# troyvvgroup/quemb

Hardware: AMD Instinct MI355X
Metric: fragment CCSD iters/sec (full BE sweep over synthetic n_occ=20 n_virt=200 fragments); corr-E error vs oracle in parity_max_abs_err_Eh / parity_n220_abs_err_Eh (higher is better)
Workload: dtype f64

## Files before the change

include/qemb_hip_ops.h:

```cpp
#ifndef QEMB_HIP_OPS_H
#define QEMB_HIP_OPS_H
#include "qemb_hip.h"
#ifdef __cplusplus
extern "C" {
#endif

#define QEMB_TIMER_LADDER 0
#define QEMB_TIMER_RINGS 1
#define QEMB_TIMER_ITER 2
#define QEMB_TIMER_AO2MO 3
#define QEMB_TIMER_SCF 4
#define QEMB_TIMER_GEMM_ANY 5
#define QEMB_TIMER_SCHMIDT 6
#define QEMB_TIMER_DF 7
int qemb_timer_begin(int slot);
int qemb_timer_end(int slot);
int qemb_timer_read(int slot, double* total_ms, int64_t* count);
int qemb_timer_reset(int slot);
int qemb_alloc_stats(long long* n_driver_allocs, long long* n_driver_frees, double* ms_in_driver_calls, double* gb_allocated, int reset);
int qemb_gemm_flop_count(double* flops, int reset);
int qemb_tape_cache_counters(int64_t* reused, int64_t* recorded, int reset);
int qemb_ctx_timer_read(int ctx, int slot, double* total_ms, int64_t* count, int reset);
int qemb_timer_live_events(int slot);


int qemb_op_gemm(int64_t M, int64_t N, int64_t K, double alpha, const double* A, int64_t lda, int a_kcontig,
                 int64_t strideA, const double* B, int64_t ldb, int b_kcontig, int64_t strideB, double beta,
                 double* C, int64_t ldc, int64_t strideC, int64_t batch);
int qemb_op_gemm_slab_rows(int64_t M, int64_t N, int64_t K, const double* A, int64_t lda, int64_t a_slab, int64_t a_slab_skip, const double* B, int64_t ldb,
                           int b_kcontig, double* C, int64_t ldc, int cfg);
int qemb_set_gemm_config(int cfg);
int qemb_mfma_f64_peak(int iters, int blocks_per_cu, double* tflops);
int qemb_set_gemm_splitk(int enabled);
int qemb_op_gemm_probe(int64_t M, int64_t N, int64_t K, const double* A, int64_t lda, int a_kcontig, const double* B, int64_t ldb, int b_kcontig,
                       double* C, int64_t ldc, int cfg, int ksplit, double* ms, double* clock_ghz, int64_t* workgroups);
int qemb_op_gemm_stamps(int64_t M, int64_t N, int64_t K, const double* A, int64_t lda, const double* B, int64_t ldb, double* C, int64_t ldc, int cfg,
                        int ksplit, double* out7);
int qemb_pair_gemm_choice(int64_t rows, int64_t cols, int* cfg, int* ksplit);
int qemb_ccsd_gemm_plans(int o, int v, int64_t* out);
int qemb_ccsd_ring_plan(int o, int v, int64_t* out);
int qemb_set_gemm_ksplit(int ksplit);
int qemb_gemm_tile_table(int index, int* id, int* rows, int* cols, int* bk, int* mode1, int* has_classic, int* ladder_twin);
int qemb_gemm_last_launch(int* cfg, int* vec2, int* mode, int* ksplit, int* sb_m, int* sb_n, int* wide_c);
int qemb_op_copy4(const int64_t dim[4], const double* in, const int64_t si[4], double* out,
                  const int64_t so[4], double alpha, double beta);
int qemb_op_outer4(const int64_t dim[4], const double* u, int64_t su0, int64_t su2, const double* v,
                   int64_t sv1, int64_t sv3, double* out, const int64_t so[4], double alpha, double beta);
int qemb_op_div_denom(double* x, int64_t d0, int64_t d1, int64_t d2, int64_t d3, const double* ea,
                      const double* eb, const double* ec, const double* ed);
int qemb_op_ladder_pack_vvvv(int64_t n, int64_t o, const double* M, double* Vp, int64_t ldp, double* Vm, int64_t ldm);
int qemb_op_ladder_pack_tau(int64_t o, int64_t v, const double* tau, double* Tp, int64_t ldp, double* Tm, int64_t ldm);
int qemb_op_ladder_scatter_pm(int64_t o, int64_t v, const double* Rp, int64_t ldp, const double* Rm, int64_t ldm, double* t2);
int qemb_op_dot(int64_t n, const double* x, const double* y, double* out_dev);
int qemb_op_absmax(int64_t n, const double* x, double* out_dev);
int qemb_op_gemv_rows(int64_t rows, int64_t cols, const double* T, int64_t ldt, const double* x, double* y,
                      double alpha, double beta);
int qemb_op_gemv_rows_batched(int64_t rows, int64_t cols, int64_t nbatch, const double* T, int64_t ldt, int64_t strideT,
                              const double* x, int64_t stridex, double* y, double alpha, double beta);
int qemb_op_contract_mid(int64_t outer, int64_t mid, int64_t inner, const double* T, const double* x,
                         double* Y, int64_t ldy, double alpha, double beta);
int qemb_op_unpack_s4(int64_t n, const double* s4, double* s1);
int qemb_op_pack_s4(int64_t n, const double* s1, double* s4);
int qemb_op_unpack_s8_to_s4(int64_t n, const double* s8, double* s4);
int qemb_op_mirror_lower(int64_t n, double* A, int64_t lda);
int qemb_op_k_from_pairs(int64_t n, const double* H, const double* D, double* K);
int qemb_op_jk_from_packed(int64_t n, const double* S4, const double* D, const double* Dp, double* Jp, double* K);
int qemb_op_pack_pm_cols(int64_t rows, int64_t v, const double* in, double* Op, int64_t ldp, double* Om, int64_t ldm);
int qemb_op_scatter_pm_rows(int64_t o, int64_t ncols, const double* Xp, const double* Xm, double* out);
int qemb_op_pack_w_pm(int64_t o, const double* W, double* Ap, int64_t lda_p, double* Am, int64_t lda_m);
int qemb_op_ladder_scatter_pm2(int64_t o, int64_t v, const double* Rp, int64_t ldp, const double* Rm, int64_t ldm, const double* Hp, const double* Hm,
                               int assign, double* t2);
int qemb_op_lincomb2(int64_t n, double a, const double* x, double b, const double* y, double beta, double* out);
int qemb_op_small_k_update(int64_t batch, int64_t M, int64_t N, int64_t K, double alpha, const double* A, int64_t sA, const double* B, int64_t sB, double* C, int64_t sC);
int qemb_op_ccsd_ph_layouts(int64_t o, int64_t v, const double* t2, const double* t1, double* T, double* Tp, double* S, double* Ut, double* Tpt, double* Th);
int qemb_op_ccsd_y_traces(int64_t o, int64_t v, const double* ZC, const double* ZB, double* Y);
int qemb_op_ccsd_ph_layouts_ring(int64_t o, int64_t v, const double* t2, const double* t1, double* Tp, double* S, double* Ut, double* Tpt);
int qemb_op_ccsd_ovvv_slabs(int64_t o, int64_t v);
int qemb_op_ccsd_ovvv_pass(int64_t o, int64_t v, const double* ovvv, const double* t1, const double* Thk, double* ZB, double* PA);
int qemb_op_ccsd_ring_prep(int64_t o, int64_t v, const double* t1, const double* P1, const double* W1base, const double* W2base, const double* ZB, const double* ZC,
                           const double* OB, const double* OC, double* R, double* W2);
int qemb_op_ccsd_ring_prep_rule(int64_t o, int64_t v, int replay);
int qemb_op_ccsd_u_update(int64_t o, int64_t v, const double* A, const double* t1, const double* Z, double* U);
int qemb_op_copy4_two(const int64_t dim[4], const double* in, const int64_t si[4], double* out, const int64_t so[4], double alpha, double beta, const double* base,
                      double* out2, const double* in2, double c2a, double c2b);
int qemb_op_scatter_pm_rows_add(int64_t o, int64_t ncols, const double* Xp, const double* Xm, double* out, const double* add);
int qemb_op_ccsd_y_traces_add(int64_t o, int64_t v, const double* ZC, const double* ZB, double* Y, const double* add);
int qemb_op_pack_w_pm_sum(int64_t o, const double* Wt, const double* X, const double* At, double* Ap, int64_t lda_p, double* Am, int64_t lda_m);
int qemb_op_ccsd_t1_assemble(int64_t o, int64_t v, const double* t1, const double* Lvv, const double* Loo, const double* Fov, const double* S, const double* Lph1,
                             const double* PA, int SA, int64_t strideA, const double* PB, int SB, int64_t strideB, double* t1n);
int qemb_op_gemv_rows_two(int64_t rows1, int64_t cols1, const double* T1, int64_t ld1, const double* x1, double* y1, double a1, double b1,
                          int64_t rows2, int64_t cols2, const double* T2, int64_t ld2, const double* x2, double* y2, double a2, double b2);
int qemb_op_ccsd_y_traces_slabs(int64_t o, int64_t v, const double* ZC, const double* ZB, double* Y, const double* add, int S, int64_t stride, double scale);
int qemb_op_ccsd_finish_t2_rings(int64_t o, int64_t v, double* t2n, const double* U, const double* OV, const double* RS, const double* M, const double* eo, const double* ev, double* t1n);
int qemb_op_diis_push(int64_t n, const double* trial, const double* prev, double* e, double* xcopy, int m, const double* const* ys, int self, double* row_dev, double* row_host);
int qemb_op_ccsd_extrapolate_energy(int64_t o, int64_t v, int nterms, const double* coef, const double* const* xs, double* amp, const double* L, double* tau, double* e_host);
int qemb_op_gather_rows(int64_t nrows, int64_t len, const int64_t* idx_dev, const double* src, int64_t ld, double* dst);
int qemb_op_scale_rows(int64_t nrows, int64_t len, double* x, const double* s);
int qemb_op_pack_pair_rows(int64_t n, int64_t ncols, const double* in, double* out);
int qemb_op_unpack_tril_pair_rows(int64_t nr, int64_t n, const double* in, double* full);
int qemb_op_extract_pf(int64_t n, const double* Mp, int64_t p0, int64_t q0, int64_t r0, int64_t s0, int64_t sp, int64_t sq,
                       int64_t sr, int64_t ss, double* out);
int qemb_op_extract_pf_t(int64_t n, const double* T, int64_t x0, int64_t r0, int64_t s0, int64_t c0, int64_t sx, int64_t sr,
                         int64_t ss, int64_t sc, double* out);
int qemb_op_ladder_pack_vvvv_pf(int64_t n, int64_t o, const double* Mp, double* Vp, int64_t ldp, double* Vm, int64_t ldm);
int qemb_op_extract_pf_t_compact(int64_t n, const double* T, int64_t x0, int64_t c0, int64_t sx, int64_t sr, int64_t ss, int64_t sc,
                                 double* out, int64_t slab);
int qemb_op_gather_pair_cols(int64_t rows, int64_t n, const double* in, int64_t r0, int64_t s0, int64_t sr, int64_t ss, double* out);
int qemb_op_extract_ps(int64_t n, const double* S, int64_t p0, int64_t q0, int64_t r0, int64_t s0, int64_t sp, int64_t sq,
                       int64_t sr, int64_t ss, double* out);
int qemb_op_extract_ps_packed(int64_t n, const double* S, int64_t p0, int64_t q0, int64_t r0, int64_t sp, int64_t sq, int64_t sr, double* out);
int qemb_op_unpack_pair_block(int64_t n, int64_t o, const double* S, double* Mv, int64_t ld);
int qemb_op_ladder_pack_vvvv_pf_ld(int64_t n, int64_t o, const double* Mp, int64_t ld, double* Vp, int64_t ldp, double* Vm, int64_t ldm);
int qemb_op_pack_pm_ovvv(int64_t o, int64_t v, const double* ovvv, double* Op, int64_t ldp, double* Om, int64_t ldm);
int qemb_op_df_pair_product(int64_t np, int64_t naux, const double* bb, double* out);
int qemb_op_unpack_tril_rows(int64_t rows, int64_t n, const double* packed, double* full);
int qemb_op_pack_tril_rows(int64_t rows, int64_t n, const double* full, double* packed);
int qemb_op_jacobi_eigh(int64_t n, double* A, double* w, double* V, int* sweeps);
int qemb_op_scf_fused_max(void);
int qemb_op_jacobi_eigh_in_basis(int64_t n, const double* F, const double* Cp, double* w, double* C_out, double* C2_out, int nocc, double* dm_out, double stop_below, int* sweeps);
int qemb_op_scf_fock_small(int64_t n, const double* h, const double* J, const double* K, const double* D, double* F, double* err, double* scal2);
int qemb_op_pack_density_sym(int64_t n, const double* D, double* Dp);
int qemb_op_jacobi_svd(int64_t m, int64_t n, double* G, double* s, double* U, double* V, int* sweeps);
int qemb_op_cholesky_lower(int64_t n, double* A);
int qemb_op_tri_inverse_lower(int64_t n, const double* L, double* Linv);


int qemb_op_mp2_amplitudes(int64_t o, int64_t v, const double* ovov, const double* eo, const double* ev, double* t2, double* G, double* e_host);

int qemb_op_rdm2_assemble(int kind, int64_t o, int64_t v, const double* t1, const double* t2, const double* dm1c, double* out);
int qemb_op_ccsd_t(int o, int v, const double* t1, const double* t2, const double* ovvv, const double* ovoo, const double* ovov, const double* eo, const double* ev, int tile, double* e_t);
int qemb_op_rdm2_add_nc(int64_t m, const double* g, double alpha, double* X);
int qemb_op_rdm2_symmetrize(int64_t m, const double* g, double* X);
int qemb_op_rdm2_eri_dot(int64_t m, int sym, const double* eri, const double* K, double* e_host);

int qemb_op_kdf_split(int64_t rows, int64_t nao, const double* z, double* planes);
int qemb_op_kdf_stack(int64_t nk, int64_t nao, int64_t n, const double* ta, double* Cs, double* Dk);
int qemb_op_kdf_pack(int64_t naux, int64_t n, const double* M, int paired, double w, double* F, int64_t ldf, double* out2_host);

int qemb_frag_prepare_ccsd(qemb_frag_t f, int nsocc, const double* h, const double* dm0, const qemb_solver_opts* opts);
int qemb_frag_ccsd_iterate(qemb_frag_t f, int niter, double* e_corr, double* normt);
int qemb_frag_ccsd_reset(qemb_frag_t f);
int qemb_frag_ccsd_export(qemb_frag_t f, const char* name, double* host, int64_t nelem);


int qemb_op_boys(int m_max, int64_t n, const double* x, double* out);
int qemb_op_int3c_class(int la, int lb, int lP, const void* bf_a, const void* bf_b, const void* bf_P, const double* c2s, double* out_host);
int qemb_op_int4c_class(int la, int lb, int lc, int ld, const void* bf_a, const void* bf_b, const void* bf_c, const void* bf_d, const double* c2s, double* out_host);
int qemb_op_int4c_tile(void* basis, const int32_t* pairs_r, int64_t n_r, const int32_t* pairs_s, int64_t n_s, double thresh, double* out_host);
int qemb_op_cd_panel_factor(int n, const double* A_host, double thr, double* T_host, int32_t* piv_host, int32_t* rank, int* in_lds);
int qemb_op_cd_diag_update(int64_t np, int r, const double* Lnew_host, const int32_t* pivrow_host, double* d_host, int64_t nsp, const int32_t* row0_host, const int32_t* cnt_host,
                           double* spmax_host, double* dmax_host);
int qemb_op_cd_permute(int64_t M, int64_t N, const double* L_host, const int32_t* pos_host, int full, double* out_host);
int qemb_op_df_get_ints(void* df, double* out_host, int* identity_metric);

int qemb_op_fci_sigma(int n, int nsocc, const double* h_host, const double* V_dev, const double* c_dev, double* sigma_dev);
int qemb_op_fci_rdm12(int n, int nsocc, const double* c_dev, int cumulant, double* dm1_host, double* dm2_dev);
int qemb_op_fci_sigma_timed(int n, int nsocc, const double* h_host, const double* V_dev, const double* c_dev, double* sigma_dev, double* ms3);
int qemb_op_fci_sigma_slab(int n, int nsocc, const double* h_host, const double* V_dev, const double* c_dev, double* sigma_dev, int64_t rows, double* ms3);
int qemb_op_fci_rdm12_slab(int n, int nsocc, const double* c_dev, int cumulant, int64_t rows, double* dm1_host, double* dm2_dev);
int qemb_op_fci_links(int n, int nsocc, int64_t* ns, int* nlink, int32_t* strings_host, int32_t* links_host);
int qemb_op_sci_screen(int n, int nsocc, const double* h_host, const double* V_dev, int64_t ndet, const uint64_t* alpha, const uint64_t* beta, const double* c, double eps,
                       int64_t slab, int64_t cap, int64_t max_out, int64_t* njoined, uint64_t* out_alpha, uint64_t* out_beta);
int qemb_op_sci_pt2(int n, int nsocc, const double* h_host, const double* V_dev, int64_t ndet, const uint64_t* alpha, const uint64_t* beta, const double* c, double e_var, double eps_pt,
                    int64_t max_ext, int64_t slab, int64_t cap, double* e_pt2, int64_t* n_ext, int* batches);
int qemb_op_sci_merge(int64_t ndet, const uint64_t* alpha, const uint64_t* beta, const double* c, int64_t njoined, const uint64_t* jalpha, const uint64_t* jbeta,
                      uint64_t* out_alpha, uint64_t* out_beta, double* out_c);
int qemb_op_sci_matrix(int n, const double* h_host, const double* V_dev, int64_t ndet, const uint64_t* alpha, const uint64_t* beta, int64_t max_nnz, int64_t* nnz,
                       int64_t* rowptr, int32_t* col, double* val);
int qemb_op_sci_spmv(int n, const double* h_host, const double* V_dev, int64_t ndet, const uint64_t* alpha, const uint64_t* beta, const double* x, double* y);
int qemb_op_sci_rdm12(int n, int nsocc, const double* h_host, const double* V_dev, int64_t ndet, const uint64_t* alpha, const uint64_t* beta, const double* c, int cumulant,
                      double* dm1, double* dm2);
int qemb_frag_sci_stage_ms(qemb_frag_t f, double* ms5);

int qemb_op_joint_diag(int64_t K, int64_t m, double* Q_dev, double* U_dev, double stop_angle, int max_sweeps, int* sweeps, double* f, int* converged);
int qemb_op_joint_diag_bytes(int64_t K, int64_t m, int64_t* bytes, int* in_lds);
int qemb_op_joint_diag_mem_limit(int64_t bytes);

#ifdef __cplusplus
}
#endif
#endif
```

quemb_amd/_lib.py:

```python

from __future__ import annotations

import ctypes as C
import os
from pathlib import Path

import numpy as np

_HERE = Path(__file__).resolve().parent
LIB_PATH = _HERE / "libqemb_hip.so"

c_dp = C.POINTER(C.c_double)
c_i64 = C.c_int64
c_vp = C.c_void_p


QEMB_ERR_ARG, QEMB_ERR_ALLOC, QEMB_ERR_DEVICE, QEMB_ERR_NOCONV, QEMB_ERR_NUMERIC, QEMB_ERR_UNSUPPORTED = -1, -2, -3, -4, -5, -6


class QembError(RuntimeError):

    def __init__(self, msg="", status=None):
        super().__init__(msg)
        self.status = status


class SolverOpts(C.Structure):
    _fields_ = [("struct_size", C.c_uint32), ("cc_conv_tol", C.c_double), ("cc_conv_tol_normt", C.c_double), ("cc_max_cycle", C.c_int),
                ("cc_diis_space", C.c_int), ("scf_conv_tol", C.c_double), ("scf_conv_tol_grad", C.c_double),
                ("scf_max_cycle", C.c_int), ("scf_diis_space", C.c_int), ("warm_start", C.c_int), ("verbose", C.c_int),
                ("relax_density", C.c_int), ("lambda_conv_tol", C.c_double), ("lambda_max_cycle", C.c_int),
                ("strict_convergence", C.c_int)]


class FciOpts(C.Structure):
    _fields_ = [("struct_size", C.c_uint32), ("conv_tol", C.c_double), ("max_cycle", C.c_int), ("max_space", C.c_int), ("lindep", C.c_double)]


class SciOpts(C.Structure):
    _fields_ = [("struct_size", C.c_uint32), ("eps_var", C.c_double), ("conv_tol", C.c_double), ("max_cycle", C.c_int), ("max_space", C.c_int),
                ("max_round", C.c_int), ("max_det", C.c_int64)]


_lib = None
_initialised_device = None


def _declare(lib):
    def f(name, restype, *argtypes):
        fn = getattr(lib, name)
        fn.restype = restype
        fn.argtypes = list(argtypes)

    I, D, P, V, L = C.c_int, C.c_double, c_vp, c_vp, c_i64
    f("qemb_init", I, I)
    f("qemb_last_error", C.c_char_p)
    f("qemb_backend", C.c_char_p)
    f("qemb_sync", I)
    f("qemb_device_sync", I)
    f("qemb_mem_info", I, C.POINTER(C.c_size_t), C.POINTER(C.c_size_t))
    f("qemb_malloc", I, C.POINTER(c_vp), C.c_size_t)
    f("qemb_free", I, V)
    f("qemb_trim", I)
    f("qemb_trim_all", I)
    f("qemb_h2d", I, V, V, C.c_size_t)
    f("qemb_d2h", I, V, V, C.c_size_t)
    f("qemb_h2d_async", I, V, V, C.c_size_t)
    f("qemb_d2d", I, V, V, C.c_size_t)
    f("qemb_timer_begin", I, I)
    f("qemb_timer_end", I, I)
    f("qemb_timer_read", I, I, C.POINTER(D), C.POINTER(L))
    f("qemb_timer_reset", I, I)
    f("qemb_timer_live_events", I, I)
    f("qemb_op_gemm", I, L, L, L, D, P, L, I, L, P, L, I, L, D, P, L, L, L)
    f("qemb_op_gemm_slab_rows", I, L, L, L, P, L, L, L, P, L, I, P, L, I)
    f("qemb_op_gemm_probe", I, L, L, L, P, L, I, P, L, I, P, L, I, I, C.POINTER(D), C.POINTER(D), C.POINTER(L))
    f("qemb_op_gemm_stamps", I, L, L, L, P, L, P, L, P, L, I, I, C.POINTER(D))
    f("qemb_set_gemm_config", I, I)
    f("qemb_set_gemm_splitk", I, I)
    f("qemb_set_gemm_ksplit", I, I)
    f("qemb_pair_gemm_choice", I, L, L, C.POINTER(I), C.POINTER(I))
    f("qemb_ccsd_gemm_plans", I, I, I, C.POINTER(L))
    f("qemb_ccsd_ring_plan", I, I, I, C.POINTER(L))
    f("qemb_gemm_tile_table", I, I, *([C.POINTER(I)] * 7))
    f("qemb_gemm_last_launch", I, *([C.POINTER(I)] * 7))
    f("qemb_op_ladder_pack_vvvv", I, L, L, P, P, L, P, L)
    f("qemb_op_ladder_pack_tau", I, L, L, P, P, L, P, L)
    f("qemb_op_ladder_scatter_pm", I, L, L, P, L, P, L, P)
    f("qemb_mfma_f64_peak", I, I, I, C.POINTER(D))
    f("qemb_op_copy4", I, C.POINTER(L), P, C.POINTER(L), P, C.POINTER(L), D, D)
    f("qemb_op_outer4", I, C.POINTER(L), P, L, L, P, L, L, P, C.POINTER(L), D, D)
    f("qemb_op_div_denom", I, P, L, L, L, L, P, P, P, P)
    f("qemb_op_dot", I, L, P, P, P)
    f("qemb_op_mp2_amplitudes", I, L, L, P, P, P, P, P, C.POINTER(D))
    f("qemb_op_rdm2_assemble", I, I, L, L, P, P, P, P)
    f("qemb_op_rdm2_add_nc", I, L, P, D, P)
    f("qemb_op_rdm2_symmetrize", I, L, P, P)
    f("qemb_op_rdm2_eri_dot", I, L, I, P, P, C.POINTER(D))
    f("qemb_op_absmax", I, L, P, P)
    f("qemb_op_gemv_rows", I, L, L, P, L, P, P, D, D)
    f("qemb_op_gemv_rows_batched", I, L, L, L, P, L, L, P, L, P, D, D)
    f("qemb_op_contract_mid", I, L, L, L, P, P, P, L, D, D)
    f("qemb_op_unpack_s4", I, L, P, P)
    f("qemb_op_pack_s4", I, L, P, P)
    f("qemb_op_unpack_s8_to_s4", I, L, P, P)
    f("qemb_op_unpack_tril_rows", I, L, L, P, P)
    f("qemb_op_pack_pair_rows", I, L, L, P, P)
    f("qemb_op_mirror_lower", I, L, P, L)
    f("qemb_op_k_from_pairs", I, L, P, P, P)
    f("qemb_op_jk_from_packed", I, L, P, P, P, P, P)
    f("qemb_op_pack_pm_cols", I, L, L, P, P, L, P, L)
    f("qemb_op_scatter_pm_rows", I, L, L, P, P, P)
    f("qemb_op_pack_w_pm", I, L, P, P, L, P, L)
    f("qemb_op_ladder_scatter_pm2", I, L, L, P, L, P, L, P, P, I, P)
    f("qemb_op_lincomb2", I, L, D, P, D, P, D, P)
    f("qemb_op_small_k_update", I, L, L, L, L, D, P, L, P, L, P, L)
    f("qemb_op_ccsd_ph_layouts", I, L, L, P, P, P, P, P, P, P, P)
    f("qemb_op_ccsd_ph_layouts_ring", I, L, L, P, P, P, P, P, P)
    f("qemb_op_ccsd_ring_prep", I, L, L, P, P, P, P, P, P, P, P, P, P)
    f("qemb_op_ccsd_ring_prep_rule", I, L, L, I)
    f("qemb_op_ccsd_u_update", I, L, L, P, P, P, P)
    f("qemb_op_ccsd_ovvv_slabs", I, L, L)
    f("qemb_op_ccsd_ovvv_pass", I, L, L, P, P, P, P, P)
    f("qemb_op_ccsd_y_traces", I, L, L, P, P, P)
    f("qemb_op_copy4_two", I, C.POINTER(L), P, C.POINTER(L), P, C.POINTER(L), D, D, P, P, P, D, D)
    f("qemb_op_scatter_pm_rows_add", I, L, L, P, P, P, P)
    f("qemb_op_ccsd_y_traces_add", I, L, L, P, P, P, P)
    f("qemb_op_pack_w_pm_sum", I, L, P, P, P, P, L, P, L)
    f("qemb_op_ccsd_t1_assemble", I, L, L, P, P, P, P, P, P, P, I, L, P, I, L, P)
    f("qemb_op_gemv_rows_two", I, L, L, P, L, P, P, D, D, L, L, P, L, P, P, D, D)
    f("qemb_op_ccsd_y_traces_slabs", I, L, L, P, P, P, P, I, L, D)
    f("qemb_op_ccsd_finish_t2_rings", I, L, L, P, P, P, P, P, P, P, P)
    f("qemb_op_diis_push", I, L, P, P, P, P, I, P, I, P, P)
    f("qemb_op_ccsd_extrapolate_energy", I, L, L, I, P, P, P, P, P, P)
    f("qemb_op_gather_rows", I, L, L, P, P, L, P)
    f("qemb_op_scale_rows", I, L, L, P, P)
    f("qemb_ctx_count", I, I)
    f("qemb_ctx_bind", I, I)
    f("qemb_ctx_partition", I, I)
    f("qemb_ctx_timer_read", I, I, I, C.POINTER(C.c_double), C.POINTER(c_i64), I)
    f("qemb_gemm_flop_count", I, C.POINTER(C.c_double), I)
    f("qemb_tape_cache_counters", I, C.POINTER(L), C.POINTER(L), I)
    f("qemb_alloc_stats", I, C.POINTER(C.c_longlong), C.POINTER(C.c_longlong), C.POINTER(C.c_double), C.POINTER(C.c_double), I)
    f("qemb_op_unpack_tril_pair_rows", I, L, L, P, P)
    f("qemb_op_extract_pf", I, L, P, L, L, L, L, L, L, L, L, P)
    f("qemb_op_extract_pf_t", I, L, P, L, L, L, L, L, L, L, L, P)
    f("qemb_op_ladder_pack_vvvv_pf", I, L, L, P, P, L, P, L)
    f("qemb_op_extract_pf_t_compact", I, L, P, L, L, L, L, L, L, P, L)
    f("qemb_op_gather_pair_cols", I, L, L, P, L, L, L, L, P)
    f("qemb_op_extract_ps", I, L, P, L, L, L, L, L, L, L, L, P)
    f("qemb_op_extract_ps_packed", I, L, P, L, L, L, L, L, L, P)
    f("qemb_op_unpack_pair_block", I, L, L, P, P, L)
    f("qemb_op_ladder_pack_vvvv_pf_ld", I, L, L, P, L, P, L, P, L)
    f("qemb_op_pack_pm_ovvv", I, L, L, P, P, L, P, L)
    f("qemb_op_df_pair_product", I, L, L, P, P)
    f("qemb_op_pack_tril_rows", I, L, L, P, P)
    f("qemb_op_jacobi_eigh", I, L, P, P, P, C.POINTER(I))
    f("qemb_op_scf_fused_max", I)
    f("qemb_op_jacobi_eigh_in_basis", I, L, P, P, P, P, P, I, P, D, C.POINTER(I))
    f("qemb_op_scf_fock_small", I, L, P, P, P, P, P, P, P)
    f("qemb_op_pack_density_sym", I, L, P, P)
    f("qemb_op_jacobi_svd", I, L, L, P, P, P, P, C.POINTER(I))
    f("qemb_op_cholesky_lower", I, L, P)
    f("qemb_op_joint_diag", I, L, L, P, P, D, I, C.POINTER(I), C.POINTER(D), C.POINTER(I))
    f("qemb_df_localize_er", I, V, P, I, D, I, P, C.POINTER(I), C.POINTER(D), C.POINTER(D), C.POINTER(I))
    f("qemb_op_joint_diag_bytes", I, L, L, C.POINTER(L), C.POINTER(I))
    f("qemb_op_joint_diag_mem_limit", I, L)
    f("qemb_op_tri_inverse_lower", I, L, P, P)
    f("qemb_comm_unique_id", I, P)
    f("qemb_comm_init", I, I, I, P)
    f("qemb_comm_info", I, C.POINTER(I), C.POINTER(I))
    f("qemb_comm_allreduce", I, P, L, I)
    f("qemb_comm_destroy", I)
    OP = C.POINTER(SolverOpts)
    IP = C.POINTER(I)
    DP = C.POINTER(D)
    f("qemb_default_opts", None, OP)
    f("qemb_frag_create", I, I, I, C.POINTER(c_vp))
    f("qemb_frag_free", I, V)
    f("qemb_frag_set_eri_s4", I, V, P)
    f("qemb_frag_set_eri_s4_dev", I, V, P)
    f("qemb_frag_set_df_factor", I, V, I, P)
    f("qemb_frag_set_df_factor_dev", I, V, I, P)
    f("qemb_frag_mo_route", I, V, I)
    f("qemb_frag_set_df_only", I, V, I, P)
    f("qemb_frag_set_df_only_dev", I, V, I, V)
    f("qemb_frag_resident_bytes", I, V, C.POINTER(L))
    f("qemb_frag_mo_route_used", I, V, IP, IP)
    f("qemb_frag_get_eri_s4", I, V, P)
    f("qemb_frag_set_energy_data", I, V, P, P, P, D, IP, I)
    f("qemb_frag_jk", I, V, P, P, P)
    f("qemb_frag_solve", I, V, I, P, P, OP, I, P, P, P, P, P, P, P, DP, DP, DP, IP, IP)
    f("qemb_frag_solve_mp2", I, V, I, P, P, OP, I, P, P, P, P, P, P, DP, DP, DP, IP)
    f("qemb_frag_solve_mp2_batch", I, I, P, IP, P, P, OP, I, P, P, P, P, P, P, P, P, P, IP)
    f("qemb_default_fci_opts", None, C.POINTER(FciOpts))
    f("qemb_frag_solve_fci", I, V, I, P, P, OP, C.POINTER(FciOpts), I, P, P, P, P, P, P, DP, DP, DP, IP, IP)
    f("qemb_frag_fci_bytes", I, I, I, I, C.POINTER(L))
    f("qemb_frag_fci_mem_limit", I, V, L)
    f("qemb_frag_fci_residual", I, V, DP)
    f("qemb_frag_fci_slab", I, V, L)
    f("qemb_frag_fci_bytes_slab", I, I, I, I, L, C.POINTER(L))
    f("qemb_frag_fci_slab_used", I, V, C.POINTER(L), C.POINTER(L))
    f("qemb_op_fci_sigma_slab", I, I, I, P, P, P, P, L, P)
    f("qemb_op_fci_rdm12_slab", I, I, I, P, I, L, P, P)
    f("qemb_op_fci_sigma", I, I, I, P, P, P, P)
    f("qemb_op_fci_rdm12", I, I, I, P, I, P, P)
    f("qemb_op_fci_sigma_timed", I, I, I, P, P, P, P, P)
    f("qemb_op_fci_links", I, I, I, C.POINTER(L), IP, P, P)
    f("qemb_default_sci_opts", None, C.POINTER(SciOpts))
    f("qemb_frag_solve_sci", I, V, I, P, P, OP, C.POINTER(SciOpts), I, P, P, P, P, P, DP, DP, DP, IP, IP)
    f("qemb_frag_sci_stats", I, V, C.POINTER(L), IP, C.POINTER(L), DP)
    f("qemb_frag_sci_stage_ms", I, V, P)
    f("qemb_frag_sci_dets", I, V, P, P, P)
    f("qemb_frag_sci_bytes", I, I, I, L, I, C.POINTER(L))
    f("qemb_frag_sci_mem_limit", I, V, L)
    f("qemb_frag_sci_pt2", I, V, D, L, DP, C.POINTER(L), IP, P)
    f("qemb_frag_sci_pt2_bytes", I, I, I, L, L, C.POINTER(L))
    f("qemb_op_sci_pt2", I, I, I, P, P, L, P, P, P, D, D, L, L, L, DP, C.POINTER(L), IP)
    f("qemb_op_sci_screen", I, I, I, P, P, L, P, P, P, D, L, L, L, C.POINTER(L), P, P)
    f("qemb_op_sci_merge", I, L, P, P, P, L, P, P, P, P, P)
    f("qemb_op_sci_matrix", I, I, P, P, L, P, P, L, C.POINTER(L), P, P, P)
    f("qemb_op_sci_spmv", I, I, P, P, L, P, P, P, P)
    f("qemb_op_sci_rdm12", I, I, I, P, P, L, P, P, P, I, P, P)
    f("qemb_frag_rdm2", I, V, I, I, P)
    f("qemb_frag_rdm2_mem_limit", I, V, L)
    f("qemb_frag_ccsd_t", I, V, DP, IP, C.POINTER(L), P)
    f("qemb_frag_ccsd_t_bytes", I, V, I, I, C.POINTER(L))
    f("qemb_frag_ccsd_t_mem_limit", I, V, L)
    f("qemb_frag_drop_amplitudes", I, V)
    f("qemb_op_ccsd_t", I, I, I, P, P, P, P, P, P, P, I, DP)
    f("qemb_frag_rdm2_dev", I, V, I, I, P)
    f("qemb_rdm2_full_guard", I, L, L, L)
    f("qemb_frag_lambda_iters", I, P, C.POINTER(C.c_int))
    f("qemb_frag_solve_batch", I, I, P, IP, P, P, OP, I, P, P, P, P, P, P, P, P, P, P, IP, IP, C.POINTER(L))
    f("qemb_frag_scf", I, V, I, P, P, OP, P, P, P, P, DP, IP, IP)
    f("qemb_frag_cphf", I, V, I, P, P, OP, P, I, P)
    f("qemb_ccsd_solve", I, I, I, I, P, P, P, OP, P, P, D, IP, I, P, P, P, P, P, P, DP, IP)
    f("qemb_frag_prepare_ccsd", I, V, I, P, P, OP)
    f("qemb_frag_ccsd_iterate", I, V, I, DP, DP)
    f("qemb_frag_ccsd_reset", I, V)
    f("qemb_frag_ccsd_export", I, V, C.c_char_p, P, L)
    LP = C.POINTER(L)
    f("qemb_aoeri_upload", I, I, P, I, C.POINTER(c_vp))
    f("qemb_aoeri_free", I, V)
    f("qemb_ao2mo_dense", I, V, P, I, P, V)
    f("qemb_df_create", I, I, P, C.POINTER(c_vp))
    f("qemb_lpq_upload", I, P, I, C.POINTER(c_vp))
    f("qemb_df_create_pbc", I, I, P, C.POINTER(c_vp), IP)
    f("qemb_df_alloc_ints", I, V, I)
    f("qemb_df_add_pw_block", I, V, I, P, P, P, P)
    f("qemb_df_add_rs_block", I, V, I, I, P)
    f("qemb_df_pw_imag_absmax", I, V, C.POINTER(C.c_double))
    f("qemb_df_pw_select", I, V, I)
    f("qemb_df_free", I, V)
    f("qemb_df_set_ints", I, V, I, P, I)
    f("qemb_df_set_ints_semisparse", I, V, I, L, P, P, P, P)
    f("qemb_df_transform", I, V, P, I, P, V)
    f("qemb_df_transform_screened", I, V, P, I, P, D, P, V)
    f("qemb_df_transform_factor", I, V, P, I, V)
    f("qemb_df_transform_screened_factor", I, V, P, I, P, D, V)
    f("qemb_kdf_create", I, I, I, I, IP, IP, C.POINTER(c_vp))
    f("qemb_kdf_set_pair", I, V, I, I, P)
    f("qemb_kdf_transform", I, V, P, I, P, V, I)
    f("qemb_kdf_free", I, V)
    f("qemb_kdf_guard", I, I, I, I, I, I, I, L)
    f("qemb_frag_get_df_factor", I, V, P)
    f("qemb_int_basis_create", I, I, P, C.c_size_t, P, C.POINTER(c_vp))
    f("qemb_int_basis_free", I, V)
    f("qemb_int3c2e", I, V, V, P, L, I, P, I)
    f("qemb_int2c2e", I, V, P, I)
    f("qemb_df_create_empty", I, C.POINTER(c_vp))
    f("qemb_df_set_ints_from_basis", I, V, V, V)
    f("qemb_df_set_ints_semisparse_from_basis", I, V, V, V, L, P, P, P, P)
    f("qemb_int4c2e", I, V, I, D, P, I)
    f("qemb_int4c_mem_limit", I, V, L)
    f("qemb_int4c_stats", I, V, C.POINTER(L), C.POINTER(L))
    f("qemb_aoeri_from_basis", I, V, D, C.POINTER(c_vp))
    f("qemb_int_jk_direct", I, V, P, D, P, P, I)
    f("qemb_int_jk_direct_bytes", I, V, C.POINTER(L))
    f("qemb_ao2mo_direct", I, V, I, P, P, P, P, L, D)
    f("qemb_ao2mo_direct_bytes", I, V, I, P, L, C.POINTER(L))
    f("qemb_int4c_tile_stats", I, V, C.POINTER(L), C.POINTER(L))
    f("qemb_op_int4c_tile", I, V, P, L, P, L, D, P)
    f("qemb_int_cholesky", I, V, D, D, L, L, P, C.POINTER(L))
    f("qemb_int_cholesky_bytes", I, V, L, L, C.POINTER(L))
    f("qemb_int_cholesky_stats", I, V, P)
    f("qemb_df_set_ints_from_cholesky", I, V, V, D, D, L, L)
# ... 112 lines not shown
```

quemb_amd/csrc/api.cpp:

```cpp
#include <cstring>
#include <cstdlib>
#include <vector>
#include <execinfo.h>
#include <signal.h>
#include <unistd.h>
#include "../../include/qemb_hip_ops.h"
#include "dev_ops.h"
#include "ccsd.h"
#include "fragment.h"
#include "ao2mo.h"
#include "kdf.h"
#include "int3c.h"
#include "int4c.h"
#include "cd_core.h"
#include "loc_core.h"
#include "sci_core.h"
#include <algorithm>
#include <cmath>
#include <mutex>
#include <set>

using namespace qemb;
namespace qemb {
int dev_mfma_f64_peak(int iters, int blocks_per_cu, double* tflops);
// ... 111 lines not shown
  if (ksplit) *ksplit = p.ks;
  return QEMB_OK;
}
int qemb_ccsd_gemm_plans(int o, int v, int64_t* out) {
  if (o < 1 || v < 0 || !out) { set_error("qemb_ccsd_gemm_plans: bad arguments"); return QEMB_ERR_ARG; }
  const CcsdGemmPlans p = ccsd_gemm_plans(o, v);
  for (const GemmPlan* g : {&p.fvv, &p.pa, &p.pb, &p.ladder_p, &p.ladder_m, &p.xw_p, &p.xw_m, &p.x_p, &p.x_m})
    for (const int64_t x : {g->M, g->N, g->K, (int64_t)g->cfg, (int64_t)g->ks, (int64_t)g->S}) *out++ = x;
  return QEMB_OK;
}
int qemb_ccsd_ring_plan(int o, int v, int64_t* out) {
  if (o < 1 || v < 0 || !out) { set_error("qemb_ccsd_ring_plan: bad arguments"); return QEMB_ERR_ARG; }
  const CcsdRingPlan r = ccsd_ring_plan(o, v);
  out[0] = ((int64_t)o * o * v * v <= (int64_t)1 << 22) ? 1 : 0; out[1] = r.cfg; out[2] = r.ks; out[3] = r.region_ws_bytes;
  return QEMB_OK;
}
int qemb_set_gemm_splitk(int enabled) { dev_gemm_set_auto_splitk(enabled); return QEMB_OK; }
int qemb_op_copy4(const int64_t dim[4], const double* in, const int64_t si[4], double* out, const int64_t so[4],
                  double alpha, double beta) {
  Copy4Desc c{};
  for (int k = 0; k < 4; ++k) { c.dim[k] = dim[k]; c.si[k] = si[k]; c.so[k] = so[k]; }
  c.in = in; c.out = out; c.alpha = alpha; c.beta = beta;
  return dev_copy4(c);
}
int qemb_op_outer4(const int64_t dim[4], const double* u, int64_t su0, int64_t su2, const double* v, int64_t sv1,
                   int64_t sv3, double* out, const int64_t so[4], double alpha, double beta) {
  Outer4Desc o{};
  for (int k = 0; k < 4; ++k) { o.dim[k] = dim[k]; o.so[k] = so[k]; }
  o.u = u; o.su0 = su0; o.su2 = su2; o.v = v; o.sv1 = sv1; o.sv3 = sv3; o.out = out; o.alpha = alpha; o.beta = beta;
  return dev_outer4(o);
}
int qemb_op_div_denom(double* x, int64_t d0, int64_t d1, int64_t d2, int64_t d3, const double* ea, const double* eb,
                      const double* ec, const double* ed) { return dev_div_denom(x, d0, d1, d2, d3, ea, eb, ec, ed); }
int qemb_op_ladder_pack_vvvv(int64_t n, int64_t o, const double* M, double* Vp, int64_t ldp, double* Vm, int64_t ldm) { return dev_ladder_pack_vvvv(n, o, M, Vp, ldp, Vm, ldm); }
int qemb_op_ladder_pack_tau(int64_t o, int64_t v, const double* tau, double* Tp, int64_t ldp, double* Tm, int64_t ldm) { return dev_ladder_pack_tau(o, v, tau, Tp, ldp, Tm, ldm); }
int qemb_op_ladder_scatter_pm(int64_t o, int64_t v, const double* Rp, int64_t ldp, const double* Rm, int64_t ldm, double* t2) { return dev_ladder_scatter_pm(o, v, Rp, ldp, Rm, ldm, t2); }
int qemb_op_dot(int64_t n, const double* x, const double* y, double* o) { return dev_dot(n, x, y, o); }
int qemb_op_absmax(int64_t n, const double* x, double* o) { return dev_absmax(n, x, o); }
int qemb_op_gemv_rows(int64_t rows, int64_t cols, const double* T, int64_t ldt, const double* x, double* y, double alpha,
                      double beta) { return dev_gemv_rows(rows, cols, T, ldt, x, y, alpha, beta); }
int qemb_op_gemv_rows_batched(int64_t rows, int64_t cols, int64_t nbatch, const double* T, int64_t ldt, int64_t strideT, const double* x,
                              int64_t stridex, double* y, double alpha, double beta) { return dev_gemv_rows_batched(rows, cols, nbatch, T, ldt, strideT, x, stridex, y, alpha, beta); }
int qemb_op_contract_mid(int64_t outer, int64_t mid, int64_t inner, const double* T, const double* x, double* Y,
                         int64_t ldy, double alpha, double beta) { return dev_contract_mid(outer, mid, inner, T, x, Y, ldy, alpha, beta); }
int qemb_op_unpack_s4(int64_t n, const double* s4, double* s1) { return dev_unpack_s4(n, s4, s1); }
int qemb_op_pack_s4(int64_t n, const double* s1, double* s4) { return dev_pack_s4(n, s1, s4); }
int qemb_op_unpack_s8_to_s4(int64_t n, const double* s8, double* s4) { return dev_unpack_s8_to_s4(n, s8, s4); }
int qemb_comm_unique_id(void* id) { return dev_comm_unique_id(id); }
int qemb_comm_init(int rank, int world, const void* id) { return dev_comm_init(rank, world, id); }
int qemb_comm_info(int* rank, int* world) { return dev_comm_info(rank, world); }
int qemb_comm_allreduce(double* buf, int64_t n, int op) { return dev_comm_allreduce(buf, n, op); }
int qemb_comm_destroy(void) { return dev_comm_destroy(); }
int qemb_ctx_count(int n) { return dev_ctx_count(n); }
int qemb_ctx_bind(int k) { return dev_ctx_bind(k); }
int qemb_ctx_partition(int parts) { return dev_ctx_partition(parts); }
int qemb_op_gemm_slab_rows(int64_t M, int64_t N, int64_t K, const double* A, int64_t lda, int64_t a_slab, int64_t a_slab_skip, const double* B, int64_t ldb,
                           int b_kcontig, double* C, int64_t ldc, int cfg) {
  GemmDesc g{};
  g.M = M; g.N = N; g.K = K; g.alpha = 1.0; g.beta = 0.0;
  g.A = A; g.lda = lda; g.a_kcontig = 0; g.strideA = 0; g.a_slab = a_slab; g.a_slab_skip = a_slab_skip;
  g.B = B; g.ldb = ldb; g.b_kcontig = b_kcontig; g.strideB = 0;
  g.C = C; g.ldc = ldc; g.strideC = 0; g.batch = 1; g.cfg = cfg; g.ksplit = 0;
  return dev_gemm(g);
}
int qemb_gemm_flop_count(double* flops, int reset) { return dev_gemm_flop_count(flops, reset); }
int qemb_tape_cache_counters(int64_t* reused, int64_t* recorded, int reset) {
  long long a = 0, b = 0;
  tape_cache_counters(&a, &b, reset);
  if (reused) *reused = a;
  if (recorded) *recorded = b;
  return QEMB_OK;
}
int qemb_alloc_stats(long long* n, long long* nfree, double* ms, double* gb, int reset) { return dev_alloc_stats(n, nfree, ms, gb, reset); }
int qemb_ctx_timer_read(int ctx, int slot, double* total_ms, int64_t* count, int reset) { return dev_ctx_timer_read(ctx, slot, total_ms, count, reset); }
int qemb_op_k_from_pairs(int64_t n, const double* H, const double* D, double* K) { return dev_k_from_pairs(n, H, D, K); }
int qemb_op_jk_from_packed(int64_t n, const double* S4, const double* D, const double* Dp, double* Jp, double* K) { return dev_jk_from_packed(n, S4, D, Dp, Jp, K); }
int qemb_op_pack_pm_cols(int64_t rows, int64_t v, const double* in, double* Op, int64_t ldp, double* Om, int64_t ldm) { return dev_pack_pm_cols(rows, v, in, Op, ldp, Om, ldm); }
int qemb_op_scatter_pm_rows(int64_t o, int64_t ncols, const double* Xp, const double* Xm, double* out) { return dev_scatter_pm_rows(o, ncols, Xp, Xm, out); }
int qemb_op_pack_w_pm(int64_t o, const double* W, double* Ap, int64_t lda_p, double* Am, int64_t lda_m) { return dev_pack_w_pm(o, W, Ap, lda_p, Am, lda_m); }
int qemb_op_ladder_scatter_pm2(int64_t o, int64_t v, const double* Rp, int64_t ldp, const double* Rm, int64_t ldm, const double* Hp, const double* Hm,
                               int assign, double* t2) { return dev_ladder_scatter_pm2(o, v, Rp, ldp, Rm, ldm, Hp, Hm, assign, t2); }
int qemb_op_lincomb2(int64_t n, double a, const double* x, double b, const double* y, double beta, double* out) {
  const double c[2] = {a, b};
  const double* xs[2] = {x, y};
  return dev_lincomb(n, 2, c, xs, beta, out);
}
int qemb_op_mirror_lower(int64_t n, double* A, int64_t lda) { return dev_mirror_lower(n, A, lda); }
int qemb_op_small_k_update(int64_t batch, int64_t M, int64_t N, int64_t K, double alpha, const double* A, int64_t sA, const double* B, int64_t sB, double* C, int64_t sC) {
  return dev_small_k_update(batch, M, N, K, alpha, A, sA, B, sB, C, sC);
}
int qemb_op_ccsd_ph_layouts(int64_t o, int64_t v, const double* t2, const double* t1, double* T, double* Tp, double* S, double* Ut, double* Tpt, double* Th) {
  return dev_ccsd_ph_layouts(o, v, t2, t1, T, Tp, S, Ut, Tpt, Th);
}
int qemb_op_ccsd_ph_layouts_ring(int64_t o, int64_t v, const double* t2, const double* t1, double* Tp, double* S, double* Ut, double* Tpt) {
  return dev_ccsd_ph_layouts_ring(o, v, t2, t1, Tp, S, Ut, Tpt);
}
int qemb_op_ccsd_ring_prep(int64_t o, int64_t v, const double* t1, const double* P1, const double* W1base, const double* W2base, const double* ZB, const double* ZC,
                           const double* OB, const double* OC, double* R, double* W2) {
  return dev_ccsd_ring_prep(o, v, t1, P1, W1base, W2base, ZB, ZC, OB, OC, R, W2);
}
int qemb_op_ccsd_u_update(int64_t o, int64_t v, const double* A, const double* t1, const double* Z, double* U) { return dev_ccsd_u_update(o, v, A, t1, Z, U); }
int qemb_op_ccsd_ring_prep_rule(int64_t o, int64_t v, int replay) { return ccsd_use_ring_prep(o, v, replay != 0) ? 1 : 0; }
int qemb_op_ccsd_ovvv_slabs(int64_t o, int64_t v) { return dev_ccsd_ovvv_slabs(o, v); }
int qemb_op_ccsd_ovvv_pass(int64_t o, int64_t v, const double* ovvv, const double* t1, const double* Thk, double* ZB, double* PA) {
  return dev_ccsd_ovvv_pass(o, v, ovvv, t1, Thk, ZB, PA);
}
int qemb_op_copy4_two(const int64_t dim[4], const double* in, const int64_t si[4], double* out, const int64_t so[4], double alpha, double beta, const double* base,
                      double* out2, const double* in2, double c2a, double c2b) {
  Copy4Desc c{};
  for (int k = 0; k < 4; ++k) { c.dim[k] = dim[k]; c.si[k] = si[k]; c.so[k] = so[k]; }
  c.in = in; c.out = out; c.alpha = alpha; c.beta = beta; c.base = base;
  c.out2 = out2; c.in2 = in2; c.c2a = c2a; c.c2b = c2b;
  return dev_copy4(c);
}
int qemb_op_scatter_pm_rows_add(int64_t o, int64_t ncols, const double* Xp, const double* Xm, double* out, const double* add) { return dev_scatter_pm_rows(o, ncols, Xp, Xm, out, add); }
int qemb_op_ccsd_y_traces_add(int64_t o, int64_t v, const double* ZC, const double* ZB, double* Y, const double* add) { return dev_ccsd_y_traces(o, v, ZC, ZB, Y, add); }
int qemb_op_pack_w_pm_sum(int64_t o, const double* Wt, const double* X, const double* At, double* Ap, int64_t lda_p, double* Am, int64_t lda_m) {
  return dev_pack_w_pm_sum(o, Wt, X, At, Ap, lda_p, Am, lda_m);
}
int qemb_op_ccsd_t1_assemble(int64_t o, int64_t v, const double* t1, const double* Lvv, const double* Loo, const double* Fov, const double* S, const double* Lph1,
                             const double* PA, int SA, int64_t strideA, const double* PB, int SB, int64_t strideB, double* t1n) {
  return dev_ccsd_t1_assemble(o, v, t1, Lvv, Loo, Fov, S, Lph1, PA, SA, strideA, PB, SB, strideB, t1n);
}
int qemb_op_gemv_rows_two(int64_t rows1, int64_t cols1, const double* T1, int64_t ld1, const double* x1, double* y1, double a1, double b1,
                          int64_t rows2, int64_t cols2, const double* T2, int64_t ld2, const double* x2, double* y2, double a2, double b2) {
  return dev_gemv_rows_two(rows1, cols1, T1, ld1, x1, y1, a1, b1, rows2, cols2, T2, ld2, x2, y2, a2, b2);
}
int qemb_op_ccsd_y_traces_slabs(int64_t o, int64_t v, const double* ZC, const double* ZB, double* Y, const double* add, int S, int64_t stride, double scale) {
  return dev_ccsd_y_traces(o, v, ZC, ZB, Y, add, S, stride, scale);
}
int qemb_op_ccsd_finish_t2_rings(int64_t o, int64_t v, double* t2n, const double* U, const double* OV, const double* RS, const double* M, const double* eo, const double* ev, double* t1n) {
  return dev_ccsd_finish_t2_rings(o, v, t2n, U, OV, RS, M, eo, ev, t1n);
}
int qemb_op_diis_push(int64_t n, const double* trial, const double* prev, double* e, double* xcopy, int m, const double* const* ys, int self, double* row_dev, double* row_host) {
  void* pin = nullptr;
  QTRY(dev_pinned_alloc(&pin, sizeof(double) * 8));
  int rc = dev_diis_push(n, trial, prev, e, xcopy, m, ys, self, row_dev, (double*)pin);
  if (!rc) rc = dev_sync();
  if (!rc) for (int j = 0; j < m; ++j) row_host[j] = ((double*)pin)[j];
  dev_pinned_free(pin);
  return rc;
}
int qemb_op_ccsd_extrapolate_energy(int64_t o, int64_t v, int nterms, const double* coef, const double* const* xs, double* amp, const double* L, double* tau, double* e_host) {
  void* pin = nullptr;
  DBuf e_dev;
  QTRY(e_dev.alloc(1));
  QTRY(dev_pinned_alloc(&pin, sizeof(double) * 8));
  int rc = dev_ccsd_extrapolate_energy(o, v, nterms, coef, xs, amp, L, tau, e_dev, (double*)pin);
  if (!rc) rc = dev_sync();
  if (!rc) *e_host = *(double*)pin;
  dev_pinned_free(pin);
  return rc;
}
int qemb_op_ccsd_y_traces(int64_t o, int64_t v, const double* ZC, const double* ZB, double* Y) { return dev_ccsd_y_traces(o, v, ZC, ZB, Y); }
int qemb_op_gather_rows(int64_t nrows, int64_t len, const int64_t* idx_dev, const double* src, int64_t ld, double* dst) { return dev_gather_rows(nrows, len, idx_dev, src, ld, dst); }
int qemb_op_scale_rows(int64_t nrows, int64_t len, double* x, const double* s) { return dev_scale_rows(nrows, len, x, s); }
int qemb_op_pack_pair_rows(int64_t n, int64_t ncols, const double* in, double* out) { return dev_pack_pair_rows(n, ncols, in, out); }
int qemb_op_extract_pf(int64_t n, const double* Mp, int64_t p0, int64_t q0, int64_t r0, int64_t s0, int64_t sp, int64_t sq, int64_t sr, int64_t ss, double* out) {
  return dev_extract_pf(n, Mp, p0, q0, r0, s0, sp, sq, sr, ss, out);
}
int qemb_op_extract_pf_t(int64_t n, const double* T, int64_t x0, int64_t r0, int64_t s0, int64_t c0, int64_t sx, int64_t sr, int64_t ss, int64_t sc, double* out) {
  return dev_extract_pf_t(n, T, x0, r0, s0, c0, sx, sr, ss, sc, out);
}
int qemb_op_ladder_pack_vvvv_pf(int64_t n, int64_t o, const double* Mp, double* Vp, int64_t ldp, double* Vm, int64_t ldm) { return dev_ladder_pack_vvvv_pf(n, o, Mp, Vp, ldp, Vm, ldm); }
int qemb_op_extract_pf_t_compact(int64_t n, const double* T, int64_t x0, int64_t c0, int64_t sx, int64_t sr, int64_t ss, int64_t sc, double* out, int64_t slab) {
  return dev_extract_pf_t_compact(n, T, x0, c0, sx, sr, ss, sc, out, slab);
}
int qemb_op_gather_pair_cols(int64_t rows, int64_t n, const double* in, int64_t r0, int64_t s0, int64_t sr, int64_t ss, double* out) {
  return dev_gather_pair_cols(rows, n, in, r0, s0, sr, ss, out);
}
int qemb_op_extract_ps(int64_t n, const double* S, int64_t p0, int64_t q0, int64_t r0, int64_t s0, int64_t sp, int64_t sq, int64_t sr, int64_t ss, double* out) {
  return dev_extract_ps(n, S, p0, q0, r0, s0, sp, sq, sr, ss, out);
}
int qemb_op_extract_ps_packed(int64_t n, const double* S, int64_t p0, int64_t q0, int64_t r0, int64_t sp, int64_t sq, int64_t sr, double* out) {
  return dev_extract_ps_packed(n, S, p0, q0, r0, sp, sq, sr, out);
}
int qemb_op_unpack_pair_block(int64_t n, int64_t o, const double* S, double* Mv, int64_t ld) { return dev_unpack_pair_block(n, o, S, Mv, ld); }
int qemb_op_ladder_pack_vvvv_pf_ld(int64_t n, int64_t o, const double* Mp, int64_t ld, double* Vp, int64_t ldp, double* Vm, int64_t ldm) {
  return dev_ladder_pack_vvvv_pf_ld(n, o, Mp, ld, Vp, ldp, Vm, ldm);
}
int qemb_op_pack_pm_ovvv(int64_t o, int64_t v, const double* ovvv, double* Op, int64_t ldp, double* Om, int64_t ldm) { return dev_pack_pm_ovvv(o, v, ovvv, Op, ldp, Om, ldm); }
int qemb_op_df_pair_product(int64_t np, int64_t naux, const double* bb, double* out) { return df_pair_product(np, naux, bb, out); }
int qemb_op_unpack_tril_pair_rows(int64_t nr, int64_t n, const double* in, double* full) { return dev_unpack_tril_pair_rows(nr, n, in, full); }
int qemb_op_unpack_tril_rows(int64_t rows, int64_t n, const double* p, double* f) { return dev_unpack_tril_rows(rows, n, p, f); }
int qemb_op_pack_tril_rows(int64_t rows, int64_t n, const double* f, double* p) { return dev_pack_tril_rows(rows, n, f, p); }
int qemb_op_jacobi_eigh(int64_t n, double* A, double* w, double* V, int* sweeps) { return dev_jacobi_eigh(n, A, w, V, sweeps); }
int qemb_op_scf_fused_max(void) { return dev_scf_fused_max(); }
int qemb_op_jacobi_eigh_in_basis(int64_t n, const double* F, const double* Cp, double* w, double* C_out, double* C2_out, int nocc, double* dm_out, double stop_below, int* sweeps) {
  DBuf st;
  QTRY(st.alloc(1));
  QTRY(dev_jacobi_eigh_in_basis(n, F, Cp, w, C_out, C2_out, nocc, dm_out, stop_below, reinterpret_cast<int*>(st.p)));
  double word = 0.0;
  QTRY(dev_d2h(&word, st.p, sizeof(double)));
  int sw; std::memcpy(&sw, &word, sizeof(int));
  if (sweeps) *sweeps = sw;
  return jacobi_status_code(sw, "dev_jacobi_eigh_in_basis");
}
int qemb_op_scf_fock_small(int64_t n, const double* h, const double* J, const double* K, const double* D, double* F, double* err, double* scal2) { return dev_scf_fock_small(n, h, J, K, D, F, err, scal2); }
int qemb_op_pack_density_sym(int64_t n, const double* D, double* Dp) { return dev_pack_density_sym(n, D, Dp); }
int qemb_op_jacobi_svd(int64_t m, int64_t n, double* G, double* s, double* U, double* V, int* sweeps) { return dev_jacobi_svd(m, n, G, s, U, V, sweeps); }
int qemb_op_cholesky_lower(int64_t n, double* A) { return dev_cholesky_lower(n, A); }
static thread_local int64_t g_joint_diag_limit = -1;
int qemb_op_joint_diag_mem_limit(int64_t bytes) { g_joint_diag_limit = bytes; return QEMB_OK; }
int qemb_op_joint_diag_bytes(int64_t K, int64_t m, int64_t* bytes, int* in_lds) {
  if (K < 0 || m < 0 || !bytes) { set_error("qemb_op_joint_diag_bytes: bad arguments"); return QEMB_ERR_ARG; }
  *bytes = (int64_t)loc::footprint_bytes(K, m);
  if (in_lds) *in_lds = loc::in_lds(K, m) ? 1 : 0;
  return QEMB_OK;
}
static int joint_diag_guard(const char* who, int64_t K, int64_t m, double extra_bytes, double to_allocate) {
  size_t free_b = 0, total_b = 0;
  QTRY(dev_mem_info(&free_b, &total_b));
  const double need = loc::footprint_bytes(K, m) + extra_bytes;
  if ((g_joint_diag_limit >= 0 && need > (double)g_joint_diag_limit) || to_allocate > (double)free_b) {
    set_error(std::string(who) + ": with K = " + std::to_string(K) + " and m = " + std::to_string(m) + " the stack, U and the workspace take " + std::to_string(need * 1e-9) +
              " GB (" + std::to_string(to_allocate * 1e-9) + " GB still to allocate), more than the " +
              std::to_string((g_joint_diag_limit >= 0 && (double)g_joint_diag_limit < (double)free_b ? (double)g_joint_diag_limit : (double)free_b) * 1e-9) + " GB they may take");
    return QEMB_ERR_ALLOC;
  }
  return QEMB_OK;
}
int qemb_op_joint_diag(int64_t K, int64_t m, double* Q_dev, double* U_dev, double stop_angle, int max_sweeps, int* sweeps, double* f, int* converged) {
  QTRY(loc::check_joint_diag("qemb_op_joint_diag", K, m, Q_dev != nullptr, U_dev != nullptr, stop_angle, max_sweeps));
  QTRY(joint_diag_guard("qemb_op_joint_diag", K, m, 0.0, 8.0 * (double)loc::work_doubles(K, m)));
  return dev_joint_diag(K, m, Q_dev, U_dev, stop_angle, max_sweeps, sweeps, f, converged);
}
int qemb_df_localize_er(qemb_df_t df, const double* C_host, int m, double stop_angle, int max_sweeps, double* U_host, int* sweeps, double* f_before, double* f_after, int* converged) {
  if (!df || !C_host || !U_host) { set_error("qemb_df_localize_er: null argument"); return QEMB_ERR_ARG; }
  const DfContext* d = reinterpret_cast<const DfContext*>(df);
  if (d->Usp.p || d->Lpq_im.p) { set_error("qemb_df_localize_er: a semi-sparse or periodic context holds no dense real 3-index tensor"); return QEMB_ERR_UNSUPPORTED; }
  if ((!d->Linv.p && !d->identity_metric) || !d->Lpq.p || d->N <= 0 || d->naux <= 0) { set_error("qemb_df_localize_er: metric and 3-index integrals must be set"); return QEMB_ERR_ARG; }
  if (m <= 0 || m > d->N) { set_error("qemb_df_localize_er: need 0 < m <= N"); return QEMB_ERR_ARG; }
  const int64_t K = d->naux, N = d->N, np = (int64_t)m * (m + 1) / 2;
  QTRY(loc::check_joint_diag("qemb_df_localize_er", K, m, true, true, stop_angle, max_sweeps));
  const double transform_b = 8.0 * ((double)K * m * N + (double)K * m * m + (d->identity_metric ? 1.0 : 2.0) * (double)K * np + (double)N * m);
  QTRY(joint_diag_guard("qemb_df_localize_er", K, m, transform_b, transform_b + loc::footprint_bytes(K, m)));
  DBuf dC, bb, Q, U;
  QTRY(dC.alloc(N * m));
  QTRY(dev_h2d(dC, C_host, sizeof(double) * N * m));
  QTRY(d->transform(dC, m, nullptr, nullptr, 0.0, &bb));
  QTRY(Q.alloc(K * m * m));
  QTRY(dev_unpack_tril_rows(K, m, bb, Q));
  bb.release();
  QTRY(U.alloc((int64_t)m * m));
  int cv0 = 0;
  QTRY(dev_joint_diag(K, m, Q, U, stop_angle, 0, nullptr, f_before, &cv0));
  QTRY(dev_joint_diag(K, m, Q, U, stop_angle, max_sweeps, sweeps, f_after, converged));
  return dev_d2h(U_host, U, sizeof(double) * m * m);
}

int qemb_op_tri_inverse_lower(int64_t n, const double* L, double* Linv) { return dev_tri_inverse_lower(n, L, Linv); }
int qemb_op_boys(int m_max, int64_t n, const double* x, double* out) { QTRY(dev_boys(m_max, n, x, out)); return dev_sync(); }
int qemb_op_int4c_class(int la, int lb, int lc, int ld, const void* bf_a, const void* bf_b, const void* bf_c, const void* bf_d, const double* c2s, double* out_host) {
  const int l[4] = {la, lb, lc, ld};
  const BfRecord* const rec[4] = {reinterpret_cast<const BfRecord*>(bf_a), reinterpret_cast<const BfRecord*>(bf_b), reinterpret_cast<const BfRecord*>(bf_c), reinterpret_cast<const BfRecord*>(bf_d)};
  return int4c_block(l, rec, c2s, out_host);
}
int qemb_op_int3c_class(int la, int lb, int lP, const void* bf_a, const void* bf_b, const void* bf_P, const double* c2s, double* out_host) {
  return int3c_block(la, lb, lP, reinterpret_cast<const BfRecord*>(bf_a), reinterpret_cast<const BfRecord*>(bf_b), reinterpret_cast<const BfRecord*>(bf_P), c2s, out_host);
}
int qemb_op_mp2_amplitudes(int64_t o, int64_t v, const double* ovov, const double* eo, const double* ev, double* t2, double* G, double* e_host) {
  DBuf part, e;
  QTRY(part.alloc(dev_mp2_partial_count(o, v))); QTRY(e.alloc(1));
  QTRY(dev_mp2_amplitudes(o, v, ovov, eo, ev, t2, G, part, e));
  return e_host ? dev_d2h(e_host, e, sizeof(double)) : dev_sync();
}

int qemb_op_rdm2_assemble(int kind, int64_t o, int64_t v, const double* t1, const double* t2, const double* dm1c, double* out) {
  QTRY(dev_rdm2_assemble(kind, o, v, t1, t2, dm1c, out));
  return dev_sync();
}

int qemb_op_ccsd_t(int o, int v, const double* t1, const double* t2, const double* ovvv, const double* ovoo, const double* ovov, const double* eo, const double* ev, int tile, double* e_t) {
  if (!e_t) { set_error("qemb_op_ccsd_t: e_t is NULL"); return QEMB_ERR_ARG; }
  return ccsd_t_energy(o, v, t1, t2, ovvv, ovoo, ovov, eo, ev, tile, e_t, nullptr);
}

int qemb_op_rdm2_add_nc(int64_t m, const double* g, double alpha, double* X) { return dev_rdm2_add_nc(m, g, alpha, X); }
int qemb_op_rdm2_symmetrize(int64_t m, const double* g, double* X) { return dev_rdm2_symmetrize(m, g, X); }
int qemb_op_rdm2_eri_dot(int64_t m, int sym, const double* eri, const double* K, double* e_host) {
  if (!e_host) { set_error("qemb_op_rdm2_eri_dot: e_host is NULL"); return QEMB_ERR_ARG; }
  DBuf w;
  QTRY(w.alloc(rdm2_full_grid(m > 0 ? m : 1) + 1));
  QTRY(dev_rdm2_eri_dot(m, sym, eri, K, w.p + 1, w.p));
  return dev_d2h(e_host, w.p, sizeof(double));
}

int qemb_op_kdf_split(int64_t rows, int64_t nao, const double* z, double* planes) { QTRY(dev_kdf_split(rows, nao, z, planes)); return dev_sync(); }
int qemb_op_kdf_stack(int64_t nk, int64_t nao, int64_t n, const double* ta, double* Cs, double* Dk) { QTRY(dev_kdf_stack(nk, nao, n, ta, Cs, Dk)); return dev_sync(); }
int qemb_op_kdf_pack(int64_t naux, int64_t n, const double* M, int paired, double w, double* F, int64_t ldf, double* out2_host) {
  if (!out2_host) { set_error("qemb_op_kdf_pack: out2_host is NULL"); return QEMB_ERR_ARG; }
  DBuf wk;
  QTRY(wk.alloc(dev_kdf_partial_count(naux > 0 ? naux : 1, n > 0 ? n : 1) + 2));
  QTRY(dev_kdf_pack(naux, n, M, paired, w, F, ldf, wk.p + 2, wk.p));
  return dev_d2h(out2_host, wk.p, 2 * sizeof(double));
}

void qemb_default_opts(qemb_solver_opts* o) {
  CcsdOptions c; ScfOptions s;
  memset(o, 0, sizeof *o);
  o->struct_size = (uint32_t)sizeof(qemb_solver_opts);
  o->cc_conv_tol = c.conv_tol; o->cc_conv_tol_normt = c.conv_tol_normt; o->cc_max_cycle = c.max_cycle; o->cc_diis_space = c.diis_space;
  o->scf_conv_tol = s.conv_tol; o->scf_conv_tol_grad = s.conv_tol_grad; o->scf_max_cycle = s.max_cycle; o->scf_diis_space = s.diis_space;
  o->warm_start = 0; o->verbose = 0;
  LambdaOptions l;
  o->relax_density = 0; o->lambda_conv_tol = l.conv_tol; o->lambda_max_cycle = l.max_cycle;
// ... 933 lines not shown
```

quemb_amd/csrc/ccsd.cpp:

```cpp
#include "ccsd.h"
#include "ao2mo.h"
#include <algorithm>
#include <chrono>
#include <cmath>
#include <cstdio>
#include <cstdlib>
#include <cstring>
#include <string>

namespace qemb {

int mo_slab_ld(int n) { return (n >= 64 && n <= 1024) ? (n + 15) / 16 * 16 : n; }
int64_t mo_transform_work(int n) { return (int64_t)n * mo_slab_ld(n) * ((int64_t)n * (n + 1) / 2); }

static int mo_three_quarter_blocks(int n, int o, int nf, const double* T, int64_t slab, MoIntegrals& out, bool build_T34) {
  const int v = n - o;
  if (nf > 0 && build_T34) {
    QTRY(out.T34.alloc((int64_t)n * n * n * nf));
    QTRY(dev_extract_pf_t(n, T, 0, 0, 0, 0, n, n, n, nf, out.T34, slab));
  } else if (nf > 0) {
    QTRY(out.A1.alloc((int64_t)v * o * v * nf));
    QTRY(out.A2.alloc((int64_t)o * o * v * nf));
    QTRY(dev_extract_pf_t(n, T, o, 0, o, 0, v, o, v, nf, out.A1, slab));
    QTRY(dev_extract_pf_t(n, T, 0, 0, o, 0, o, o, v, nf, out.A2, slab));
// ... 175 lines not shown
  QTRY(axpby(N2, 2.0, W1base_, -1.0, Lph1_));
  {
    QTRY(OVp_.alloc(nov * I_.ldp)); QTRY(OVm_.alloc(nov * I_.ldm));
    if (v >= 32) QTRY(dev_pack_pm_ovvv(o, v, I_.ovvv, OVp_, I_.ldp, OVm_, I_.ldm));
    else {
      DBuf OVl;
      QTRY(OVl.alloc(o * v * vv));
      QTRY(perm4(OVl, I_.ovvv, o, v, v, v, 0, 2, 3, 1));
      QTRY(dev_pack_pm_cols(nov, v, OVl, OVp_, I_.ldp, OVm_, I_.ldm));
    }
  }
  {
    const int64_t npv = v * (v + 1) / 2;
    QTRY(ZCp_.alloc(oo * npv));
    if (I_.ovvv_pk.p) ovvv_pk_ = std::move(I_.ovvv_pk);
    else { QTRY(ovvv_pk_.alloc(o * v * npv)); QTRY(dev_pack_tril_rows(o * v, v, I_.ovvv, ovvv_pk_)); }
  }
  QTRY(Gp_.alloc(oo * I_.ldp)); QTRY(Gm_.alloc(oo * I_.ldm));
  QTRY(dev_pack_pm_cols(oo, v, OVoovv_, Gp_, I_.ldp, Gm_, I_.ldm));
  QTRY(perm4(oooo_p_, I_.oooo, o, o, o, o, 1, 3, 0, 2));
  QTRY(ovoo_cikl_.alloc(v * oo * o));
  QTRY(perm4(ovoo_cikl_, I_.ovoo, o, v, o, o, 1, 3, 2, 0));
  const int64_t na = nov + N2;
  QTRY(amp_.alloc(na)); QTRY(ampn_.alloc(na)); QTRY(diff_.alloc(na));
  for (DBuf* b : {&tau_, &T_, &Tp_, &S_, &W1_, &W2_, &W12_, &W12b_, &R_, &U_}) QTRY(b->alloc(N2));
  const int64_t NG = std::max<int64_t>(N2, oo * o * v);
  QTRY(G2_.alloc(NG));
  plans_ = ccsd_gemm_plans(o, v);
  if (replay_regime()) QTRY(dev_region_workspace_reserve((size_t)ccsd_ring_plan(o, v).region_ws_bytes));
  QTRY(Fvv_.alloc(plans_.fvv.elems()));
  ovvv_pass_ = use_ovvv_pass(o, v, replay_regime());
  ovvv_G_ = ovvv_pass_ ? dev_ccsd_ovvv_slabs(o, v) : 0;
  if (ovvv_pass_ && ovvv_G_ <= 0) ovvv_pass_ = false;
  if (ovvv_pass_) {
    QTRY(LovooK_.alloc(o * v * oo));
    QTRY(perm4(LovooK_, Lovoo_, o, v, o, o, 0, 2, 1, 3));
  }
  ring_prep_ = ccsd_use_ring_prep(o, v, replay_regime());
  if (ring_prep_) {
    QTRY(ovoo_kicl_.alloc(o * v * oo));
    QTRY(perm4(ovoo_kicl_, I_.ovoo, o, v, o, o, 0, 3, 2, 1));
  }
  QTRY(T1P_.alloc((ovvv_pass_ ? (int64_t)ovvv_G_ * nov : plans_.pa.elems()) + plans_.pb.elems()));
  QTRY(Foo_.alloc(oo)); QTRY(Fov_.alloc(nov)); QTRY(Z_.alloc(oo)); QTRY(Y_.alloc(vv));
  QTRY(Ytmp_.alloc(vv)); QTRY(Loo_.alloc(oo)); QTRY(Lvv_.alloc(vv)); QTRY(Q_.alloc(oo)); QTRY(Wo_.alloc(oo * oo));
  QTRY(O1_.alloc(oo * oo)); QTRY(X_.alloc(oo * nov)); QTRY(scal_.alloc(8));
  {
    const int64_t npo = o * (o + 1) / 2, nmo = std::max<int64_t>(o * (o - 1) / 2, 1);
    QTRY(LTp_.alloc(npo * I_.ldp)); QTRY(LRp_.alloc(std::max(npo * I_.ldp, plans_.ladder_p.elems())));
    QTRY(LTm_.alloc(nmo * I_.ldm)); QTRY(LRm_.alloc(std::max(nmo * I_.ldm, plans_.ladder_m.elems())));
    QTRY(Xp_.alloc(plans_.x_p.elems())); QTRY(Xm_.alloc(plans_.x_m.elems()));
    QTRY(Xwp_.alloc(plans_.xw_p.elems())); QTRY(Xwm_.alloc(plans_.xw_m.elems())); QTRY(Xw_.alloc(oo * oo));
    lwp_ = npo + (npo & 1); lwm_ = std::max<int64_t>(2, nmo + (nmo & 1));
    QTRY(WAp_.alloc(npo * lwp_)); QTRY(WAm_.alloc(nmo * lwm_)); QTRY(HRp_.alloc(npo * I_.ldp)); QTRY(HRm_.alloc(nmo * I_.ldm));
    QTRY(ZB_.alloc(N2)); QTRY(ZC_.alloc(N2));
  }
  first_ = true;
  return 0;
}

int CcsdSolver::make_tau(const double* t1, const double* t2, double* tau) {
  const int64_t o = o_, v = v_;
  Outer4Desc d{};
  d.dim[0] = o; d.dim[1] = o; d.dim[2] = v; d.dim[3] = v;
  d.u = t1; d.su0 = v; d.su2 = 1; d.v = t1; d.sv1 = v; d.sv3 = 1;
  d.out = tau; d.so[0] = o * v * v; d.so[1] = v * v; d.so[2] = v; d.so[3] = 1;
  d.alpha = 1.0; d.beta = 1.0; d.base = t2;
  return dev_outer4(d);
}

int CcsdSolver::energy(const double* t1, const double* t2, double* e) {
  QTRY(make_tau(t1, t2, tau_));
  QTRY(dev_dot((int64_t)o_ * o_ * v_ * v_, Loovv_, tau_, scal_));
  return dev_d2h(e, scal_, sizeof(double));
}

int CcsdSolver::init_amps() {
  const int64_t o = o_, v = v_;
  QTRY(dev_fill(t1(), o * v, 0.0));
  QTRY(dcopy(o * o * v * v, OVoovv_, t2()));
  QTRY(dev_div_denom(t2(), o, o, v, v, eo_, eo_, ev_, ev_));
  first_ = true;
  diis_.clear();
  return energy(t1(), t2(), &ecc_);
}

int CcsdSolver::set_amps(const double* t1d, const double* t2d) {
  QTRY(dev_d2d(t1(), t1d, sizeof(double) * o_ * v_));
  QTRY(dev_d2d(t2(), t2d, sizeof(double) * (int64_t)o_ * o_ * v_ * v_));
  first_ = true;
  diis_.clear();
  return energy(t1(), t2(), &ecc_);
}

GemmPlan pick_pair_gemm(int64_t rows, int64_t cols, int64_t K, bool k_aware) {
  int cfg = -1, ks = 0;
  if (cols < 1024) return GemmPlan(rows, cols, K, cfg, ks);
  static const struct { int cfg; double cost; } cand[] = {{GEMM_224x128, 1.0}, {GEMM_192x128, 1.0}, {GEMM_160x128, 1.03}, {GEMM_128x256, 1.0},
                                                          {GEMM_112x128_COL, 1.25}, {GEMM_80x128, 1.08}, {GEMM_64x128_COL, 1.6}, {GEMM_48x128, 1.12}};
  double best_cost = -1.0;
  int64_t tiles = 0;
  for (const auto& c : cand) {
    const int64_t tile_rows = gemm_tile_rows(c.cfg), mt = (rows + tile_rows - 1) / tile_rows;
    if (c.cfg == GEMM_48x128 && mt > 1) continue;
    const double cost = (double)(mt * tile_rows) * c.cost;
    if (best_cost < 0 || cost < best_cost - 1e-9) { best_cost = cost; cfg = c.cfg; tiles = gemm_tile_count(c.cfg, rows, cols); }
  }
  double best = 0.0;
  for (int c = 1; c <= 8; ++c) {
    const int64_t units = tiles * c, rounds = (units + 255) / 256;
    const double eff = (double)units / (double)(rounds * 256) - (c == 1 ? 0.0 : 0.002 * c);
    if (units >= 512 && eff > best + 1e-9) { best = eff; ks = c; }
  }
  if (ks == 0) ks = (int)std::max<int64_t>(1, std::min<int64_t>(8, (1024 + tiles - 1) / tiles));
  if (k_aware && K > 0 && tiles * ks < 256) ks = (int)std::max<int64_t>(ks, std::min<int64_t>(std::min<int64_t>(32, K / 256), (512 + tiles - 1) / tiles));
  return GemmPlan(rows, cols, K, cfg, ks);
}

struct SlabGemm { int S = 1; int64_t stride = 0, ld = 0; };
static int gemm_slabs(const GemmPlan& p, const double* A, int64_t lda, const double* B, int64_t ldb, double* C, int64_t ldc, SlabGemm& out, bool a_kc = true, bool b_kc = true) {
  GemmDesc g{};
  g.M = p.M; g.N = p.N; g.K = p.K; g.alpha = 1.0; g.beta = 0.0;
  g.A = A; g.lda = lda; g.a_kcontig = a_kc ? 1 : 0; g.B = B; g.ldb = ldb; g.b_kcontig = b_kc ? 1 : 0;
  g.C = C; g.ldc = ldc; g.batch = 1; g.cfg = p.cfg; g.ksplit = p.ks;
  out.S = p.S;
  if (out.S > 1) { g.keep_slabs = 1; out.stride = p.M * p.N; out.ld = p.N; }
  else { out.stride = 0; out.ld = ldc; }
  return dev_gemm(g);
}
static GemmPlan pick_xw_split(int64_t rows, int64_t oo, int64_t K) {
  if (K < 2048) return GemmPlan(rows, oo, K, -1, 0);
  const int cfg = GEMM_64x64;
  const int64_t tiles = gemm_tile_count(cfg, rows, oo);
  return GemmPlan(rows, oo, K, cfg, (int)std::max<int64_t>(1, std::min<int64_t>(std::min<int64_t>(64, K / 256), (512 + tiles - 1) / tiles)));
}
static GemmPlan pick_long_k(int64_t M, int64_t N, int64_t K, int cfg, bool many_slices = false) {
  if (cfg < 0) return GemmPlan(M, N, K, cfg, 0);
  int ks = gemm_auto_ksplit(gemm_tile_count(cfg, M, N), K);
  if (many_slices && ks > 1 && M <= 32 && N <= 32) ks = (int)std::min<int64_t>(512, K / 64);
  return GemmPlan(M, N, K, cfg, ks);
}
static int tile_tall(int64_t o) { return (o <= 32) ? GEMM_128x32 : -1; }
static int tile_wide(int64_t o) { return (o <= 32) ? GEMM_32x128 : -1; }
static bool use_ovvv_pass(int64_t o, int64_t v, bool replay) {
  const long long sw = env_int("QEMB_OVVV_PASS", -1);
  if (sw == 0 || !ccsd_ovvv_shape_ok(o, v)) return false;
  return sw > 0 || !replay;
}
bool ccsd_use_ring_prep(int64_t o, int64_t v, bool replay) {
  const long long sw = env_int("QEMB_RING_PREP", -1);
  if (sw == 0 || !ccsd_ring_prep_shape_ok(o, v)) return false;
  return sw > 0 || !replay;
}

CcsdGemmPlans ccsd_gemm_plans(int64_t o, int64_t v) {
  int64_t ldp, ldm;
  packed_pair_lds(v, ldp, ldm);
  const int64_t oo = o * o, vv = v * v, nov = o * v;
  const int64_t npo = o * (o + 1) / 2, nmo = std::max<int64_t>(o * (o - 1) / 2, 1), npv = v * (v + 1) / 2, nmv = std::max<int64_t>(v * (v - 1) / 2, 1);
  CcsdGemmPlans p;
  p.fvv = pick_long_k(v, v, oo * v, (v <= 256) ? GEMM_64x64 : -1);
  p.pa = pick_long_k(o, v, o * vv, tile_wide(o), true);
  p.pb = pick_long_k(o, v, o * v * o, tile_wide(o), true);
  p.ladder_p = pick_pair_gemm(npo, npv, ldp);
  p.ladder_m = pick_pair_gemm(nmo, nmv, ldm);
  p.xw_p = pick_xw_split(npo, oo, ldp);
  p.xw_m = pick_xw_split(nmo, oo, ldm);
  p.x_p = pick_pair_gemm(npo, nov, ldp, true);
  p.x_m = pick_pair_gemm(nmo, nov, ldm, true);
  return p;
}
CcsdRingPlan ccsd_ring_plan(int64_t o, int64_t v) {
  const int64_t nov = o * v;
  CcsdRingPlan r;
  const bool mid_ring = nov >= 1024 && nov < 2048;
  r.cfg = (nov >= 2048) ? GEMM_128x256 : mid_ring ? GEMM_96x96 : (nov >= 256 && gemm_tile_count(GEMM_64x64, nov, nov) >= 200) ? GEMM_64x64 : -1;
  r.ks = mid_ring ? 2 : 0;
  const int S = gemm_slab_count(nov, r.ks > 1 ? r.ks : r.cfg >= 0 ? gemm_auto_ksplit(gemm_tile_count(r.cfg, nov, nov), nov) : 0);
  if (S > 1) r.region_ws_bytes = 2 * (((int64_t)sizeof(double) * S * nov * nov + 255) / 256 * 256);
  return r;
}
int CcsdSolver::apply_ladder(const double* x, double* out, bool rows_packed, bool hh) {
  const int64_t o = o_, v = v_;
  {
    const int64_t npo = o * (o + 1) / 2, nmo = o * (o - 1) / 2, npv = v * (v + 1) / 2, nmv = v * (v - 1) / 2;
    const int64_t ldp = I_.ldp, ldm = I_.ldm;
    if (!rows_packed) QTRY(dev_ladder_pack_tau(o, v, x, LTp_, ldp, LTm_, ldm));
    TimerScope lap_LADDER(TIMER_LADDER);
    SlabGemm sp, sm;
    GemmPlan lp = plans_.ladder_p, lm = plans_.ladder_m;
    lp.cfg = gemm_tile_ladder_symbol(lp.cfg); lm.cfg = gemm_tile_ladder_symbol(lm.cfg);
    QTRY(dev_region_begin());
    QTRY(gemm_slabs(lp, LTp_, ldp, I_.Vp, ldp, LRp_, ldp, sp));
    QTRY(dev_region_chain());
    if (nmo > 0 && nmv > 0) QTRY(gemm_slabs(lm, LTm_, ldm, I_.Vm, ldm, LRm_, ldm, sm));
    QTRY(dev_region_end());
    QTRY(lap_LADDER.close());
    if (hh) {
      static const int cand[] = {GEMM_224x128, GEMM_192x128, GEMM_160x128, GEMM_128x128, GEMM_64x64};
      auto tile_for = [&](int64_t rows) { int best = -1; int64_t pad = -1; for (const int c : cand) { const int64_t r = gemm_tile_rows(c), q = (rows + r - 1) / r * r; if (pad < 0 || q < pad) { pad = q; best = c; } } return best; };
      QTRY(dev_region_begin());
      QTRY(gemm(npo, npv, npo, 1.0, WAp_, lwp_, true, LTp_, ldp, false, 0.0, HRp_, ldp, 1, 0, 0, 0, npv >= 2048 ? tile_for(npo) : -1));
      QTRY(dev_region_chain());
      if (nmo > 0 && nmv > 0) QTRY(gemm(nmo, nmv, nmo, 1.0, WAm_, lwm_, true, LTm_, ldm, false, 0.0, HRm_, ldm, 1, 0, 0, 0, nmv >= 2048 ? tile_for(nmo) : -1));
      QTRY(dev_region_end());
      QTRY(dev_ladder_scatter_pm2(o, v, LRp_, sp.ld, LRm_, sm.ld, HRp_, (nmo > 0 && nmv > 0) ? HRm_.p : nullptr, 1, out, sp.S, sp.stride, sm.S, sm.stride, ldp, ldm));
    } else {
      QTRY(dev_ladder_scatter_pm2(o, v, LRp_, sp.ld, LRm_, sm.ld, nullptr, nullptr, 0, out, sp.S, sp.stride, sm.S, sm.stride));
    }
  }
  return 0;
}

int CcsdSolver::update_amps(double* t1n, double* t2n) {
  const int64_t o = o_, v = v_, nov = o * v, oo = o * o, vv = v * v;
  const double* t1 = this->t1();
  const double* t2 = this->t2();
  QTRY(dev_region_begin());
  if (ovvv_pass_) QTRY(dev_ccsd_ph_layouts_ring(o, v, t2, t1, Tp_, S_, W12_, W12b_));
  else QTRY(dev_ccsd_ph_layouts(o, v, t2, t1, T_, Tp_, S_, W12_, W12b_, R_));
  QTRY(dev_region_chain());
  QTRY(dev_ladder_pack_tau(o, v, tau_, LTp_, I_.ldp, LTm_, I_.ldm));
  QTRY(dev_region_end());

  {
    const int64_t nmo = o * (o - 1) / 2, nmv = v * (v - 1) / 2;
    SlabGemm sp, sm;
    QTRY(dev_region_begin());
    QTRY(gemm_slabs(plans_.xw_p, LTp_, I_.ldp, Gp_, I_.ldp, Xwp_, oo, sp));
    QTRY(dev_region_chain());
    if (nmo > 0) {
      if (nmv > 0) QTRY(gemm_slabs(plans_.xw_m, LTm_, I_.ldm, Gm_, I_.ldm, Xwm_, oo, sm));
      else QTRY(dev_fill(Xwm_, nmo * oo, 0.0));
    }
    QTRY(dev_region_end());
    QTRY(dev_scatter_pm_rows(o, oo, Xwp_, Xwm_, Xw_, nullptr, sp.S, sp.stride, sm.S, sm.stride));
  }
  QTRY(dev_foo_from_x(o, Xw_, Loo_));
  SlabGemm sfvv;
  double fvv_scale = -1.0;
  if (plans_.fvv.ks > 1) QTRY(gemm_slabs(plans_.fvv, tau_, v, Loovv_, v, Fvv_, v, sfvv, false, false));
  else { QTRY(gemm(v, v, oo * v, -1.0, tau_, v, false, Loovv_, v, false, 0.0, Fvv_, v, 1, 0, 0, 0, plans_.fvv.cfg)); fvv_scale = 1.0; }
  QTRY(dev_gemv_rows_two(nov, nov, Lovov_, nov, t1, Fov_, 1.0, 0.0, oo, nov, LovooT_, nov, t1, Loo_, 1.0, 1.0));
  const int cfg_tall = tile_tall(o), cfg_wide = tile_wide(o);
  double* PA = T1P_.p;
  QTRY(dev_region_begin());
  if (ovvv_pass_) QTRY(dev_ccsd_ovvv_pass(o, v, I_.ovvv, t1, S_, ZB_, PA));
  else QTRY(gemm(o * vv, o, v, 1.0, I_.ovvv, v, true, t1, v, true, 0.0, ZB_, o, 1, 0, 0, 0, cfg_tall));
  QTRY(dev_region_chain());
  {
    const int64_t npv = v * (v + 1) / 2;
    const bool vec_ok = (npv % 2) == 0;
    QTRY(gemm(o, npv, v, 1.0, t1, v, true, ovvv_pk_, npv, false, 0.0, ZCp_, npv, o, 0, v * npv, o * npv, vec_ok ? cfg_wide : -1));
    QTRY(dev_unpack_tril_rows(oo, v, ZCp_, ZC_));
  }
  QTRY(dev_region_end());
  QTRY(dev_ccsd_y_traces(o, v, ZC_, ZB_, Lvv_, Fvv_, sfvv.S, sfvv.stride, fvv_scale));

  SlabGemm spa, spb;
  double* PB = nullptr;
  if (ovvv_pass_) {
    spa.S = ovvv_G_; spa.stride = nov; spa.ld = v;
    PB = PA + (int64_t)spa.S * nov;
    QTRY(gemm_slabs(plans_.pb, LovooK_, o, t2, v, PB, v, spb, false, false));
  } else {
    QTRY(dev_region_begin());
    QTRY(gemm_slabs(plans_.pa, R_, o * vv, I_.ovvv, v, PA, v, spa, true, false));
    PB = PA + (int64_t)spa.S * nov;
    QTRY(dev_region_chain());
    QTRY(gemm_slabs(plans_.pb, Lovoo_, o, T_, v, PB, v, spb, false, false));
    QTRY(dev_region_end());
  }
  QTRY(dev_ccsd_t1_assemble(o, v, t1, Lvv_, Loo_, Fov_, S_, Lph1_, PA, spa.S, nov, PB, spb.S, nov, t1n));

  QTRY(gemm(o, oo * o, v, 1.0, t1, v, true, ovoo_cikl_, oo * o, false, 0.0, O1_, oo * o));
  QTRY(dev_pack_w_pm_sum(o, oooo_p_, Xw_, O1_, WAp_, lwp_, WAm_, lwm_));
  QTRY(apply_ladder(tau_, t2n, true, true));

  QTRY(gemm(oo * v, v, v, 1.0, t2, v, true, Lvv_, v, true, 0.0, U_, v));
  QTRY(gemm(o, o * vv, o, -1.0, Loo_, o, false, t2, o * vv, false, 1.0, U_, o * vv, 1, 0, 0, 0, cfg_wide));
  {
    const int64_t nmo = o * (o - 1) / 2;
    SlabGemm sp, sm;
    QTRY(dev_region_begin());
    QTRY(gemm_slabs(plans_.x_p, LTp_, I_.ldp, OVp_, I_.ldp, Xp_, nov, sp));
    QTRY(dev_region_chain());
    if (nmo > 0) QTRY(gemm_slabs(plans_.x_m, LTm_, I_.ldm, OVm_, I_.ldm, Xm_, nov, sm));
    QTRY(dev_region_end());
    QTRY(dev_scatter_pm_rows(o, nov, Xp_, Xm_, X_, ovoo_ijka_, sp.S, sp.stride, sm.S, sm.stride));
  }
  if (!ring_prep_) {
    QTRY(dev_region_begin());
    QTRY(perm4(U_, ZB_, o, v, v, o, 0, 3, 1, 2, 1.0, 1.0));
    QTRY(dev_region_chain());
  }
  QTRY(gemm(oo * v, o, v, 1.0, I_.oovv, v, true, t1, v, true, 0.0, G2_, o, 1, 0, 0, 0, cfg_tall));
  QTRY(gemm(o, v * o, v, 1.0, t1, v, true, I_.ovvo, v * o, false, 1.0, G2_, v * o, o, 0, v * v * o, o * v * o, cfg_wide));
  if (!ring_prep_) QTRY(dev_region_end());
  QTRY(perm4(X_, G2_, o, o, v, o, 3, 1, 0, 2, 1.0, 1.0));
  if (ring_prep_) QTRY(dev_ccsd_u_update(o, v, X_, t1, ZB_, U_));
  else QTRY(dev_small_k_update(oo, v, v, o, -1.0, X_, nov, t1, 0, U_, vv));
  TimerScope lap_RINGS(TIMER_RINGS);
  if (!ring_prep_) {
    QTRY(dev_small_k_update(nov, v, o, o, -1.0, t1, 0, I_.ovoo, oo, ZB_, v * o));
    QTRY(perm4(W1_, ZB_, o, v, v, o, 3, 2, 0, 1, 1.0, 1.0, W1base_));
  }
  const CcsdRingPlan rp = ccsd_ring_plan(o, v);
  auto ring = [&](double al, const double* A, const double* Bsym, double be, double* C) {
    return gemm(nov, nov, nov, al, A, nov, true, Bsym, nov, true, be, C, nov, 1, 0, 0, 0, rp.cfg, rp.ks);
  };
  if (ring_prep_) {
    QTRY(ring(0.25, W12_, Lovov_, 0.0, W1_));
    QTRY(dev_ccsd_ring_prep(o, v, t1, W1_, W1base_, W2base_, ZB_, ZC_, ovoo_kicl_, ovoo_kilc_, R_, W2_));
  } else {
    QTRY(ring(0.25, W12_, Lovov_, 1.0, W1_));
    QTRY(dev_small_k_update(oo, v, v, o, -1.0, t1, 0, ovoo_kilc_, nov, ZC_, vv));
    {
      Copy4Desc c{};
      const int64_t d[4] = {o, o, v, v};
      const int perm[4] = {1, 2, 0, 3};
      int64_t od[4], ostr[4];
      for (int k = 0; k < 4; ++k) od[k] = d[perm[k]];
      ostr[3] = 1; ostr[2] = od[3]; ostr[1] = od[3] * od[2]; ostr[0] = od[3] * od[2] * od[1];
      c.in = ZC_; c.out = W2_; c.alpha = 1.0; c.beta = 1.0; c.base = W2base_;
      c.si[3] = 1; c.si[2] = d[3]; c.si[1] = d[3] * d[2]; c.si[0] = d[3] * d[2] * d[1];
      for (int k = 0; k < 4; ++k) { c.dim[k] = d[k]; c.so[perm[k]] = ostr[k]; }
      c.out2 = R_; c.in2 = W1_; c.c2a = 1.0; c.c2b = -0.5;
      QTRY(dev_copy4(c));
    }
  }
  QTRY(ring(-0.5, W12b_, ovov_t_, 1.0, W2_));
  QTRY(dev_region_begin());
  QTRY(ring(1.0, W2_, Tp_, 0.0, W1_));
  QTRY(dev_region_chain());
  QTRY(ring(1.0, R_, S_, 0.0, W12_));
  QTRY(dev_region_end());
  QTRY(lap_RINGS.close());

  QTRY(dev_ccsd_finish_t2_rings(o, v, t2n, U_, OVoovv_, W12_, W1_, eo_, ev_, t1n));
  return 0;
}

int CcsdSolver::iterate(double* e_corr, double* normt) {
  TimerScope lap_ITER(TIMER_ITER);
  QTRY(iterate_update(false, false, nullptr));
  QTRY(iterate_post(e_corr, normt));
  QTRY(lap_ITER.close());
  return 0;
}

static bool graphs_allowed() {
  static const bool on = env_flag("QEMB_GRAPH", !profiled_run());
  return on;
}
bool CcsdSolver::replay_regime() const { return (int64_t)o_ * o_ * v_ * v_ <= (int64_t)1 << 22 && graph_ok_; }

int CcsdSolver::record_update(bool as_tape, bool* began, bool regions) {
  *began = false;
  const int rc = dev_graph_begin(as_tape ? (regions ? 1 : 2) : 0);
  if (rc != 0) return rc;
  *began = true;
  const int rc2 = update_amps(ampn_.p, ampn_.p + (int64_t)o_ * v_);
  dev_tape_t t = nullptr;
  dev_graph_t g = nullptr;
  const int rc3 = as_tape ? dev_tape_end(&t) : dev_graph_end(&g);
  if (!rc2 && !rc3) { if (as_tape) tape_ = t; else graph_ = g; return 0; }
  if (t) dev_tape_destroy(t);
  if (g) dev_graph_destroy(g);
  return rc2 ? rc2 : rc3;
}

int CcsdSolver::iterate_update(bool prefer_tape, bool defer_tape, bool* deferred) {
  if (deferred) *deferred = false;
  const bool use_diis = !first_ && !diis_.empty();
  const bool replayable = graphs_allowed() && replay_regime();
  double* out = (use_diis && !replayable) ? diis_[0].next_x() : ampn_.p;
  last_out_ = out; last_use_diis_ = use_diis; last_replayable_ = replayable;
  if (replayable && tape_) {
    if (defer_tape && deferred) { *deferred = true; return 0; }
    QTRY(dev_tape_run(&tape_, 1));
  } else if (replayable && graph_) {
    QTRY(dev_graph_launch(graph_));
  } else if (replayable && eager_iters_ >= 1) {
    bool began = false;
    const int rc = record_update(prefer_tape, &began);
    if (rc == 0) QTRY(prefer_tape ? dev_tape_run(&tape_, 1) : dev_graph_launch(graph_));
    else {
      graph_ok_ = false;
      if (prefer_tape && began && rc < 0) return rc;
      QTRY(update_amps(ampn_.p, ampn_.p + (int64_t)o_ * v_));
    }
  } else {
    QTRY(update_amps(out, out + (int64_t)o_ * v_));
    ++eager_iters_;
  }
  return 0;
}

int CcsdSolver::prepare_tape() {
  if (tape_ || !(graphs_allowed() && replay_regime())) return 0;
  for (int attempt = 0; attempt < 2; ++attempt) {
    if (attempt == 1) { QTRY(update_amps(ampn_.p, ampn_.p + (int64_t)o_ * v_)); ++eager_iters_; }
    bool began = false;
    const int rc = record_update(true, &began);
    if (rc == 0) return 0;
    if (!began || attempt == 1) {
      if (began && rc == QEMB_ERR_ALLOC && record_update(true, &began, false) == 0) return 0;
      graph_ok_ = false; return rc < 0 ? rc : 0;
    }
  }
  return 0;
}

int CcsdSolver::iterate_post(double* e_corr, double* normt) {
  QTRY(post_issue());
  QTRY(post_wait(1));
  QTRY(post_extrapolate(normt));
  QTRY(post_wait(2));
  return post_energy(e_corr);
}
int CcsdSolver::post_wait(int step) {
  if (!fused_post()) return dev_sync();
  if (step == 1 && last_use_diis_) return diis_[0].wait_row();
  QTRY(dev_wait_flag(step == 1 ? host_scal_ + 3 : host_scal_ + 2, step == 1 ? seq_push_ : seq_energy_));
  post_pending_ = false;
  return 0;
}
bool CcsdSolver::fused_post() const {
  return !(last_use_diis_ && diis_[0].space() > 8) && (int64_t)o_ * o_ <= 16384 && v_ <= 4096;
}
int CcsdSolver::post_issue() {
  const int64_t na = n_amp();
  double* out = last_out_;
  if (!host_scal_) { void* q = nullptr; QTRY(dev_pinned_alloc(&q, 4 * sizeof(double))); host_scal_ = (double*)q; for (int k = 0; k < 4; ++k) host_scal_[k] = 0.0; seq_push_ = seq_energy_ = 0; }
  if (!fused_post()) {
    double* err = last_use_diis_ ? diis_[0].next_e() : diff_.p;
    QTRY(lincomb2(na, 1.0, out, -1.0, amp_, err));
    if (last_use_diis_) {
      if (out != diis_[0].next_x()) QTRY(dcopy(na, out, diis_[0].next_x()));
      return diis_[0].gram_issue();
    }
    QTRY(dev_dot(na, err, err, scal_.p + 1));
    QTRY(dcopy(na, out, amp_));
    return dev_d2h_async(host_scal_ + 1, scal_.p + 1, sizeof(double));
  }
  if (last_use_diis_) return diis_[0].push_diff_issue(out, amp_);
  const double* self[1] = {diff_.p};
  post_pending_ = true;
  return dev_diis_push(na, out, amp_, diff_, amp_, 1, self, 0, scal_.p + 1, host_scal_ + 1, host_scal_ + 3, ++seq_push_);
}
int CcsdSolver::post_extrapolate(double* normt) {
  double nn = 0.0;
  first_ = false;
  if (!fused_post()) {
    if (last_use_diis_) QTRY(diis_[0].gram_finish(amp_, false, &nn));
    else nn = host_scal_[1];
    *normt = std::sqrt(nn);
    QTRY(make_tau(t1(), t2(), tau_));
    QTRY(dev_dot((int64_t)o_ * o_ * v_ * v_, Loovv_, tau_, scal_));
    return dev_d2h_async(host_scal_, scal_, sizeof(double));
  }
  double c[8] = {1.0};
  const double* xs[8] = {amp_.p};
  int m = 1;
  if (last_use_diis_) QTRY(diis_[0].coefficients(&m, c, xs, &nn));
  else nn = host_scal_[1];
  *normt = std::sqrt(nn);
  post_pending_ = true;
  return dev_ccsd_extrapolate_energy(o_, v_, m, c, xs, amp_, Loovv_, tau_, scal_, host_scal_, host_scal_ + 2, ++seq_energy_);
}
int CcsdSolver::post_energy(double* e_corr) {
  ecc_ = host_scal_[0];
  *e_corr = ecc_;
  return 0;
}

struct CcsdSolver::Convergence {
  CcsdSolver* s; CcsdOptions opt; int frag;
  double eold = 0.0, e = 0.0, normt = 0.0;
  int n_iter = 0;
  bool converged = false, active = true;
  int begin() {
    s->diis_.clear();
    if (opt.diis_space > 1) { s->diis_.emplace_back(opt.diis_space, s->n_amp()); QTRY(s->diis_[0].init()); }
    eold = e = s->ecc_;
    return 0;
  }
  int verdict(int it) {
    n_iter = it;
    if (opt.verbose > 0) {
      if (frag < 0) std::fprintf(stderr, "[qemb ccsd] cycle %3d  E(corr) = %.12f  dE = %.3e  |dt| = %.3e\n", it, e, e - eold, normt);
      else std::fprintf(stderr, "[qemb ccsd lockstep] frag %d cycle %3d  E(corr) = %.12f  dE = %.3e  |dt| = %.3e\n", frag, it, e, e - eold, normt);
    }
    if (!std::isfinite(e)) { set_error("CCSD diverged (non-finite energy)"); return QEMB_ERR_NUMERIC; }
    if (std::fabs(e - eold) < opt.conv_tol && normt < opt.conv_tol_normt) { converged = true; active = false; }
    else if (it >= opt.max_cycle) active = false;
    eold = e;
    return 0;
  }
  double end() { s->diis_.clear(); return e; }
};

int ccsd_kernel_lockstep(const std::vector<CcsdSolver*>& s, const std::vector<CcsdOptions>& opt, const std::vector<int>& ctx, int home_ctx,
                         std::vector<double>& e_corr, std::vector<int>& n_iter, std::vector<char>& converged, LockstepStats* stats) {
  const int F = (int)s.size();
  e_corr.assign(F, 0.0); n_iter.assign(F, 0); converged.assign(F, 0);
  std::vector<CcsdSolver::Convergence> c;
  struct Rebind { int home; ~Rebind() { (void)dev_ctx_bind(home); } } rebind{home_ctx};
  int max_cycle = 0;
  for (int f = 0; f < F; ++f) {
    QTRY(dev_ctx_bind(ctx[f]));
    c.push_back({s[f], opt[f], f});
    QTRY(c[f].begin());
    max_cycle = std::max(max_cycle, opt[f].max_cycle);
  }
  for (int it = 1; it <= max_cycle; ++it) {
    std::vector<dev_tape_t> tapes;
    int nactive = 0;
    for (int f = 0; f < F; ++f) {
      if (!c[f].active) continue;
      ++nactive;
      QTRY(dev_ctx_bind(ctx[f]));
      bool deferred = false;
      QTRY(s[f]->iterate_update(true, true, &deferred));
      if (deferred) tapes.push_back(s[f]->tape());
    }
    if (nactive == 0) break;
    auto now = [] { return std::chrono::duration<double, std::milli>(std::chrono::steady_clock::now().time_since_epoch()).count(); };
    const double t0 = now();
    bool batched_post = false;
    if (!tapes.empty()) {
      const int nt = (int)tapes.size();
      QTRY(dev_ctx_bind(home_ctx));
      QTRY(dev_tape_run(tapes.data(), nt));
      if (stats) {
        long long l = 0, g = 0, ops = 0;
        (void)dev_tape_last_stats(&l, &g, &ops);
        stats->launches += l; stats->grouped += g; stats->operations += ops;
        stats->max_group = std::max<long long>(stats->max_group, (long long)nt);
        stats->merged_runs += 1;
      }
      batched_post = (nt == nactive);
      for (int f = 0; f < F && batched_post; ++f) if (c[f].active && !s[f]->fused_post()) batched_post = false;
      if (!batched_post) QTRY(dev_sync());
    }
    const double t1 = now();
    if (stats) stats->ms_tapes += t1 - t0;
    static const bool trace_iters = env_int("QEMB_BATCH_TRACE", 0) >= 2;
    struct IterTrace { bool on; int it; double t0, t1; double (*now)(); ~IterTrace() { const double t = now(); if (on && t - t0 > 5.0) std::fprintf(stderr, "[qemb lockstep] iteration %d took %.2f ms: tape issue %.2f, post steps %.2f\n", it, t - t0, t1 - t0, t - t1); } } iter_trace{trace_iters, it, t0, t1, +now};
    struct PostTime { LockstepStats* st; double t1; double (*now)(); ~PostTime() { if (st) st->ms_post += now() - t1; } } post_time{stats, t1, +now};
    if (batched_post) {
      struct Flush { bool open = false; ~Flush() { if (open) (void)dev_batch_flush(); } } guard;
      QTRY(dev_ctx_bind(home_ctx));
      QTRY(dev_batch_begin()); guard.open = true;
      for (int f = 0; f < F; ++f) if (c[f].active) QTRY(s[f]->post_issue());
      guard.open = false; QTRY(dev_batch_flush());
      QTRY(dev_batch_begin()); guard.open = true;
      for (int f = 0; f < F; ++f) if (c[f].active) { QTRY(s[f]->post_wait(1)); QTRY(s[f]->post_extrapolate(&c[f].normt)); }
      guard.open = false; QTRY(dev_batch_flush());
    } else {
      for (int f = 0; f < F; ++f) if (c[f].active) { QTRY(dev_ctx_bind(ctx[f])); QTRY(s[f]->post_issue()); }
      for (int f = 0; f < F; ++f) if (c[f].active) { QTRY(dev_ctx_bind(ctx[f])); QTRY(s[f]->post_wait(1)); QTRY(s[f]->post_extrapolate(&c[f].normt)); }
    }
    for (int f = 0; f < F; ++f) {
      if (!c[f].active) continue;
      if (!batched_post) QTRY(dev_ctx_bind(ctx[f]));
      QTRY(s[f]->post_wait(2));
      QTRY(s[f]->post_energy(&c[f].e));
      QTRY(c[f].verdict(it));
    }
  }
  for (int f = 0; f < F; ++f) { e_corr[f] = c[f].end(); n_iter[f] = c[f].n_iter; converged[f] = c[f].converged ? 1 : 0; }
  return 0;
}

int CcsdSolver::kernel(const CcsdOptions& opt, double* e_corr, int* n_iter, bool* converged) {
  Convergence c{this, opt, -1};
  *converged = false;
  QTRY(c.begin());
  for (int it = 1; c.active && it <= opt.max_cycle; ++it) {
    QTRY(iterate(&c.e, &c.normt));
    QTRY(c.verdict(it));
  }
  *e_corr = c.end();
  *n_iter = c.n_iter;
  *converged = c.converged;
  return 0;
}

int CcsdSolver::export_block(const char* name, double* host, int64_t nelem) {
  const std::string nm(name ? name : "");
  const DBuf* b = nullptr;
  if (nm == "oooo") b = &I_.oooo; else if (nm == "ovoo") b = &I_.ovoo; else if (nm == "ovov") b = &I_.ovov;
  else if (nm == "ovvv") b = &I_.ovvv; else if (nm == "Vl") b = &I_.Vl; else if (nm == "Vp") b = &I_.Vp; else if (nm == "Vm") b = &I_.Vm; else if (nm == "W1base") b = &W1base_;
  else if (nm == "W2base") b = &W2base_; else if (nm == "eo") b = &eo_; else if (nm == "ev") b = &ev_;
  if (!b || !b->p) { set_error("export_block: unknown block name"); return QEMB_ERR_ARG; }
  if (nelem != b->n) { set_error("export_block: element count mismatch"); return QEMB_ERR_ARG; }
  return dev_d2h(host, b->p, sizeof(double) * nelem);
}

int CcsdSolver::energy_intermediates(std::vector<double>& Z1, std::vector<double>& Z2) {
  const int64_t o = o_, v = v_, nf = nf_, N2 = o * o * v * v;
  Z1.assign((size_t)(o * nf), 0.0); Z2.assign((size_t)(v * nf), 0.0);
  if (nf <= 0) return 0;
  QTRY(make_tau(t1(), t2(), tau_));
  QTRY(perm4(S_, tau_, o, o, v, v, 0, 2, 1, 3, 2.0, 0.0));
  QTRY(perm4(S_, tau_, o, o, v, v, 1, 2, 0, 3, -1.0, 1.0));
  DBuf z1, z2, a2p;
  QTRY(z1.alloc(o * nf)); QTRY(z2.alloc(v * nf)); QTRY(a2p.alloc(o * o * v * nf));
  QTRY(gemm_nn(o, nf, v * o * v, 1.0, S_, I_.A1, 0.0, z1));
  QTRY(perm4(a2p, I_.A2, o, o, v, nf, 1, 2, 0, 3));
  QTRY(gemm_tn(v, nf, o * v * o, 1.0, S_, a2p, 0.0, z2));
  QTRY(dev_d2h(Z1.data(), z1, sizeof(double) * o * nf));
  QTRY(dev_d2h(Z2.data(), z2, sizeof(double) * v * nf));
  (void)N2;
  return 0;
}

}
```

quemb_amd/csrc/ccsd.h:

```cpp
#pragma once
#include <cstdint>
#include <vector>
#include "dev_ops.h"
#include "tensor_utils.h"

namespace qemb {

struct CcsdOptions {
  double conv_tol = 1e-10;
  double conv_tol_normt = 1e-8;
  int max_cycle = 100;
  int diis_space = 6;
  int verbose = 0;
};

struct MoIntegrals {
  int n = 0, o = 0, v = 0, nf = 0;
  DBuf oooo, ovoo, ovov, oovv, ovvo, ovvv;
  DBuf ovvv_pk;
  DBuf Vl;
  DBuf Vp, Vm;
  int64_t ldp = 0, ldm = 0;
  DBuf A1, A2;
  DBuf T34;
};

int mo_slab_ld(int n);
int64_t mo_transform_work(int n);
int mo_transform(int n, int o, int nf, const double* eri_s4, double* X0, double* X1, const double* C, MoIntegrals& out,
                 bool build_Vl = false, bool build_T34 = false, bool x1_is_unpacked = false);
int mo_transform_factor(int n, int o, int nf, int naux, const double* B_packed, double* X0, double* X1, const double* C, MoIntegrals& out,
                        bool build_Vl = false, bool build_T34 = false);
inline bool mo_factor_route_pays(int n, int naux) { return naux > 0 && (int64_t)naux <= 8 * (int64_t)n; }

struct CcsdGemmPlans { GemmPlan fvv, pa, pb, ladder_p, ladder_m, xw_p, xw_m, x_p, x_m; };
CcsdGemmPlans ccsd_gemm_plans(int64_t o, int64_t v);
bool ccsd_use_ring_prep(int64_t o, int64_t v, bool replay);
struct CcsdRingPlan { int cfg = -1, ks = 0; int64_t region_ws_bytes = 0; };
CcsdRingPlan ccsd_ring_plan(int64_t o, int64_t v);

class CcLambda;

struct LockstepStats { long long merged_runs = 0, launches = 0, grouped = 0, operations = 0, max_group = 0; double ms_tapes = 0.0, ms_post = 0.0; };
class CcsdSolver;
int ccsd_kernel_lockstep(const std::vector<CcsdSolver*>& s, const std::vector<CcsdOptions>& opt, const std::vector<int>& ctx, int home_ctx,
                         std::vector<double>& e_corr, std::vector<int>& n_iter, std::vector<char>& converged, LockstepStats* stats);

class CcsdSolver {
  friend class CcLambda;
 public:
  int setup(MoIntegrals&& ints, const double* mo_energy_dev);
  int init_amps();
  int set_amps(const double* t1_dev, const double* t2_dev);
  int iterate(double* e_corr, double* normt);
  int iterate_update(bool prefer_tape, bool defer_tape, bool* deferred);
  int iterate_post(double* e_corr, double* normt);
  bool fused_post() const;
  int post_wait(int step);
  int post_issue();
  int post_extrapolate(double* normt);
  int post_energy(double* e_corr);
  int prepare_tape();
  struct Convergence;
  int kernel(const CcsdOptions& opt, double* e_corr, int* n_iter, bool* converged);
  int energy_intermediates(std::vector<double>& Z1, std::vector<double>& Z2);
  int export_block(const char* name, double* host, int64_t nelem);
  int apply_ladder(const double* x, double* out, bool rows_packed = false, bool hh = false);
  const MoIntegrals& integrals() const { return I_; }
  double* t1() { return amp_.p; }
  double* t2() { return amp_.p + (int64_t)o_ * v_; }
  int o() const { return o_; }
  int v() const { return v_; }
  int64_t n_amp() const { return (int64_t)o_ * v_ + (int64_t)o_ * o_ * v_ * v_; }

 private:
  int update_amps(double* t1n, double* t2n);
  bool replay_regime() const;
  int record_update(bool as_tape, bool* began, bool regions = true);
  int energy(const double* t1, const double* t2, double* e);
  int make_tau(const double* t1, const double* t2, double* tau);

  int o_ = 0, v_ = 0, nf_ = 0;
  MoIntegrals I_;
  DBuf eo_, ev_;
  DBuf ovov_t_, Lovov_, Loovv_, OVoovv_, Lovoo_, ovoo_ijka_, ovoo_kilc_, W1base_, W2base_, Lph1_, OVp_, OVm_, oooo_p_, ovoo_cikl_;
  DBuf amp_, ampn_, diff_;
  DBuf tau_, T_, Tp_, S_, W1_, W2_, W12_, W12b_, R_, U_, G2_, T1P_;
  bool ovvv_pass_ = false;
  int ovvv_G_ = 0;
  DBuf LovooK_;
  bool ring_prep_ = false;
  DBuf ovoo_kicl_;
  DBuf LTp_, LTm_, LRp_, LRm_;
  DBuf Xp_, Xm_;
  DBuf ovvv_pk_, ZCp_;
  DBuf Gp_, Gm_;
  DBuf Xwp_, Xwm_, Xw_;
  DBuf WAp_, WAm_, HRp_, HRm_;
  int64_t lwp_ = 0, lwm_ = 0;
  DBuf ZB_, ZC_;
  CcsdGemmPlans plans_;
  DBuf Foo_, Fvv_, Fov_, Z_, Y_, Ytmp_, Loo_, Lvv_, Q_, Wo_, O1_, X_, scal_, LovooT_;
  std::vector<DeviceDIIS> diis_;
  bool first_ = true;
  dev_graph_t graph_ = nullptr;
  dev_tape_t tape_ = nullptr;
  int eager_iters_ = 0;
  bool graph_ok_ = true;
  double* last_out_ = nullptr;
  double* host_scal_ = nullptr;
  unsigned long long seq_push_ = 0, seq_energy_ = 0;
  bool post_pending_ = false;
  bool last_use_diis_ = false, last_replayable_ = false;
 public:
  ~CcsdSolver() {
    if (graph_) dev_graph_destroy(graph_);
    if (tape_) dev_tape_destroy(tape_);
    if (host_scal_) { if (post_pending_) (void)dev_sync_device(); dev_pinned_free(host_scal_); }
  }
  CcsdSolver() = default;
  dev_tape_t release_tape() { dev_tape_t t = tape_; tape_ = nullptr; return t; }
  void adopt_tape(dev_tape_t t) { if (tape_) dev_tape_destroy(tape_); tape_ = t; }
  dev_tape_t tape() const { return tape_; }
  CcsdSolver(const CcsdSolver&) = delete;
  CcsdSolver& operator=(const CcsdSolver&) = delete;
 private:
  double ecc_ = 0.0;
};

GemmPlan pick_pair_gemm(int64_t rows, int64_t cols, int64_t K = 0, bool k_aware = false);
}
```

quemb_amd/csrc/dev_ops.h:

```cpp
#pragma once
#include <cstddef>
#include <cstdint>
#include <string>
#include "../../include/qemb_hip_ops.h"
#include "gemm_tiles.h"
#include "env.h"

namespace qemb {

void set_error(const std::string& msg);
const char* last_error();

#define QTRY(expr)              \
  do {                          \
    int _rc = (expr);           \
    if (_rc != 0) return _rc;   \
  } while (0)


int dev_init(int device);
int dev_sync();
int dev_sync_device();
int dev_ctx_count(int n);
int dev_ctx_bind(int k);
// ... 161 lines not shown
int dev_ladder_scatter_pm(int64_t o, int64_t v, const double* Rp, int64_t ldp, const double* Rm, int64_t ldm, double* t2);
int dev_ladder_scatter_pm2(int64_t o, int64_t v, const double* Rp, int64_t ldp, const double* Rm, int64_t ldm, const double* Hp, const double* Hm,
                           int assign, double* t2, int Sp = 1, int64_t strideP = 0, int Sm = 1, int64_t strideM = 0, int64_t ldhp = 0, int64_t ldhm = 0);
int dev_pack_w_pm(int64_t o, const double* W, double* Ap, int64_t lda_p, double* Am, int64_t lda_m);
int dev_pack_w_pm_sum(int64_t o, const double* Wt, const double* X, const double* At, double* Ap, int64_t lda_p, double* Am, int64_t lda_m);
int dev_ccsd_t1_assemble(int64_t o, int64_t v, const double* t1, const double* Lvv, const double* Loo, const double* Fov, const double* S, const double* Lph1,
                         const double* PA, int SA, int64_t strideA, const double* PB, int SB, int64_t strideB, double* t1n);
int dev_gemv_rows_two(int64_t rows1, int64_t cols1, const double* T1, int64_t ld1, const double* x1, double* y1, double a1, double b1,
                      int64_t rows2, int64_t cols2, const double* T2, int64_t ld2, const double* x2, double* y2, double a2, double b2);
int dev_foo_from_x(int64_t o, const double* X, double* F);
int dev_ccsd_ph_layouts(int64_t o, int64_t v, const double* t2, const double* t1, double* T, double* Tp, double* S, double* Ut, double* Tpt, double* Th);
int dev_ccsd_ph_layouts_ring(int64_t o, int64_t v, const double* t2, const double* t1, double* Tp, double* S, double* Ut, double* Tpt);
constexpr int CCSD_OVVV_MAX_TILES = 48;
constexpr int CCSD_OVVV_MAX_ROWT = 18;
inline bool ccsd_ovvv_shape_ok(int64_t o, int64_t v) {
  if (o < 1 || v < 1 || o > 32) return false;
  const int64_t rt = (v + 15) / 16, nt = (2 * o + 15) / 16;
  return rt * nt <= CCSD_OVVV_MAX_TILES && rt + nt <= CCSD_OVVV_MAX_ROWT;
}
int dev_ccsd_ovvv_slabs(int64_t o, int64_t v);
int dev_ccsd_ovvv_pass(int64_t o, int64_t v, const double* ovvv, const double* t1, const double* Thk, double* ZB, double* PA);
constexpr int CCSD_RING_PREP_MAX_O = 32;
inline bool ccsd_ring_prep_shape_ok(int64_t o, int64_t v) { return o >= 1 && o <= CCSD_RING_PREP_MAX_O && v >= 1 && v <= 4096; }
int dev_ccsd_ring_prep(int64_t o, int64_t v, const double* t1, const double* P1, const double* W1base, const double* W2base, const double* ZB, const double* ZC,
                       const double* OB, const double* OC, double* R, double* W2);
int dev_ccsd_u_update(int64_t o, int64_t v, const double* A, const double* t1, const double* Z, double* U);
int dev_small_k_update(int64_t batch, int64_t M, int64_t N, int64_t K, double alpha, const double* A, int64_t sA, const double* B, int64_t sB,
                       double* C, int64_t sC);
int dev_ccsd_y_traces(int64_t o, int64_t v, const double* ZC, const double* ZB, double* Y, const double* add = nullptr, int S = 1, int64_t stride = 0, double scale = 1.0);

inline int64_t dev_mp2_partial_count(int64_t o, int64_t v) {
  const int64_t nt = (v + 31) / 32, oo = o * o;
  return nt * (nt + 1) / 2 * (oo < 4096 ? oo : 4096);
}
int dev_mp2_amplitudes(int64_t o, int64_t v, const double* ovov, const double* eo, const double* ev, double* t2, double* G, double* partials, double* e_dev);

inline int rdm2_check_args(int kind, int64_t o, int64_t v, const double* t1, const double* t2, const double* out) {
  if (kind != QEMB_RDM2_CCSD && kind != QEMB_RDM2_MP2) { set_error("dev_rdm2_assemble: kind must be QEMB_RDM2_CCSD or QEMB_RDM2_MP2"); return QEMB_ERR_ARG; }
  if (o <= 0 || v < 0 || !out || (v > 0 && (!t2 || (kind == QEMB_RDM2_CCSD && !t1)))) { set_error("dev_rdm2_assemble: bad arguments"); return QEMB_ERR_ARG; }
  if (o + v > 32767) { set_error("dev_rdm2_assemble: n = " + std::to_string(o + v) + " is beyond any n^4 tensor"); return QEMB_ERR_ARG; }
  return 0;
}
int dev_rdm2_assemble(int kind, int64_t o, int64_t v, const double* t1, const double* t2, const double* dm1c, double* out);
inline int64_t rdm2_full_grid(int64_t m) { return m * m < 4096 ? m * m : 4096; }
inline int rdm2_check_full(int64_t m, const void* a, const void* b) {
  if (m <= 0 || m > 32767 || !a || !b) { set_error("rdm2 full-basis pass: bad arguments (N = " + std::to_string(m) + ")"); return QEMB_ERR_ARG; }
  return 0;
}
int dev_rdm2_add_nc(int64_t m, const double* g, double alpha, double* X);
int dev_rdm2_symmetrize(int64_t m, const double* g, double* X);
int dev_rdm2_eri_dot(int64_t m, int sym, const double* eri, const double* K, double* partials, double* out_dev);

constexpr int kFciMaxOrb = 16;
constexpr int64_t kFciMaxDet = (int64_t)12870 * 12870;
inline int fci_check_args(const char* who, int n, int64_t ns, int nlink, const void* a, const void* b, const void* c) {
  if (n <= 0 || n > kFciMaxOrb || ns <= 0 || ns > 12870 || nlink <= 0 || nlink > kFciMaxOrb * kFciMaxOrb || !a || !b || !c) {
    set_error(std::string(who) + ": bad arguments (n = " + std::to_string(n) + ", strings = " + std::to_string(ns) + ")");
    return QEMB_ERR_ARG;
  }
  return 0;
}
inline int fci_check_slab(const char* who, int64_t ns, int64_t a0, int64_t a1) {
  if (a0 < 0 || a1 <= a0 || a1 > ns) { set_error(std::string(who) + ": bad slab [" + std::to_string(a0) + ", " + std::to_string(a1) + ") of " + std::to_string(ns) + " alpha rows"); return QEMB_ERR_ARG; }
  return 0;
}
int dev_fci_gather_slab(int n, int64_t ns, int nlink, const int32_t* links, const double* c, int64_t a0, int64_t a1, double* Ds);
int dev_fci_sigma_slab(int n, int64_t ns, int nlink, const int32_t* links, const double* k, int64_t a0, int64_t a1, const double* Ds, const double* Gs, double* sigma);
int dev_fci_diag(int n, int64_t ns, const int32_t* strings, const double* h, const double* V, double* hdiag);
int dev_fci_precond(int64_t N, const double* r, const double* hdiag, double theta, double* out);
int dev_fci_dm2(int n, int o_cum, const double* A, const double* dm1, double* out);

constexpr int kSciMaxOrb = 64;
constexpr int kSciScreenLanes = 256;
int dev_sci_screen_count(int n, const double* h, const double* V, int64_t nd, const uint64_t* keys, const double* c, double eps, double dbl_bound, int32_t* counts);
int dev_sci_screen_emit(int n, const double* h, const double* V, int64_t nd, const uint64_t* keys, const double* c, double eps, double dbl_bound, const int64_t* offsets, uint64_t* out,
                        uint64_t alpha_lo = 0, uint64_t alpha_hi = ~(uint64_t)0);
int dev_sci_pt2_rows(int n, const double* h, const double* V, int64_t N, const uint64_t* keys, const double* c, int64_t nseg, const int64_t* seg, int64_t K, const uint64_t* ext,
                     double e_var, double eps, double dbl_bound, double* contrib);
int dev_sci_sum(int64_t m, const double* in, double* out);
int dev_sci_scan(int64_t m, const int32_t* in, int64_t* out);
int dev_sci_sort(int64_t m, int64_t mpad, uint64_t* keys);
int dev_sci_flag_new(int64_t m, const uint64_t* cand, int64_t nA, const uint64_t* A, int64_t nB, const uint64_t* B, int32_t* flags);
int dev_sci_compact(int64_t m, const uint64_t* cand, const int32_t* flags, const int64_t* offsets, uint64_t* out);
int dev_sci_merge(int64_t nA, const uint64_t* A, const double* cA, int64_t nB, const uint64_t* B, uint64_t* out, double* cout);
int dev_sci_csr_count(int64_t N, const uint64_t* keys, int64_t nseg, const int64_t* seg, int32_t* counts);
int dev_sci_csr_fill(int n, const double* h, const double* V, int64_t N, const uint64_t* keys, int64_t nseg, const int64_t* seg, const int64_t* rowptr, int32_t* col, double* val, double* hdiag);
int dev_sci_spmv(int64_t N, const int64_t* rowptr, const int32_t* col, const double* val, const double* x, double* y);
int dev_sci_rdm(int n, int64_t N, const uint64_t* keys, const int64_t* rowptr, const int32_t* col, const double* c, double* dm1, double* dm2);
int dev_sci_dm2_finish(int n, int o_cum, const double* dm1, double* dm2);

struct CcsdTArgs;
int dev_ccsd_t_assemble(const CcsdTArgs& A);
int dev_ccsd_t_sum(int64_t m, const double* in, double* out, int64_t slot);
int dev_ccsd_t_total(int64_t m, const double* in, double* out);

inline int64_t kdf_ld(int64_t nao) { return (nao + 15) / 16 * 16; }
int dev_kdf_split(int64_t rows, int64_t nao, const double* z, double* planes);
int dev_kdf_stack(int64_t nk, int64_t nao, int64_t n, const double* ta, double* Cs, double* Dk);
inline int64_t dev_kdf_partial_count(int64_t naux, int64_t n) {
  const int64_t nt = (n + 31) / 32;
  return 2 * (nt * (nt + 1) / 2) * (naux < 1024 ? naux : 1024);
}
inline int kdf_check_pack(int64_t naux, int64_t n, const void* M, const void* F, int64_t ldf, const void* partials, const void* out2) {
  if (naux <= 0 || n <= 0 || n > 32767 || !M || !F || !partials || !out2 || ldf < n * (n + 1) / 2) { set_error("dev_kdf_pack: bad arguments"); return QEMB_ERR_ARG; }
  return 0;
}
int dev_kdf_pack(int64_t naux, int64_t n, const double* M, int paired, double w, double* F, int64_t ldf, double* partials, double* out2_dev);

int dev_boys(int m_max, int64_t n, const double* x, double* out);
namespace int3c { struct ClassArgs; }
int dev_int3c_class(int la, int lb, int lp, const int3c::ClassArgs& args);

namespace int1e { struct Args; }
int dev_int1e_class(int la, int lb, const int1e::Args& args);

namespace int4c { struct PairArgs; struct ClassArgs; }
int dev_int4c_pairs(int la, int lb, const int4c::PairArgs& args);
int dev_int4c_class(int la, int lb, int lc, int ld, const int4c::ClassArgs& args);
namespace int4c { struct JkArgs; }
namespace int3c { struct Shell; }
int dev_int4c_jk_class(int la, int lb, int lc, int ld, const int4c::JkArgs& args);
int dev_int4c_dmax(const int3c::Shell* sh, int nshell, int64_t N, const double* dm, double* out);
namespace int4c { struct PairProdArgs; }
int dev_int4c_pairprod(const int4c::PairProdArgs& args);
int dev_int4c_add_transpose(int64_t m, double* A);

int dev_cd_gather_cols(int64_t rows, int64_t ncols, const double* in, int64_t ldi, const int32_t* idx, double* out, int64_t ldo);
int dev_joint_diag(int64_t K, int64_t m, double* Q, double* U, double stop_angle, int max_sweeps, int* sweeps, double* f, int* converged);
int dev_cd_panel_factor(const double* E, int64_t ld, const int32_t* srow, int n, double thr, const double* d, double* T, int32_t* piv, int32_t* rank, double* work);
int dev_cd_new_rows(int64_t np, int n, int r, const double* E, int64_t ld, const double* T, const int32_t* piv, double* Lnew, int64_t ldl);
int dev_cd_diag_update(int64_t np, int r, const double* Lnew, int64_t ldl, const int32_t* piv, const int32_t* srow, double* d, int64_t nsp, const int32_t* row0, const int32_t* cnt,
                       double* spmax, double* partials, double* dmax);
int dev_cd_unpack(int64_t M, int64_t N, const double* L, int64_t ld, const int32_t* pos, double* out);

int dev_threshold_mask(int64_t n, const double* x, double eps, double* out);
int dev_mul_bcast_rows(int64_t rows, int64_t cols, double* x, const double* m);

int dev_abs_overlap_prim(int nsh, const int* l, const double* ex, const double* xyz, const int64_t* cart0, int64_t ncart, int nroots,
                         const double* roots, const double* weights, double* out);

int dev_gather_rows(int64_t nrows, int64_t len, const int64_t* idx_dev, const double* src, int64_t ld, double* dst);
int dev_scale_rows(int64_t nrows, int64_t len, double* x, const double* s);

int dev_dot(int64_t n, const double* x, const double* y, double* out_dev);
int dev_absmax(int64_t n, const double* x, double* out_dev);
int dev_dot_many(int64_t n, const double* x, int m, const double* const* ys, double* out_dev);
int dev_diis_push(int64_t n, const double* trial, const double* prev, double* e, double* xcopy, int m, const double* const* ys, int self,
                  double* row_dev, double* row_host, void* flag_host = nullptr, unsigned long long seq = 0);
int dev_batch_begin();
int dev_batch_flush();
int dev_wait_flag(const void* flag_host, unsigned long long seq);
int dev_ccsd_extrapolate_energy(int64_t o, int64_t v, int nterms, const double* coef, const double* const* xs, double* amp, const double* L,
                                double* tau, double* e_dev, double* e_host, void* flag_host = nullptr, unsigned long long seq = 0);

int dev_gemv_rows(int64_t rows, int64_t cols, const double* T, int64_t ldt, const double* x,
                  double* y, double alpha, double beta);
int dev_gemv_rows_batched(int64_t rows, int64_t cols, int64_t nbatch, const double* T, int64_t ldt, int64_t strideT,
                          const double* x, int64_t stridex, double* y, double alpha, double beta);
int dev_contract_mid(int64_t outer, int64_t mid, int64_t inner, const double* T, const double* x,
                     double* Y, int64_t ldy, double alpha, double beta);

int dev_unpack_s4(int64_t n, const double* s4, double* s1);
int dev_pack_s4(int64_t n, const double* s1, double* s4);
int dev_unpack_s8_to_s4(int64_t n, const double* s8, double* s4);
int dev_unpack_tril_rows(int64_t rows, int64_t n, const double* packed, double* full);
int dev_unpack_tril_rows_ld(int64_t rows, int64_t n, int64_t ld, const double* packed, double* full);
int dev_pack_tril_rows(int64_t rows, int64_t n, const double* full, double* packed);
int dev_unpack_tril_pair_rows(int64_t nr, int64_t n, const double* in, double* full);
int dev_unpack_tril_pair_rows_ld(int64_t nr, int64_t n, int64_t ld, const double* in, double* full);

int dev_jacobi_eigh(int64_t n, double* A, double* w, double* V, int* sweeps_out);
int dev_jacobi_eigh_until(int64_t n, double* A, double* w, double* V, int* sweeps_out, double stop_below);
enum { JACOBI_STATUS_NOCONV = -1, JACOBI_STATUS_NONFINITE = -2 };
inline int jacobi_status_code(int st, const char* who) {
  if (st == JACOBI_STATUS_NONFINITE) { set_error(std::string(who) + ": the matrix holds a NaN or an infinity"); return QEMB_ERR_NUMERIC; }
  if (st < 0) { set_error(std::string(who) + ": Jacobi sweeps did not converge in 40 sweeps"); return QEMB_ERR_NOCONV; }
  return QEMB_OK;
}
int dev_scf_fused_max();
int dev_jacobi_eigh_in_basis(int64_t n, const double* F, const double* Cp, double* w, double* C_out, double* C2_out, int nocc, double* dm_out, double stop_below,
                             int* status_dev);
int dev_scf_fock_small(int64_t n, const double* h, const double* J, const double* K, const double* D, double* F, double* err, double* scal2);
int dev_pack_density_sym(int64_t n, const double* D, double* Dp);
int dev_jacobi_svd(int64_t m, int64_t n, double* G, double* s, double* U, double* V, int* sweeps_out);

enum { COMM_ID_BYTES = 128, COMM_SUM = 0, COMM_MAX = 1 };
int dev_comm_unique_id(void* id128);
int dev_comm_init(int rank, int world, const void* id128);
int dev_comm_info(int* rank, int* world);
int dev_comm_allreduce(double* host_buf, int64_t n, int op);
int dev_comm_destroy();

int dev_cholesky_lower(int64_t n, double* A);
int dev_tri_inverse_lower(int64_t n, const double* L, double* Linv);

}
```

quemb_amd/csrc/tensor_utils.h:

```cpp
#pragma once
#include <algorithm>
#include <cmath>
#include <cstdint>
#include <cstring>
#include <string>
#include <vector>
#include "dev_ops.h"

namespace qemb {

struct DBuf {
  double* p = nullptr;
  int64_t n = 0;
  DBuf() = default;
  DBuf(const DBuf&) = delete;
  DBuf& operator=(const DBuf&) = delete;
  DBuf(DBuf&& o) noexcept : p(o.p), n(o.n) { o.p = nullptr; o.n = 0; }
  DBuf& operator=(DBuf&& o) noexcept { if (this != &o) { release(); p = o.p; n = o.n; o.p = nullptr; o.n = 0; } return *this; }
  ~DBuf() { release(); }
  int alloc(int64_t nelem) {
    release();
    void* q = nullptr;
    int rc = dev_alloc(&q, (size_t)(nelem > 0 ? nelem : 1) * sizeof(double));
    if (rc) return rc;
    p = (double*)q; n = nelem;
    return 0;
  }
  void release() { if (p) { dev_free(p); p = nullptr; n = 0; } }
  operator double*() const { return p; }
};

inline int axpby(int64_t n, double alpha, const double* x, double beta, double* y) {
  const int64_t C = 1 << 20;
  int64_t done = 0;
  while (done < n) {
    const int64_t left = n - done;
    Copy4Desc c{};
    if (left >= C) {
      int64_t rows = left / C;
      if (rows > (1 << 10)) rows = 1 << 10;
      c.dim[0] = 1; c.dim[1] = 1; c.dim[2] = rows; c.dim[3] = C;
    } else {
      c.dim[0] = 1; c.dim[1] = 1; c.dim[2] = 1; c.dim[3] = left;
    }
    c.in = x + done; c.out = y + done;
    c.si[0] = c.si[1] = 0; c.si[2] = c.dim[3]; c.si[3] = 1;
    c.so[0] = c.so[1] = 0; c.so[2] = c.dim[3]; c.so[3] = 1;
    c.alpha = alpha; c.beta = beta;
    QTRY(dev_copy4(c));
    done += c.dim[2] * c.dim[3];
  }
  return 0;
}
inline int dcopy(int64_t n, const double* x, double* y) { return axpby(n, 1.0, x, 0.0, y); }
inline int lincomb2(int64_t n, double a, const double* x, double b, const double* y, double* out) {
  const double c[2] = {a, b};
  const double* xs[2] = {x, y};
  return dev_lincomb(n, 2, c, xs, 0.0, out);
}

inline int perm4(double* dst, const double* src, int64_t d0, int64_t d1, int64_t d2, int64_t d3, int p0, int p1, int p2,
                 int p3, double alpha = 1.0, double beta = 0.0, const double* base = nullptr) {
  const int64_t d[4] = {d0, d1, d2, d3};
  const int perm[4] = {p0, p1, p2, p3};
  int64_t od[4], ostr[4];
  for (int k = 0; k < 4; ++k) od[k] = d[perm[k]];
  ostr[3] = 1; ostr[2] = od[3]; ostr[1] = od[3] * od[2]; ostr[0] = od[3] * od[2] * od[1];
  Copy4Desc c{};
  c.in = src; c.out = dst; c.alpha = alpha; c.beta = beta;
  c.si[3] = 1; c.si[2] = d[3]; c.si[1] = d[3] * d[2]; c.si[0] = d[3] * d[2] * d[1];
  for (int k = 0; k < 4; ++k) { c.dim[k] = d[k]; }
  for (int k = 0; k < 4; ++k) c.so[perm[k]] = ostr[k];
  c.base = base;
  return dev_copy4(c);
}

inline int extract4(double* dst, const double* src, int64_t n1, int64_t n2, int64_t n3, int64_t o0, int64_t o1, int64_t o2,
                    int64_t o3, int64_t s0, int64_t s1, int64_t s2, int64_t s3) {
  Copy4Desc c{};
  c.dim[0] = s0; c.dim[1] = s1; c.dim[2] = s2; c.dim[3] = s3;
  c.si[3] = 1; c.si[2] = n3; c.si[1] = n3 * n2; c.si[0] = n3 * n2 * n1;
  c.in = src + o0 * c.si[0] + o1 * c.si[1] + o2 * c.si[2] + o3;
  c.so[3] = 1; c.so[2] = s3; c.so[1] = s3 * s2; c.so[0] = s3 * s2 * s1;
  c.out = dst; c.alpha = 1.0; c.beta = 0.0;
  return dev_copy4(c);
}

inline int gemm(int64_t M, int64_t N, int64_t K, double alpha, const double* A, int64_t lda, bool a_kc, const double* B,
                int64_t ldb, bool b_kc, double beta, double* C, int64_t ldc, int64_t batch = 1, int64_t sA = 0,
                int64_t sB = 0, int64_t sC = 0, int cfg = -1, int ksplit = 0) {
  GemmDesc g{};
  g.M = M; g.N = N; g.K = K; g.alpha = alpha; g.beta = beta;
  g.A = A; g.lda = lda; g.a_kcontig = a_kc ? 1 : 0; g.strideA = sA;
  g.B = B; g.ldb = ldb; g.b_kcontig = b_kc ? 1 : 0; g.strideB = sB;
  g.C = C; g.ldc = ldc; g.strideC = sC; g.batch = batch; g.cfg = cfg; g.ksplit = ksplit;
  return dev_gemm(g);
}
inline int gemm_nn(int64_t M, int64_t N, int64_t K, double al, const double* A, const double* B, double be, double* C) {
  return gemm(M, N, K, al, A, K, true, B, N, false, be, C, N);
}
inline int gemm_nt(int64_t M, int64_t N, int64_t K, double al, const double* A, const double* B, double be, double* C) {
  return gemm(M, N, K, al, A, K, true, B, K, true, be, C, N);
}
inline int gemm_tn(int64_t M, int64_t N, int64_t K, double al, const double* A, const double* B, double be, double* C) {
  return gemm(M, N, K, al, A, M, false, B, N, false, be, C, N);
}

inline int gemm_quarter_lower_rows(int n, int64_t inner, int64_t K, const double* C, const double* In, double* Out) {
  const int64_t ncol = (int64_t)n * inner;
  if (!fits_one_224_tile(n)) return gemm(n, ncol, K, 1.0, C, n, false, In, K, true, 0.0, Out, ncol);
  static const int tiles[] = {GEMM_224x128, GEMM_192x128, GEMM_128x256, GEMM_112x128, GEMM_64x128_COL};
  int s0 = 0;
  for (int t = 0; t < 5 && s0 < n; ++t) {
    const int s1 = (t + 1 < 5) ? std::min(n, std::max(s0, n - gemm_tile_rows(tiles[t + 1]))) : n;
    if (s1 > s0) {
      const int rc = gemm(n - s0, (int64_t)(s1 - s0) * inner, K, 1.0, C + s0, n, false, In + (int64_t)s0 * inner * K, K, true, 0.0,
                          Out + (int64_t)s0 * ncol + (int64_t)s0 * inner, ncol, 1, 0, 0, 0, tiles[t]);
      if (rc) return rc;
    }
    s0 = s1;
  }
  return 0;
}

inline bool solve_dense(int n, std::vector<double>& A, std::vector<double>& b) {
  for (int k = 0; k < n; ++k) {
    int piv = k; double best = std::fabs(A[k * n + k]);
    for (int i = k + 1; i < n; ++i) if (std::fabs(A[i * n + k]) > best) { best = std::fabs(A[i * n + k]); piv = i; }
    if (best < 1e-300) return false;
    if (piv != k) { for (int j = 0; j < n; ++j) std::swap(A[k * n + j], A[piv * n + j]); std::swap(b[k], b[piv]); }
    for (int i = k + 1; i < n; ++i) {
      const double f = A[i * n + k] / A[k * n + k];
      if (f == 0.0) continue;
      for (int j = k; j < n; ++j) A[i * n + j] -= f * A[k * n + j];
      b[i] -= f * b[k];
    }
  }
  for (int k = n - 1; k >= 0; --k) {
    double s = b[k];
    for (int j = k + 1; j < n; ++j) s -= A[k * n + j] * b[j];
    b[k] = s / A[k * n + k];
  }
  return true;
}

class DeviceDIIS {
 public:
  DeviceDIIS(int space, int64_t n) : space_(space), n_(n) {}
  int init() {
    xs_.resize(space_); es_.resize(space_);
    for (int i = 0; i < space_; ++i) { QTRY(xs_[i].alloc(n_)); QTRY(es_[i].alloc(n_)); }
    QTRY(scal_.alloc(space_ + 1));
    B_.assign((size_t)space_ * space_, 0.0);
    return 0;
  }
  int size() const { return count_ < space_ ? count_ : space_; }
  int extrapolate(double* x, const double* e) {
    QTRY(dcopy(n_, x, next_x()));
    QTRY(dcopy(n_, e, next_e()));
    return extrapolate_pushed(x, true);
  }
  double* next_x() { return xs_[count_ % space_]; }
  double* next_e() { return es_[count_ % space_]; }
  int extrapolate_pushed(double* x, bool x_holds_trial = false, double* err_dot = nullptr) {
    QTRY(gram_issue());
    QTRY(dev_sync());
    return gram_finish(x, x_holds_trial, err_dot);
  }
  int gram_issue() {
    const int slot = count_ % space_;
    ++count_;
    const int m = size();
    QTRY(ensure_row_host());
    flagged_ = false;
    for (int j0 = 0; j0 < m; j0 += 8) {
      const int cnt = std::min(8, m - j0);
      const double* ps[8];
      for (int q = 0; q < cnt; ++q) ps[q] = es_[j0 + q].p;
      QTRY(dev_dot_many(n_, es_[slot], cnt, ps, scal_.p + j0));
    }
    QTRY(dev_d2h_async(row_host_, scal_.p, sizeof(double) * m));
    pending_slot_ = slot;
    return 0;
  }
  int push_diff_issue(const double* trial, const double* prev) {
    const int slot = count_ % space_;
    if (space_ > 8) {
      QTRY(lincomb2(n_, 1.0, trial, -1.0, prev, es_[slot]));
      if (trial != xs_[slot].p) QTRY(dcopy(n_, trial, xs_[slot]));
      return gram_issue();
    }
    ++count_;
    const int m = size();
    QTRY(ensure_row_host());
    const double* ps[8];
    for (int q = 0; q < m; ++q) ps[q] = es_[q].p;
    QTRY(dev_diis_push(n_, trial, prev, es_[slot], trial == xs_[slot].p ? nullptr : xs_[slot].p, m, ps, slot, scal_.p, row_host_, row_host_ + space_ + 1, ++seq_));
    pending_slot_ = slot; flagged_ = true;
    return 0;
  }
  int wait_row() {
    if (flagged_) { flagged_ = false; return dev_wait_flag(row_host_ + space_ + 1, seq_); }
    return dev_sync();
  }
  int coefficients(int* nterms, double* c, const double** xs, double* err_dot = nullptr) {
    const int slot = pending_slot_;
    *nterms = 1; c[0] = 1.0; xs[0] = xs_[slot].p;
    const int m = size();
    const double* row = row_host_;
    for (int j = 0; j < m; ++j) { B_[(size_t)slot * space_ + j] = row[j]; B_[(size_t)j * space_ + slot] = row[j]; }
    if (err_dot) *err_dot = row[slot];
    if (m < 2) return 0;
    std::vector<double> A((size_t)(m + 1) * (m + 1), 0.0), rhs(m + 1, 0.0);
    double scale = 0.0;
    for (int i = 0; i < m; ++i) scale = std::fmax(scale, B_[(size_t)i * space_ + i]);
    if (scale <= 0.0) return 0;
    for (int i = 0; i < m; ++i) {
      for (int j = 0; j < m; ++j) A[(size_t)(i + 1) * (m + 1) + (j + 1)] = B_[(size_t)i * space_ + j] / scale;
      A[i + 1] = 1.0; A[(size_t)(i + 1) * (m + 1)] = 1.0;
    }
    rhs[0] = 1.0;
    if (!solve_dense(m + 1, A, rhs)) return 0;
    for (int i = 0; i < m; ++i) if (!std::isfinite(rhs[i + 1])) return 0;
    *nterms = m;
    for (int i = 0; i < m; ++i) { c[i] = rhs[i + 1]; xs[i] = xs_[i].p; }
    return 0;
  }
  int gram_finish(double* x, bool x_holds_trial = false, double* err_dot = nullptr) {
    std::vector<double> c((size_t)space_);
    std::vector<const double*> ps((size_t)space_);
    int m = 0;
    QTRY(coefficients(&m, c.data(), ps.data(), err_dot));
    if (m == 1) return x_holds_trial ? 0 : dcopy(n_, ps[0], x);
    for (int i0 = 0; i0 < m; i0 += 8)
      QTRY(dev_lincomb(n_, std::min(8, m - i0), c.data() + i0, ps.data() + i0, i0 == 0 ? 0.0 : 1.0, x));
    return 0;
  }
  int space() const { return space_; }
  void reset() { count_ = 0; }

 private:
  int space_; int64_t n_; int count_ = 0;
  std::vector<DBuf> xs_, es_;
  DBuf scal_;
  std::vector<double> B_;
  double* row_host_ = nullptr;
  unsigned long long seq_ = 0;
  bool flagged_ = false;
  int pending_slot_ = 0;
  int ensure_row_host() {
    if (row_host_) return 0;
    void* q = nullptr;
    QTRY(dev_pinned_alloc(&q, sizeof(double) * (space_ + 2)));
    row_host_ = (double*)q;
    for (int i = 0; i < space_ + 2; ++i) row_host_[i] = 0.0;
    seq_ = 0;
    return 0;
  }
 public:
  ~DeviceDIIS() { if (row_host_) { if (flagged_) (void)dev_sync_device(); dev_pinned_free(row_host_); } }
  DeviceDIIS(DeviceDIIS&& o) noexcept : space_(o.space_), n_(o.n_), count_(o.count_), xs_(std::move(o.xs_)), es_(std::move(o.es_)), scal_(std::move(o.scal_)),
                                        B_(std::move(o.B_)), row_host_(o.row_host_), seq_(o.seq_), flagged_(o.flagged_), pending_slot_(o.pending_slot_) { o.row_host_ = nullptr; }
  DeviceDIIS(const DeviceDIIS&) = delete;
  DeviceDIIS& operator=(const DeviceDIIS&) = delete;
  DeviceDIIS& operator=(DeviceDIIS&&) = delete;
};

}
```

Baseline: 59.43.

## Store DIIS t2 amplitudes in packed i>=j pair layout to halve DIIS traffic

Adds a pair-packed layout for the DIIS history of t2 amplitudes. Only i>=j occupied pairs are kept, and off-diagonal pairs get weight two in the error dot products. The ladder scatter and the ring/denominator finish write straight into this packed layout. A new extrapolation kernel rebuilds the full t2 and tau while it computes the energy. The aim is to cut the memory footprint and bandwidth of the DIIS push, Gram and extrapolation steps, at the cost of new kernels, index unpairing math, and disabling graph replay when the path is on.

```diff
diff --git a/include/qemb_hip_ops.h b/include/qemb_hip_ops.h
--- a/include/qemb_hip_ops.h
+++ b/include/qemb_hip_ops.h
@@ -94,6 +94,12 @@
 int qemb_op_ccsd_finish_t2_rings(int64_t o, int64_t v, double* t2n, const double* U, const double* OV, const double* RS, const double* M, const double* eo, const double* ev, double* t1n);
 int qemb_op_diis_push(int64_t n, const double* trial, const double* prev, double* e, double* xcopy, int m, const double* const* ys, int self, double* row_dev, double* row_host);
 int qemb_op_ccsd_extrapolate_energy(int64_t o, int64_t v, int nterms, const double* coef, const double* const* xs, double* amp, const double* L, double* tau, double* e_host);
+int qemb_op_ccsd_pair_diis_rule(int64_t o, int64_t v, int replay);
+int qemb_op_ladder_scatter_pm_pairs(int64_t o, int64_t v, const double* Rp, int64_t ldp, const double* Rm, int64_t ldm, const double* Hp, const double* Hm,
+                                    int assign, double* t2p);
+int qemb_op_ccsd_finish_t2_rings_pairs(int64_t o, int64_t v, double* t2p, const double* U, const double* OV, const double* RS, const double* M, const double* eo, const double* ev, double* t1n);
+int qemb_op_diis_push_pairs(int64_t o, int64_t v, const double* trial, const double* prev, double* e, int m, const double* const* ys, int self, double* row_dev, double* row_host);
+int qemb_op_ccsd_extrapolate_energy_pairs(int64_t o, int64_t v, int nterms, const double* coef, const double* const* xs, double* amp, const double* L, double* tau, double* e_host);
 int qemb_op_gather_rows(int64_t nrows, int64_t len, const int64_t* idx_dev, const double* src, int64_t ld, double* dst);
 int qemb_op_scale_rows(int64_t nrows, int64_t len, double* x, const double* s);
 int qemb_op_pack_pair_rows(int64_t n, int64_t ncols, const double* in, double* out);
diff --git a/quemb_amd/_lib.py b/quemb_amd/_lib.py
--- a/quemb_amd/_lib.py
+++ b/quemb_amd/_lib.py
@@ -133,6 +133,11 @@
     f("qemb_op_ccsd_finish_t2_rings", I, L, L, P, P, P, P, P, P, P, P)
     f("qemb_op_diis_push", I, L, P, P, P, P, I, P, I, P, P)
     f("qemb_op_ccsd_extrapolate_energy", I, L, L, I, P, P, P, P, P, P)
+    f("qemb_op_ccsd_pair_diis_rule", I, L, L, I)
+    f("qemb_op_ladder_scatter_pm_pairs", I, L, L, P, L, P, L, P, P, I, P)
+    f("qemb_op_ccsd_finish_t2_rings_pairs", I, L, L, P, P, P, P, P, P, P, P)
+    f("qemb_op_diis_push_pairs", I, L, L, P, P, P, I, P, I, P, P)
+    f("qemb_op_ccsd_extrapolate_energy_pairs", I, L, L, I, P, P, P, P, P, P)
     f("qemb_op_gather_rows", I, L, L, P, P, L, P)
     f("qemb_op_scale_rows", I, L, L, P, P)
     f("qemb_ctx_count", I, I)
diff --git a/quemb_amd/csrc/api.cpp b/quemb_amd/csrc/api.cpp
--- a/quemb_amd/csrc/api.cpp
+++ b/quemb_amd/csrc/api.cpp
@@ -287,6 +287,32 @@
   dev_pinned_free(pin);
   return rc;
 }
+int qemb_op_ccsd_pair_diis_rule(int64_t o, int64_t v, int replay) { return ccsd_use_pair_diis(o, v, CcsdOptions().diis_space, replay != 0) ? 1 : 0; }
+int qemb_op_ladder_scatter_pm_pairs(int64_t o, int64_t v, const double* Rp, int64_t ldp, const double* Rm, int64_t ldm, const double* Hp, const double* Hm,
+                                    int assign, double* t2p) { return dev_ladder_scatter_pm_pairs(o, v, Rp, ldp, Rm, ldm, Hp, Hm, assign, t2p); }
+int qemb_op_ccsd_finish_t2_rings_pairs(int64_t o, int64_t v, double* t2p, const double* U, const double* OV, const double* RS, const double* M, const double* eo, const double* ev, double* t1n) {
+  return dev_ccsd_finish_t2_rings_pairs(o, v, t2p, U, OV, RS, M, eo, ev, t1n);
+}
+int qemb_op_diis_push_pairs(int64_t o, int64_t v, const double* trial, const double* prev, double* e, int m, const double* const* ys, int self, double* row_dev, double* row_host) {
+  void* pin = nullptr;
+  QTRY(dev_pinned_alloc(&pin, sizeof(double) * 8));
+  int rc = dev_diis_push_pairs(o, v, trial, prev, e, m, ys, self, row_dev, (double*)pin);
+  if (!rc) rc = dev_sync();
+  if (!rc) for (int j = 0; j < m; ++j) row_host[j] = ((double*)pin)[j];
+  dev_pinned_free(pin);
+  return rc;
+}
+int qemb_op_ccsd_extrapolate_energy_pairs(int64_t o, int64_t v, int nterms, const double* coef, const double* const* xs, double* amp, const double* L, double* tau, double* e_host) {
+  void* pin = nullptr;
+  DBuf e_dev;
+  QTRY(e_dev.alloc(1));
+  QTRY(dev_pinned_alloc(&pin, sizeof(double) * 8));
+  int rc = dev_ccsd_extrapolate_energy_pairs(o, v, nterms, coef, xs, amp, L, tau, e_dev, (double*)pin);
+  if (!rc) rc = dev_sync();
+  if (!rc) *e_host = *(double*)pin;
+  dev_pinned_free(pin);
+  return rc;
+}
 int qemb_op_ccsd_y_traces(int64_t o, int64_t v, const double* ZC, const double* ZB, double* Y) { return dev_ccsd_y_traces(o, v, ZC, ZB, Y); }
 int qemb_op_gather_rows(int64_t nrows, int64_t len, const int64_t* idx_dev, const double* src, int64_t ld, double* dst) { return dev_gather_rows(nrows, len, idx_dev, src, ld, dst); }
 int qemb_op_scale_rows(int64_t nrows, int64_t len, double* x, const double* s) { return dev_scale_rows(nrows, len, x, s); }
diff --git a/quemb_amd/csrc/ccsd.cpp b/quemb_amd/csrc/ccsd.cpp
--- a/quemb_amd/csrc/ccsd.cpp
+++ b/quemb_amd/csrc/ccsd.cpp
@@ -351,6 +351,11 @@
   if (sw == 0 || !ccsd_ring_prep_shape_ok(o, v)) return false;
   return sw > 0 || !replay;
 }
+bool ccsd_use_pair_diis(int64_t o, int64_t v, int diis_space, bool replay) {
+  const long long sw = env_int("QEMB_PAIR_DIIS", -1);
+  if (sw == 0 || diis_space < 2 || diis_space > 8 || !ccsd_pair_diis_shape_ok(o, v)) return false;
+  return sw > 0 || !replay;
+}
 
 CcsdGemmPlans ccsd_gemm_plans(int64_t o, int64_t v) {
   int64_t ldp, ldm;
@@ -379,7 +384,7 @@
   if (S > 1) r.region_ws_bytes = 2 * (((int64_t)sizeof(double) * S * nov * nov + 255) / 256 * 256);
   return r;
 }
-int CcsdSolver::apply_ladder(const double* x, double* out, bool rows_packed, bool hh) {
+int CcsdSolver::apply_ladder(const double* x, double* out, bool rows_packed, bool hh, bool pairs) {
   const int64_t o = o_, v = v_;
   {
     const int64_t npo = o * (o + 1) / 2, nmo = o * (o - 1) / 2, npv = v * (v + 1) / 2, nmv = v * (v - 1) / 2;
@@ -403,15 +408,18 @@
       QTRY(dev_region_chain());
       if (nmo > 0 && nmv > 0) QTRY(gemm(nmo, nmv, nmo, 1.0, WAm_, lwm_, true, LTm_, ldm, false, 0.0, HRm_, ldm, 1, 0, 0, 0, nmv >= 2048 ? tile_for(nmo) : -1));
       QTRY(dev_region_end());
-      QTRY(dev_ladder_scatter_pm2(o, v, LRp_, sp.ld, LRm_, sm.ld, HRp_, (nmo > 0 && nmv > 0) ? HRm_.p : nullptr, 1, out, sp.S, sp.stride, sm.S, sm.stride, ldp, ldm));
+      const double* hrm = (nmo > 0 && nmv > 0) ? HRm_.p : nullptr;
+      if (pairs) QTRY(dev_ladder_scatter_pm_pairs(o, v, LRp_, sp.ld, LRm_, sm.ld, HRp_, hrm, 1, out, sp.S, sp.stride, sm.S, sm.stride, ldp, ldm));
+      else QTRY(dev_ladder_scatter_pm2(o, v, LRp_, sp.ld, LRm_, sm.ld, HRp_, hrm, 1, out, sp.S, sp.stride, sm.S, sm.stride, ldp, ldm));
     } else {
-      QTRY(dev_ladder_scatter_pm2(o, v, LRp_, sp.ld, LRm_, sm.ld, nullptr, nullptr, 0, out, sp.S, sp.stride, sm.S, sm.stride));
-    }
-  }
-  return 0;
-}
-
-int CcsdSolver::update_amps(double* t1n, double* t2n) {
+      if (pairs) QTRY(dev_ladder_scatter_pm_pairs(o, v, LRp_, sp.ld, LRm_, sm.ld, nullptr, nullptr, 0, out, sp.S, sp.stride, sm.S, sm.stride));
+      else QTRY(dev_ladder_scatter_pm2(o, v, LRp_, sp.ld, LRm_, sm.ld, nullptr, nullptr, 0, out, sp.S, sp.stride, sm.S, sm.stride));
+    }
+  }
+  return 0;
+}
+
+int CcsdSolver::update_amps(double* t1n, double* t2n, bool pairs) {
   const int64_t o = o_, v = v_, nov = o * v, oo = o * o, vv = v * v;
   const double* t1 = this->t1();
   const double* t2 = this->t2();
@@ -474,7 +482,7 @@
 
   QTRY(gemm(o, oo * o, v, 1.0, t1, v, true, ovoo_cikl_, oo * o, false, 0.0, O1_, oo * o));
   QTRY(dev_pack_w_pm_sum(o, oooo_p_, Xw_, O1_, WAp_, lwp_, WAm_, lwm_));
-  QTRY(apply_ladder(tau_, t2n, true, true));
+  QTRY(apply_ladder(tau_, t2n, true, true, pairs));
 
   QTRY(gemm(oo * v, v, v, 1.0, t2, v, true, Lvv_, v, true, 0.0, U_, v));
   QTRY(gemm(o, o * vv, o, -1.0, Loo_, o, false, t2, o * vv, false, 1.0, U_, o * vv, 1, 0, 0, 0, cfg_wide));
@@ -536,7 +544,8 @@
   QTRY(dev_region_end());
   QTRY(lap_RINGS.close());
 
-  QTRY(dev_ccsd_finish_t2_rings(o, v, t2n, U_, OVoovv_, W12_, W1_, eo_, ev_, t1n));
+  if (pairs) QTRY(dev_ccsd_finish_t2_rings_pairs(o, v, t2n, U_, OVoovv_, W12_, W1_, eo_, ev_, t1n));
+  else QTRY(dev_ccsd_finish_t2_rings(o, v, t2n, U_, OVoovv_, W12_, W1_, eo_, ev_, t1n));
   return 0;
 }
 
@@ -552,7 +561,8 @@
   static const bool on = env_flag("QEMB_GRAPH", !profiled_run());
   return on;
 }
-bool CcsdSolver::replay_regime() const { return (int64_t)o_ * o_ * v_ * v_ <= (int64_t)1 << 22 && graph_ok_; }
+static bool replay_size(int64_t o, int64_t v) { return o * o * v * v <= (int64_t)1 << 22; }
+bool CcsdSolver::replay_regime() const { return replay_size(o_, v_) && graph_ok_; }
 
 int CcsdSolver::record_update(bool as_tape, bool* began, bool regions) {
   *began = false;
@@ -572,7 +582,7 @@
 int CcsdSolver::iterate_update(bool prefer_tape, bool defer_tape, bool* deferred) {
   if (deferred) *deferred = false;
   const bool use_diis = !first_ && !diis_.empty();
-  const bool replayable = graphs_allowed() && replay_regime();
+  const bool replayable = graphs_allowed() && replay_regime() && !pair_diis_;
   double* out = (use_diis && !replayable) ? diis_[0].next_x() : ampn_.p;
   last_out_ = out; last_use_diis_ = use_diis; last_replayable_ = replayable;
   if (replayable && tape_) {
@@ -590,7 +600,7 @@
       QTRY(update_amps(ampn_.p, ampn_.p + (int64_t)o_ * v_));
     }
   } else {
-    QTRY(update_amps(out, out + (int64_t)o_ * v_));
+    QTRY(update_amps(out, out + (int64_t)o_ * v_, use_diis && pair_diis_));
     ++eager_iters_;
   }
   return 0;
@@ -666,6 +676,7 @@
   else nn = host_scal_[1];
   *normt = std::sqrt(nn);
   post_pending_ = true;
+  if (last_use_diis_ && pair_diis_) return dev_ccsd_extrapolate_energy_pairs(o_, v_, m, c, xs, amp_, Loovv_, tau_, scal_, host_scal_, host_scal_ + 2, ++seq_energy_);
   return dev_ccsd_extrapolate_energy(o_, v_, m, c, xs, amp_, Loovv_, tau_, scal_, host_scal_, host_scal_ + 2, ++seq_energy_);
 }
 int CcsdSolver::post_energy(double* e_corr) {
@@ -681,7 +692,12 @@
   bool converged = false, active = true;
   int begin() {
     s->diis_.clear();
-    if (opt.diis_space > 1) { s->diis_.emplace_back(opt.diis_space, s->n_amp()); QTRY(s->diis_[0].init()); }
+    s->pair_diis_ = ccsd_use_pair_diis(s->o_, s->v_, opt.diis_space, replay_size(s->o_, s->v_));
+    if (opt.diis_space > 1) {
+      if (s->pair_diis_) s->diis_.emplace_back(opt.diis_space, s->n_amp(), s->o_, s->v_);
+      else s->diis_.emplace_back(opt.diis_space, s->n_amp());
+      QTRY(s->diis_[0].init());
+    }
     eold = e = s->ecc_;
     return 0;
   }
diff --git a/quemb_amd/csrc/ccsd.h b/quemb_amd/csrc/ccsd.h
--- a/quemb_amd/csrc/ccsd.h
+++ b/quemb_amd/csrc/ccsd.h
@@ -36,6 +36,7 @@
 struct CcsdGemmPlans { GemmPlan fvv, pa, pb, ladder_p, ladder_m, xw_p, xw_m, x_p, x_m; };
 CcsdGemmPlans ccsd_gemm_plans(int64_t o, int64_t v);
 bool ccsd_use_ring_prep(int64_t o, int64_t v, bool replay);
+bool ccsd_use_pair_diis(int64_t o, int64_t v, int diis_space, bool replay);
 struct CcsdRingPlan { int cfg = -1, ks = 0; int64_t region_ws_bytes = 0; };
 CcsdRingPlan ccsd_ring_plan(int64_t o, int64_t v);
 
@@ -65,7 +66,7 @@
   int kernel(const CcsdOptions& opt, double* e_corr, int* n_iter, bool* converged);
   int energy_intermediates(std::vector<double>& Z1, std::vector<double>& Z2);
   int export_block(const char* name, double* host, int64_t nelem);
-  int apply_ladder(const double* x, double* out, bool rows_packed = false, bool hh = false);
+  int apply_ladder(const double* x, double* out, bool rows_packed = false, bool hh = false, bool pairs = false);
   const MoIntegrals& integrals() const { return I_; }
   double* t1() { return amp_.p; }
   double* t2() { return amp_.p + (int64_t)o_ * v_; }
@@ -74,7 +75,7 @@
   int64_t n_amp() const { return (int64_t)o_ * v_ + (int64_t)o_ * o_ * v_ * v_; }
 
  private:
-  int update_amps(double* t1n, double* t2n);
+  int update_amps(double* t1n, double* t2n, bool pairs = false);
   bool replay_regime() const;
   int record_update(bool as_tape, bool* began, bool regions = true);
   int energy(const double* t1, const double* t2, double* e);
@@ -90,6 +91,7 @@
   int ovvv_G_ = 0;
   DBuf LovooK_;
   bool ring_prep_ = false;
+  bool pair_diis_ = false;
   DBuf ovoo_kicl_;
   DBuf LTp_, LTm_, LRp_, LRm_;
   DBuf Xp_, Xm_;
diff --git a/quemb_amd/csrc/ccsd_pair_diis_ops.hip b/quemb_amd/csrc/ccsd_pair_diis_ops.hip
--- /dev/null
+++ b/quemb_amd/csrc/ccsd_pair_diis_ops.hip
@@ -0,0 +1,344 @@
+#include <algorithm>
+#include <cstdint>
+#include "hip_common.h"
+
+namespace qemb {
+namespace pair_diis {
+
+constexpr int NPART = 2048;
+
+__device__ __forceinline__ void unpair_ge(long long p, long long& x, long long& y) {
+  x = (long long)((sqrt(8.0 * (double)p + 1.0) - 1.0) * 0.5);
+  while (x * (x + 1) / 2 > p) --x;
+  while ((x + 1) * (x + 2) / 2 <= p) ++x;
+  y = p - x * (x + 1) / 2;
+}
+__device__ __forceinline__ double slab_sum(const double* __restrict__ p, int S, long long stride) {
+  switch (S) {
+    case 1: return p[0];
+    case 2: { const double a = p[0], b = p[stride]; return a + b; }
+    case 3: { const double a = p[0], b = p[stride], c = p[2 * stride]; return (a + b) + c; }
+    case 4: { const double a = p[0], b = p[stride], c = p[2 * stride], d = p[3 * stride]; return ((a + b) + c) + d; }
+    default: {
+      double acc = 0.0;
+      int sl = 0;
+      for (; sl + 4 <= S; sl += 4) { const double a = p[sl * stride], b = p[(sl + 1) * stride], c = p[(sl + 2) * stride], d = p[(sl + 3) * stride]; acc = (((acc + a) + b) + c) + d; }
+      for (; sl < S; ++sl) acc += p[sl * stride];
+      return acc;
+    }
+  }
+}
+__device__ __forceinline__ double block_sum(double v, double* sh) {
+  const int lane = threadIdx.x & 63, w = threadIdx.x >> 6, nw = blockDim.x >> 6;
+#pragma unroll
+  for (int off = 32; off > 0; off >>= 1) v += __shfl_down(v, off, 64);
+  if (lane == 0) sh[w] = v;
+  __syncthreads();
+  double r = 0.0;
+  if (threadIdx.x == 0) { r = sh[0]; for (int k = 1; k < nw; ++k) r += sh[k]; }
+  __syncthreads();
+  return r;
+}
+__global__ void __launch_bounds__(256) pair_finish_partials_kernel(int m, int np, const double* __restrict__ partial, double* out_dev, double* out_host,
+                                                                   unsigned long long* flag_host, unsigned long long seq) {
+  __shared__ double sh[4];
+  double acc[8];
+#pragma unroll
+  for (int j = 0; j < 8; ++j) {
+    acc[j] = 0.0;
+    if (j < m) for (int i = threadIdx.x; i < np; i += blockDim.x) acc[j] += partial[(long long)j * np + i];
+  }
+#pragma unroll
+  for (int j = 0; j < 8; ++j) {
+    if (j >= m) break;
+    const double r = block_sum(acc[j], sh);
+    if (threadIdx.x == 0) { out_dev[j] = r; out_host[j] = r; }
+  }
+  if (threadIdx.x == 0 && flag_host) {
+    __threadfence_system();
+    __hip_atomic_store(flag_host, seq, __ATOMIC_RELEASE, __HIP_MEMORY_SCOPE_SYSTEM);
+  }
+}
+
+__global__ void __launch_bounds__(256) ladder_scatter_pm_pairs_kernel(long long o, long long v, const double* __restrict__ Rp, long long ldp,
+                                                                      const double* __restrict__ Rm, long long ldm, double* __restrict__ t2p,
+                                                                      const double* __restrict__ Hp, const double* __restrict__ Hm, int assign,
+                                                                      int Sp, long long strideP, int Sm, long long strideM, long long ldhp, long long ldhm) {
+  __shared__ double sp[32][33], sm[32][33];
+  const uint3 LB = xcd_logical_block(block_id(), grid_dim());
+  const long long ij = LB.y;
+  long long i, j; unpair_ge(ij, i, j);
+  long long t = LB.x, ta, tb; unpair_ge(t, ta, tb);
+  const int tx = threadIdx.x & 31, ty = threadIdx.x >> 5;
+  const double* rp = Rp + ij * ldp;
+  const double* rm = (i > j) ? Rm + (i * (i - 1) / 2 + j) * ldm : nullptr;
+  const double* hp = Hp ? Hp + ij * ldhp : nullptr;
+  const double* hm = (Hm && i > j) ? Hm + (i * (i - 1) / 2 + j) * ldhm : nullptr;
+  double* tij = t2p + ij * v * v;
+#pragma unroll
+  for (int k = 0; k < 4; ++k) {
+    const int aa = ty + 8 * k;
+    const long long a = ta * 32 + aa, b = tb * 32 + tx;
+    double p = 0.0, m = 0.0;
+    if (a < v && b <= a) {
+      p = slab_sum(rp + a * (a + 1) / 2 + b, Sp, strideP);
+      if (hp) p += (a == b ? 2.0 : 1.0) * hp[a * (a + 1) / 2 + b];
+      if (rm && b < a) { m = slab_sum(rm + a * (a - 1) / 2 + b, Sm, strideM); if (hm) m += hm[a * (a - 1) / 2 + b]; }
+    }
+    sp[aa][tx] = p; sm[aa][tx] = m;
+  }
+  __syncthreads();
+#pragma unroll
+  for (int k = 0; k < 4; ++k) {
+    const int aa = ty + 8 * k;
+    {
+      const long long a = ta * 32 + aa, b = tb * 32 + tx;
+      if (a < v && b <= a) {
+        const double p = sp[aa][tx], m = sm[aa][tx];
+        if (assign) tij[a * v + b] = p + m;
+        else tij[a * v + b] += p + m;
+      }
+    }
+    {
+      const long long r = tb * 32 + aa, c = ta * 32 + tx;
+      if (c < v && r < c) {
+        const double p = sp[tx][aa], m = sm[tx][aa];
+        if (assign) tij[r * v + c] = p - m;
+        else tij[r * v + c] += p - m;
+      }
+    }
+  }
+}
+
+__global__ void __launch_bounds__(256) ccsd_finish_t2_rings_pairs_kernel(long long o, long long v, double* __restrict__ t2p, const double* __restrict__ U,
+                                                                         const double* __restrict__ OV, const double* __restrict__ RS, const double* __restrict__ M,
+                                                                         const double* __restrict__ eo, const double* __restrict__ ev, double* __restrict__ t1n) {
+  __shared__ double tile[32][33];
+  const uint3 LB = xcd_logical_block(block_id(), grid_dim());
+  long long i, j; unpair_ge((long long)LB.y, i, j);
+  const long long nt = (v + 31) / 32;
+  const long long ta = LB.x / nt, tb = LB.x - ta * nt;
+  const int tx = threadIdx.x & 31, ty = threadIdx.x >> 5;
+  const long long vv = v * v, ov = o * v;
+  const double* Uij = U + (i * o + j) * vv;
+  const double* Uji = U + (j * o + i) * vv;
+  const double* RSij = RS + i * v * ov + j * v;
+  const double* RSji = RS + j * v * ov + i * v;
+  const double* Mij = M + i * v * ov + j * v;
+  const double* Mji = M + j * v * ov + i * v;
+#pragma unroll
+  for (int k = 0; k < 4; ++k) {
+    const int bb = ty + 8 * k;
+    const long long b = tb * 32 + bb, a = ta * 32 + tx;
+    tile[bb][tx] = (a < v && b < v) ? ((Uji[b * v + a] + RSji[b * ov + a]) - 0.5 * Mji[b * ov + a]) - Mij[b * ov + a] : 0.0;
+  }
+  __syncthreads();
+  const double eij = eo[i] + eo[j];
+#pragma unroll
+  for (int k = 0; k < 4; ++k) {
+    const int aa = ty + 8 * k;
+    const long long a = ta * 32 + aa, b = tb * 32 + tx;
+    if (a < v && b < v) {
+      const long long idx = (i * o + j) * vv + a * v + b, pk = (long long)LB.y * vv + a * v + b;
+      const double straight = ((Uij[a * v + b] + RSij[a * ov + b]) - 0.5 * Mij[a * ov + b]) - Mji[a * ov + b];
+      t2p[pk] = (t2p[pk] + OV[idx] + straight + tile[tx][aa]) / (eij - ev[a] - ev[b]);
+    }
+  }
+  if (t1n && LB.x == 0 && LB.y == 0)
+    for (long long t = threadIdx.x; t < ov; t += blockDim.x) t1n[t] /= eo[t / v] - ev[t % v];
+}
+
+struct PushK { const double* y[8]; int m, self; };
+template <bool VEC2>
+__global__ void __launch_bounds__(256) diis_push_pairs_kernel(int o, int v, const double* __restrict__ trial, const double* __restrict__ prev, double* __restrict__ e,
+                                                              PushK k, double* __restrict__ partial) {
+  __shared__ double sh[4];
+  constexpr int W = VEC2 ? 2 : 1;
+  const long long vv = (long long)v * v, nov = (long long)o * v;
+  const int nseg = o * (o + 1) / 2 + 1;
+  double acc[8];
+#pragma unroll
+  for (int j = 0; j < 8; ++j) acc[j] = 0.0;
+  for (int s = (int)blockIdx.y; s < nseg; s += (int)gridDim.y) {
+    long long offp = 0, offf = 0, len = nov;
+    double wgt = 1.0;
+    if (s > 0) {
+      long long i, j; unpair_ge((long long)(s - 1), i, j);
+      offp = nov + (long long)(s - 1) * vv; offf = nov + (i * o + j) * vv; len = vv;
+      wgt = (i == j) ? 1.0 : 2.0;
+    }
+    const long long nw = len / W;
+    for (long long x = (long long)blockIdx.x * blockDim.x + threadIdx.x; x < nw; x += (long long)gridDim.x * blockDim.x) {
+      const long long xp = offp / W + x, xf = offf / W + x;
+      double t[W], p[W], y[8][W];
+      if (VEC2) {
+        const double2 tt = reinterpret_cast<const double2*>(trial)[xp], pp = reinterpret_cast<const double2*>(prev)[xf];
+        t[0] = tt.x; t[W - 1] = tt.y; p[0] = pp.x; p[W - 1] = pp.y;
+#pragma unroll
+        for (int j = 0; j < 8; ++j) { y[j][0] = 0.0; y[j][W - 1] = 0.0; if (j < k.m && j != k.self) { const double2 yy = reinterpret_cast<const double2*>(k.y[j])[xp]; y[j][0] = yy.x; y[j][W - 1] = yy.y; } }
+      } else {
+        t[0] = trial[xp]; p[0] = prev[xf];
+#pragma unroll
+        for (int j = 0; j < 8; ++j) { y[j][0] = 0.0; if (j < k.m && j != k.self) y[j][0] = k.y[j][xp]; }
+      }
+      double ei[W], we[W];
+#pragma unroll
+      for (int w = 0; w < W; ++w) { ei[w] = t[w] - p[w]; we[w] = wgt * ei[w]; }
+      if (VEC2) reinterpret_cast<double2*>(e)[xp] = make_double2(ei[0], ei[W - 1]);
+      else e[xp] = ei[0];
+#pragma unroll
+      for (int j = 0; j < 8; ++j) if (j < k.m) {
+#pragma unroll
+        for (int w = 0; w < W; ++w) acc[j] += we[w] * (j == k.self ? ei[w] : y[j][w]);
+      }
+    }
+  }
+  const int np = (int)(gridDim.x * gridDim.y), me = (int)(blockIdx.y * gridDim.x + blockIdx.x);
+#pragma unroll
+  for (int j = 0; j < 8; ++j) {
+    if (j >= k.m) break;
+    const double r = block_sum(acc[j], sh);
+    if (threadIdx.x == 0) partial[(long long)j * np + me] = r;
+  }
+}
+
+struct ExtrapK { const double* x[8]; double c[8]; int n; };
+__global__ void __launch_bounds__(256) ccsd_extrapolate_energy_pairs_kernel(int o, int v, ExtrapK k, double* __restrict__ amp, const double* __restrict__ L,
+                                                                            double* __restrict__ tau, double* __restrict__ partial) {
+  __shared__ double tval[32][33];
+  __shared__ double ti[32], tj[32];
+  __shared__ double sh[4];
+  const uint3 LB = xcd_logical_block(block_id(), grid_dim());
+  long long il, jl; unpair_ge((long long)LB.y, il, jl);
+  const int i = (int)il, j = (int)jl;
+  const int nt = (v + 31) / 32;
+  const int tx = threadIdx.x & 31, ty = threadIdx.x >> 5;
+  const long long vv = (long long)v * v, nov = (long long)o * v;
+  const long long offp = nov + (long long)LB.y * vv, offij = ((long long)i * o + j) * vv, offji = ((long long)j * o + i) * vv;
+  double acc = 0.0;
+  for (int tl = (int)LB.x; tl < nt * nt; tl += (int)gridDim.x) {
+    const int ta = tl / nt, tb = tl - ta * nt;
+    if (threadIdx.x < 64) {
+      const bool is_j = threadIdx.x >= 32;
+      const int col = (is_j ? tb : ta) * 32 + tx;
+      if (col < v) {
+        const long long src = (long long)(is_j ? j : i) * v + col;
+        double sacc = 0.0;
+#pragma unroll
+        for (int q = 0; q < 8; ++q) if (q < k.n) sacc += k.c[q] * k.x[q][src];
+        if (is_j) { tj[tx] = sacc; if (i == j && ta == 0) amp[src] = sacc; }
+        else ti[tx] = sacc;
+      }
+    }
+    __syncthreads();
+#pragma unroll
+    for (int r = 0; r < 4; ++r) {
+      const int aa = ty + 8 * r;
+      const int a = ta * 32 + aa, b = tb * 32 + tx;
+      double val = 0.0;
+      if (a < v && b < v) {
+        const long long pos = (long long)a * v + b;
+        double xv[8];
+#pragma unroll
+        for (int q = 0; q < 8; ++q) if (q < k.n) xv[q] = k.x[q][offp + pos];
+        const double lv = L[offij + pos];
+#pragma unroll
+        for (int q = 0; q < 8; ++q) if (q < k.n) val += k.c[q] * xv[q];
+        const double tv = fma(ti[aa], tj[tx], val);
+        acc += lv * tv;
+        amp[nov + offij + pos] = val;
+        tau[offij + pos] = tv;
+      }
+      tval[aa][tx] = val;
+    }
+    if (i != j) {
+      __syncthreads();
+#pragma unroll
+      for (int r = 0; r < 4; ++r) {
+        const int bb = ty + 8 * r;
+        const int b = tb * 32 + bb, a = ta * 32 + tx;
+        if (a < v && b < v) {
+          const long long pos = offji + (long long)b * v + a;
+          const double val = tval[tx][bb];
+          amp[nov + pos] = val;
+          tau[pos] = fma(ti[tx], tj[bb], val);
+        }
+      }
+    }
+    __syncthreads();
+  }
+  const double r = block_sum((i == j) ? acc : 2.0 * acc, sh);
+  if (threadIdx.x == 0) partial[(long long)LB.y * gridDim.x + LB.x] = r;
+}
+
+static bool al16(const void* q) { return (reinterpret_cast<uintptr_t>(q) & 15) == 0; }
+
+}
+using namespace pair_diis;
+
+#define PAIR_REQUIRE(who)                                                                                              \
+  hipStream_t st = hip_stream();                                                                                       \
+  if (!st) { set_error("libqemb_hip: call qemb_init(device) first"); return QEMB_ERR_DEVICE; }                         \
+  if (!ccsd_pair_diis_shape_ok(o, v)) { set_error(who ": shape outside the rule (ccsd_pair_diis_shape_ok)"); return QEMB_ERR_ARG; }
+
+int dev_ladder_scatter_pm_pairs(int64_t o, int64_t v, const double* Rp, int64_t ldp, const double* Rm, int64_t ldm, const double* Hp, const double* Hm,
+                                int assign, double* t2p, int Sp, int64_t strideP, int Sm, int64_t strideM, int64_t ldhp, int64_t ldhm) {
+  PAIR_REQUIRE("dev_ladder_scatter_pm_pairs")
+  if (!Rp || !t2p || (o > 1 && v > 1 && !Rm)) { set_error("dev_ladder_scatter_pm_pairs: bad arguments"); return QEMB_ERR_ARG; }
+  const long long npo = o * (o + 1) / 2, nt = (v + 31) / 32;
+  return launch("dev_ladder_scatter_pm_pairs", ladder_scatter_pm_pairs_kernel, dim3((unsigned)(nt * (nt + 1) / 2), (unsigned)npo), dim3(256), 0, st, o, v, Rp, ldp, Rm, ldm,
+                t2p, Hp, Hm, assign, std::max(Sp, 1), strideP, std::max(Sm, 1), strideM, (long long)(ldhp ? ldhp : ldp), (long long)(ldhm ? ldhm : ldm));
+}
+
+int dev_ccsd_finish_t2_rings_pairs(int64_t o, int64_t v, double* t2p, const double* U, const double* OV, const double* RS, const double* M, const double* eo,
+                                   const double* ev, double* t1n) {
+  PAIR_REQUIRE("dev_ccsd_finish_t2_rings_pairs")
+  if (!t2p || !U || !OV || !RS || !M || !eo || !ev) { set_error("dev_ccsd_finish_t2_rings_pairs: bad arguments"); return QEMB_ERR_ARG; }
+  const long long npo = o * (o + 1) / 2, nt = (v + 31) / 32;
+  return launch("dev_ccsd_finish_t2_rings_pairs", ccsd_finish_t2_rings_pairs_kernel, dim3((unsigned)(nt * nt), (unsigned)npo), dim3(256), 0, st, o, v, t2p, U, OV, RS, M,
+                eo, ev, t1n);
+}
+
+int dev_diis_push_pairs(int64_t o, int64_t v, const double* trial, const double* prev, double* e, int m, const double* const* ys, int self,
+                        double* row_dev, double* row_host, void* flag_host, unsigned long long seq) {
+  PAIR_REQUIRE("dev_diis_push_pairs")
+  if (m <= 0 || m > 8 || self < 0 || self >= m) { set_error("dev_diis_push_pairs: 1 <= m <= 8 vectors, 0 <= self < m"); return QEMB_ERR_ARG; }
+  if (!trial || !prev || !e || !ys || !row_dev || !row_host) { set_error("dev_diis_push_pairs: bad arguments"); return QEMB_ERR_ARG; }
+  PushK k{};
+  k.m = m; k.self = self;
+  bool vec2 = (v % 2 == 0) && al16(trial) && al16(prev) && al16(e);
+  for (int j = 0; j < m; ++j) { k.y[j] = ys[j]; vec2 = vec2 && al16(ys[j]); }
+  const int64_t nseg = o * (o + 1) / 2 + 1, nw = vec2 ? v * v / 2 : v * v;
+  const int gy = (int)std::min<int64_t>(nseg, NPART);
+  const int gx = (int)std::max<int64_t>(1, std::min<int64_t>((nw + 1023) / 1024, NPART / gy));
+  void* part = nullptr;
+  QTRY(dev_alloc(&part, sizeof(double) * 8 * NPART));
+  int rc = vec2 ? launch("dev_diis_push_pairs", diis_push_pairs_kernel<true>, dim3(gx, gy), dim3(256), 0, st, (int)o, (int)v, trial, prev, e, k, (double*)part)
+                : launch("dev_diis_push_pairs", diis_push_pairs_kernel<false>, dim3(gx, gy), dim3(256), 0, st, (int)o, (int)v, trial, prev, e, k, (double*)part);
+  if (!rc) rc = launch("dev_diis_push_pairs", pair_finish_partials_kernel, dim3(1), dim3(256), 0, st, m, gx * gy, (const double*)part, row_dev, row_host,
+                       (unsigned long long*)flag_host, seq);
+  dev_free(part);
+  return rc;
+}
+
+int dev_ccsd_extrapolate_energy_pairs(int64_t o, int64_t v, int nterms, const double* coef, const double* const* xs, double* amp, const double* L, double* tau,
+                                      double* e_dev, double* e_host, void* flag_host, unsigned long long seq) {
+  PAIR_REQUIRE("dev_ccsd_extrapolate_energy_pairs")
+  if (nterms <= 0 || nterms > 8) { set_error("dev_ccsd_extrapolate_energy_pairs: 1 <= nterms <= 8"); return QEMB_ERR_ARG; }
+  if (!coef || !xs || !amp || !L || !tau || !e_dev || !e_host) { set_error("dev_ccsd_extrapolate_energy_pairs: bad arguments"); return QEMB_ERR_ARG; }
+  ExtrapK k{};
+  k.n = nterms;
+  for (int q = 0; q < nterms; ++q) { k.x[q] = xs[q]; k.c[q] = coef[q]; }
+  const int64_t npo = o * (o + 1) / 2, nt = (v + 31) / 32;
+  const int G = (int)std::max<int64_t>(1, std::min<int64_t>(nt * nt, (int64_t)(8 * NPART) / npo));
+  void* part = nullptr;
+  QTRY(dev_alloc(&part, sizeof(double) * 8 * NPART));
+  int rc = launch("dev_ccsd_extrapolate_energy_pairs", ccsd_extrapolate_energy_pairs_kernel, dim3((unsigned)G, (unsigned)npo), dim3(256), 0, st, (int)o, (int)v, k, amp, L,
+                  tau, (double*)part);
+  if (!rc) rc = launch("dev_ccsd_extrapolate_energy_pairs", pair_finish_partials_kernel, dim3(1), dim3(256), 0, st, 1, (int)(G * npo), (const double*)part, e_dev, e_host,
+                       (unsigned long long*)flag_host, seq);
+  dev_free(part);
+  return rc;
+}
+
+}
diff --git a/quemb_amd/csrc/ccsd_pair_diis_ops_hostcheck.cpp b/quemb_amd/csrc/ccsd_pair_diis_ops_hostcheck.cpp
--- /dev/null
+++ b/quemb_amd/csrc/ccsd_pair_diis_ops_hostcheck.cpp
@@ -0,0 +1,100 @@
+#ifdef QEMB_HOSTCHECK
+#include <algorithm>
+#include <vector>
+#include "dev_ops.h"
+
+namespace qemb {
+
+#define PAIR_SHAPE(who) \
+  if (!ccsd_pair_diis_shape_ok(o, v)) { set_error(who ": shape outside the rule (ccsd_pair_diis_shape_ok)"); return QEMB_ERR_ARG; }
+
+int dev_ladder_scatter_pm_pairs(int64_t o, int64_t v, const double* Rp, int64_t ldp, const double* Rm, int64_t ldm, const double* Hp, const double* Hm,
+                                int assign, double* t2p, int Sp, int64_t strideP, int Sm, int64_t strideM, int64_t ldhp, int64_t ldhm) {
+  PAIR_SHAPE("dev_ladder_scatter_pm_pairs")
+  if (!ldhp) ldhp = ldp;
+  if (!ldhm) ldhm = ldm;
+  for (int64_t i = 0; i < o; ++i) for (int64_t j = 0; j <= i; ++j) for (int64_t a = 0; a < v; ++a) for (int64_t b = 0; b <= a; ++b) {
+    const bool has_m = (i > j && a > b);
+    const int64_t cp = a * (a + 1) / 2 + b, cm = a * (a - 1) / 2 + b, rp = i * (i + 1) / 2 + j, rm = i * (i - 1) / 2 + j;
+    double p = 0.0, m = 0.0;
+    for (int sl = 0; sl < std::max(Sp, 1); ++sl) p += Rp[sl * strideP + rp * ldp + cp];
+    if (has_m) for (int sl = 0; sl < std::max(Sm, 1); ++sl) m += Rm[sl * strideM + rm * ldm + cm];
+    if (Hp) p += (a == b ? 2.0 : 1.0) * Hp[rp * ldhp + cp];
+    if (Hm && has_m) m += Hm[rm * ldhm + cm];
+    double* t = t2p + rp * v * v;
+    t[a * v + b] = (assign ? 0.0 : t[a * v + b]) + (p + m);
+    if (a != b) t[b * v + a] = (assign ? 0.0 : t[b * v + a]) + (p - m);
+  }
+  return 0;
+}
+
+int dev_ccsd_finish_t2_rings_pairs(int64_t o, int64_t v, double* t2p, const double* U, const double* OV, const double* RS, const double* M, const double* eo,
+                                   const double* ev, double* t1n) {
+  PAIR_SHAPE("dev_ccsd_finish_t2_rings_pairs")
+  const int64_t ov = o * v;
+  auto F = [&](int64_t i, int64_t j, int64_t a, int64_t b) {
+    return U[((i * o + j) * v + a) * v + b] + RS[(i * v + a) * ov + j * v + b] - 0.5 * M[(i * v + a) * ov + j * v + b] - M[(i * v + b) * ov + j * v + a];
+  };
+  for (int64_t i = 0; i < o; ++i) for (int64_t j = 0; j <= i; ++j) for (int64_t a = 0; a < v; ++a) for (int64_t b = 0; b < v; ++b) {
+    const int64_t idx = ((i * o + j) * v + a) * v + b;
+    double* t = t2p + (i * (i + 1) / 2 + j) * v * v;
+    if (i == j && b > a) continue;
+    const double r = (t[a * v + b] + OV[idx] + F(i, j, a, b) + F(j, i, b, a)) / (eo[i] + eo[j] - ev[a] - ev[b]);
+    t[a * v + b] = r;
+    if (i == j) t[b * v + a] = r;
+  }
+  if (t1n) for (int64_t t = 0; t < ov; ++t) t1n[t] /= eo[t / v] - ev[t % v];
+  return 0;
+}
+
+static inline void pair_locate(int64_t o, int64_t v, int64_t x, int64_t& full, double& w) {
+  const int64_t nov = o * v, vv = v * v;
+  if (x < nov) { full = x; w = 1.0; return; }
+  const int64_t p = (x - nov) / vv, r = (x - nov) - p * vv;
+  int64_t i = 0;
+  while ((i + 1) * (i + 2) / 2 <= p) ++i;
+  const int64_t j = p - i * (i + 1) / 2;
+  full = nov + (i * o + j) * vv + r;
+  w = (i == j) ? 1.0 : 2.0;
+}
+
+int dev_diis_push_pairs(int64_t o, int64_t v, const double* trial, const double* prev, double* e, int m, const double* const* ys, int self,
+                        double* row_dev, double* row_host, void* flag_host, unsigned long long seq) {
+  PAIR_SHAPE("dev_diis_push_pairs")
+  if (m <= 0 || m > 8 || self < 0 || self >= m) { set_error("dev_diis_push_pairs: 1 <= m <= 8 vectors, 0 <= self < m"); return QEMB_ERR_ARG; }
+  const int64_t n = ccsd_pair_diis_len(o, v);
+  std::vector<double> w((size_t)n);
+  for (int64_t x = 0; x < n; ++x) { int64_t f; pair_locate(o, v, x, f, w[(size_t)x]); e[x] = trial[x] - prev[f]; }
+  for (int j = 0; j < m; ++j) {
+    const double* y = (j == self) ? e : ys[j];
+    double s = 0;
+    for (int64_t x = 0; x < n; ++x) s += (w[(size_t)x] * e[x]) * y[x];
+    row_dev[j] = s; row_host[j] = s;
+  }
+  if (flag_host) *(unsigned long long*)flag_host = seq;
+  return 0;
+}
+
+int dev_ccsd_extrapolate_energy_pairs(int64_t o, int64_t v, int nterms, const double* coef, const double* const* xs, double* amp, const double* L, double* tau,
+                                      double* e_dev, double* e_host, void* flag_host, unsigned long long seq) {
+  PAIR_SHAPE("dev_ccsd_extrapolate_energy_pairs")
+  if (nterms <= 0 || nterms > 8) { set_error("dev_ccsd_extrapolate_energy_pairs: 1 <= nterms <= 8"); return QEMB_ERR_ARG; }
+  const int64_t nov = o * v, vv = v * v;
+  auto comb = [&](int64_t x) { double acc = 0.0; for (int q = 0; q < nterms; ++q) acc += coef[q] * xs[q][x]; return acc; };
+  for (int64_t t = 0; t < nov; ++t) amp[t] = comb(t);
+  long double s = 0;
+  for (int64_t i = 0; i < o; ++i) for (int64_t j = 0; j <= i; ++j) for (int64_t a = 0; a < v; ++a) for (int64_t b = 0; b < v; ++b) {
+    const int64_t ij = ((i * o + j) * v + a) * v + b, ji = ((j * o + i) * v + b) * v + a;
+    const double val = comb(nov + (i * (i + 1) / 2 + j) * vv + a * v + b);
+    const double tv = val + amp[i * v + a] * amp[j * v + b];
+    amp[nov + ij] = val; tau[ij] = tv;
+    if (i != j) { amp[nov + ji] = val; tau[ji] = tv; }
+    s += (long double)(i == j ? 1.0 : 2.0) * L[ij] * tv;
+  }
+  *e_dev = (double)s; *e_host = (double)s;
+  if (flag_host) *(unsigned long long*)flag_host = seq;
+  return 0;
+}
+
+}
+#endif
diff --git a/quemb_amd/csrc/dev_ops.h b/quemb_amd/csrc/dev_ops.h
--- a/quemb_amd/csrc/dev_ops.h
+++ b/quemb_amd/csrc/dev_ops.h
@@ -337,6 +337,16 @@
 int dev_wait_flag(const void* flag_host, unsigned long long seq);
 int dev_ccsd_extrapolate_energy(int64_t o, int64_t v, int nterms, const double* coef, const double* const* xs, double* amp, const double* L,
                                 double* tau, double* e_dev, double* e_host, void* flag_host = nullptr, unsigned long long seq = 0);
+inline int64_t ccsd_pair_diis_len(int64_t o, int64_t v) { return o * v + o * (o + 1) / 2 * v * v; }
+inline bool ccsd_pair_diis_shape_ok(int64_t o, int64_t v) { return o >= 1 && v >= 1 && o * o <= 16384 && v <= 4096 && o * (o + 1) / 2 <= 65535; }
+int dev_ladder_scatter_pm_pairs(int64_t o, int64_t v, const double* Rp, int64_t ldp, const double* Rm, int64_t ldm, const double* Hp, const double* Hm,
+                                int assign, double* t2p, int Sp = 1, int64_t strideP = 0, int Sm = 1, int64_t strideM = 0, int64_t ldhp = 0, int64_t ldhm = 0);
+int dev_ccsd_finish_t2_rings_pairs(int64_t o, int64_t v, double* t2p, const double* U, const double* OV, const double* RS, const double* M, const double* eo,
+                                   const double* ev, double* t1n);
+int dev_diis_push_pairs(int64_t o, int64_t v, const double* trial, const double* prev, double* e, int m, const double* const* ys, int self,
+                        double* row_dev, double* row_host, void* flag_host = nullptr, unsigned long long seq = 0);
+int dev_ccsd_extrapolate_energy_pairs(int64_t o, int64_t v, int nterms, const double* coef, const double* const* xs, double* amp, const double* L, double* tau,
+                                      double* e_dev, double* e_host, void* flag_host = nullptr, unsigned long long seq = 0);
 
 int dev_gemv_rows(int64_t rows, int64_t cols, const double* T, int64_t ldt, const double* x,
                   double* y, double alpha, double beta);
diff --git a/quemb_amd/csrc/tensor_utils.h b/quemb_amd/csrc/tensor_utils.h
--- a/quemb_amd/csrc/tensor_utils.h
+++ b/quemb_amd/csrc/tensor_utils.h
@@ -147,6 +147,7 @@
 class DeviceDIIS {
  public:
   DeviceDIIS(int space, int64_t n) : space_(space), n_(n) {}
+  DeviceDIIS(int space, int64_t n, int64_t pair_o, int64_t pair_v) : space_(space), n_(ccsd_pair_diis_len(pair_o, pair_v)), po_(pair_o), pv_(pair_v) { (void)n; }
   int init() {
     xs_.resize(space_); es_.resize(space_);
     for (int i = 0; i < space_; ++i) { QTRY(xs_[i].alloc(n_)); QTRY(es_[i].alloc(n_)); }
@@ -185,6 +186,7 @@
   }
   int push_diff_issue(const double* trial, const double* prev) {
     const int slot = count_ % space_;
+    if (po_ > 0 && (space_ > 8 || trial != xs_[slot].p)) { set_error("DeviceDIIS: the pair layout takes at most eight vectors and a trial vector written in place"); return QEMB_ERR_ARG; }
     if (space_ > 8) {
       QTRY(lincomb2(n_, 1.0, trial, -1.0, prev, es_[slot]));
       if (trial != xs_[slot].p) QTRY(dcopy(n_, trial, xs_[slot]));
@@ -195,7 +197,8 @@
     QTRY(ensure_row_host());
     const double* ps[8];
     for (int q = 0; q < m; ++q) ps[q] = es_[q].p;
-    QTRY(dev_diis_push(n_, trial, prev, es_[slot], trial == xs_[slot].p ? nullptr : xs_[slot].p, m, ps, slot, scal_.p, row_host_, row_host_ + space_ + 1, ++seq_));
+    if (po_ > 0) QTRY(dev_diis_push_pairs(po_, pv_, trial, prev, es_[slot], m, ps, slot, scal_.p, row_host_, row_host_ + space_ + 1, ++seq_));
+    else QTRY(dev_diis_push(n_, trial, prev, es_[slot], trial == xs_[slot].p ? nullptr : xs_[slot].p, m, ps, slot, scal_.p, row_host_, row_host_ + space_ + 1, ++seq_));
     pending_slot_ = slot; flagged_ = true;
     return 0;
   }
@@ -240,7 +243,7 @@
   void reset() { count_ = 0; }
 
  private:
-  int space_; int64_t n_; int count_ = 0;
+  int space_; int64_t n_; int64_t po_ = 0, pv_ = 0; int count_ = 0;
   std::vector<DBuf> xs_, es_;
   DBuf scal_;
   std::vector<double> B_;
@@ -259,7 +262,7 @@
   }
  public:
   ~DeviceDIIS() { if (row_host_) { if (flagged_) (void)dev_sync_device(); dev_pinned_free(row_host_); } }
-  DeviceDIIS(DeviceDIIS&& o) noexcept : space_(o.space_), n_(o.n_), count_(o.count_), xs_(std::move(o.xs_)), es_(std::move(o.es_)), scal_(std::move(o.scal_)),
+  DeviceDIIS(DeviceDIIS&& o) noexcept : space_(o.space_), n_(o.n_), po_(o.po_), pv_(o.pv_), count_(o.count_), xs_(std::move(o.xs_)), es_(std::move(o.es_)), scal_(std::move(o.scal_)),
                                         B_(std::move(o.B_)), row_host_(o.row_host_), seq_(o.seq_), flagged_(o.flagged_), pending_slot_(o.pending_slot_) { o.row_host_ = nullptr; }
   DeviceDIIS(const DeviceDIIS&) = delete;
   DeviceDIIS& operator=(const DeviceDIIS&) = delete;
```

New measurement: 59.83, median of 6. No clear change (+0.7%).
